# shuaigroup/Renormalizer

Measured on AMD Instinct MI355X. Metric: TDVP-PS sweep site-updates/sec at (Nsite=50, Dbond=256, dphys=2/16), higher is better.
Workload: dtype c128

## Files before the change

include/mpsengine.h:

```cpp
#ifndef MPSENGINE_H
#define MPSENGINE_H

#include <stddef.h>
#include <stdint.h>

#ifdef __cplusplus
extern "C" {
#endif

typedef struct mpse_ctx mpse_ctx;

enum {
  MPSE_OK = 0,
  MPSE_ERR_OOM = 1,
  MPSE_ERR_SHAPE = 2,
  MPSE_ERR_NOCONV = 3,
  MPSE_ERR_HIP = 4,
  MPSE_ERR_ARG = 5
};

enum { MPSE_F64 = 0, MPSE_C128 = 1 };
enum { MPSE_DOMAIN_L = 0, MPSE_DOMAIN_R = 1 };


// ... 78 lines not shown
  int64_t d0, d1;
  int64_t danc;
  int64_t wl, wm, wr;
  int64_t env_unit;
  int64_t danc1;
} mpse_dims;

int mpse_env_update(mpse_ctx* ctx, int dtype, int domain, const mpse_dims* dims,
                    const void* env, int env_dtype, const void* ket, const void* bra, int bra_conj,
                    const void* W, int w_dtype, void* out);

int mpse_env_update_multi(mpse_ctx* ctx, int dtype, int domain, const mpse_dims* dims, int n_mpo,
                          const int64_t* wl, const int64_t* wr, const void* env, int env_dtype,
                          const void* ket, const void* bra, int bra_conj, const void* const* W, int w_dtype, void* out);

int mpse_env_unit_channel(mpse_ctx* ctx, int dtype, const void* env, int64_t D, int64_t w, double tol,
                          int64_t* unit_host);

typedef struct {
  int nsite;
  mpse_dims dims;
  const void* L; int l_dtype;
  const void* R; int r_dtype;
  const void* W0; const void* W1; int w_dtype;
  int64_t l_unit, r_unit;
} mpse_heff;

int mpse_heff_apply(mpse_ctx* ctx, int dtype, const mpse_heff* h, const void* C, void* out);

int mpse_mpo_site_hint(mpse_ctx* ctx, const void* W_dev, const double* W_host_f64, int64_t wl, int64_t d, int64_t wr);

int mpse_heff_fused_stats(mpse_ctx* ctx, int64_t* bond_launches, int64_t* site_launches);

int mpse_heff_apply2(mpse_ctx* ctx, int dtype, const mpse_heff* h, const void* C, void* out);

enum { MPSE_LEG_UP = 0, MPSE_LEG_DOWN = 1 };
typedef struct {
  int64_t Dl, Dr, d_up, d_down;
  int64_t wl1, wr1, wl2, wr2;
  int leg1, leg2;
  int trans1, trans2;
  const void* L; int l_dtype;
  const void* R; int r_dtype;
  const void* W1; const void* W2; int w_dtype;
} mpse_heff_ft;

int mpse_heff_apply_ft(mpse_ctx* ctx, int dtype, const mpse_heff_ft* h, const void* C, void* out);

int mpse_env_update_ft(mpse_ctx* ctx, int dtype, int domain, const mpse_heff_ft* h, const void* env, int env_dtype,
                       const void* X, void* out);

int mpse_expm_centre_mask(mpse_ctx* ctx, const void* mask_dev, int64_t nbytes);

int mpse_expm_lanczos(mpse_ctx* ctx, int dtype, const mpse_heff* h, double dt_re, double dt_im,
                      const void* C, void* out, double rtol, double atol, int max_dim, int* nvec);
int mpse_expm_lanczos_batch(mpse_ctx* ctx, int dtype, int count, const mpse_heff* h, double dt_re, double dt_im,
                            const void* const* C, void* const* out, double rtol, double atol, int max_dim, int* nvec);
int mpse_expm_lanczos_batch_stats(mpse_ctx* ctx, int64_t* batched_members, int64_t* single_members);
int mpse_expm_lanczos_path_stats(mpse_ctx* ctx, int64_t* counts, int n);

int mpse_davidson(mpse_ctx* ctx, int dtype, const mpse_heff* h, int twolayer, const void* hdiag_f64,
                  const void* mask_f64, int nroots, int nguess, const void* guess, double tol, int max_cycle,
                  int max_space, double lindep, double shift, double* e_host, void* x_out, int* ncycle, int* nmatvec);

int mpse_pcg(mpse_ctx* ctx, int dtype, const mpse_heff* h, int twolayer, double shift, const void* diag_f64,
             const void* mask_f64, const void* b, void* x, double tol, int max_iter, int* iters_host,
             double* relres_host, double* lvalue_host);
int mpse_pcg_stats(mpse_ctx* ctx, int64_t* counts, int n);

int mpse_pcg_sum(mpse_ctx* ctx, int dtype, int nterms, const mpse_heff_ft* terms, const double* weights_host,
                 double shift, const void* diag_f64, const void* mask_f64, const void* b, void* x, double tol,
                 int max_iter, int* iters_host, double* relres_host, double* lvalue_host);
int mpse_pcg_sum_stats(mpse_ctx* ctx, int64_t* counts, int n);

int mpse_site_factor_ft(mpse_ctx* ctx, const mpse_heff_ft* h, void* S_f64);
int mpse_diag_ft(mpse_ctx* ctx, const mpse_heff_ft* h, const void* S_f64, double weight, double shift, int accumulate,
                 void* diag_f64);

int mpse_truncate_select(const double* sigma_host, const int64_t* block_id_host, int64_t count, int64_t m_max,
                         double percent, int64_t* picked_host, int64_t* npicked);


int mpse_block_qr(mpse_ctx* ctx, int dtype, const void* coef, int64_t nrow, int64_t ncol,
                  int nblocks, const int64_t* row_idx_host, const int64_t* row_off_host,
                  const int64_t* col_idx_host, const int64_t* col_off_host,
                  int system_is_R, void* U, void* Vt, int64_t K);

int mpse_block_qr_stats(mpse_ctx* ctx, int64_t* calls, int64_t* chol_calls, int64_t* chol_fallbacks);

int mpse_block_qr_optimistic(mpse_ctx* ctx, int on);
int mpse_block_qr_check(mpse_ctx* ctx, int* tripped);

int mpse_block_qr_pass_stats(mpse_ctx* ctx, int64_t* blocks, int64_t* two_pass);

int mpse_block_qr_scheme(mpse_ctx* ctx, int scheme);

int mpse_block_svd(mpse_ctx* ctx, int dtype, const void* coef, int64_t nrow, int64_t ncol,
                   int nblocks, const int64_t* row_idx_host, const int64_t* row_off_host,
                   const int64_t* col_idx_host, const int64_t* col_off_host,
                   void* U, void* Vt, double* S_host, int64_t K);

int mpse_block_svd_full(mpse_ctx* ctx, int dtype, const void* coef, int64_t nrow, int64_t ncol,
                        int nblocks, const int64_t* row_idx_host, const int64_t* row_off_host,
                        const int64_t* col_idx_host, const int64_t* col_off_host, const int64_t* extra_host,
                        void* U, int64_t KU, void* Vt, int64_t KV, double* S_host, int64_t K);

// ... 10 lines not shown
```

renormalizer_amd/csrc/mpse_contract.hip:

```cpp
#include <deque>

#include "mpse_internal.h"
#include "mpse_plans.h"

using namespace mpse_plan;

namespace {

__device__ __forceinline__ long long off2(const mpse_index m, long long i) {
  if (m.lo_ext >= m.ext) return i * m.s_lo;
  const long long hi = i / m.lo_ext;
  return hi * m.s_hi + (i - hi * m.lo_ext) * m.s_lo;
}

template <typename T>
__global__ __launch_bounds__(256) void k_copy_strided(T* dst, const T* src, mpse_index mi, mpse_index ni, mpse_index mo,
                                                      mpse_index no, const int* skip) {
  if (skip && *skip) return;
  const long long nn = ni.ext;
  const long long total = mi.ext * nn;
  const long long stride = (long long)gridDim.x * blockDim.x;
  for (long long t = (long long)blockIdx.x * blockDim.x + threadIdx.x; t < total; t += stride) {
    const long long i = t / nn, j = t - i * nn;
    dst[off2(mo, i) + off2(no, j)] = src[off2(mi, i) + off2(ni, j)];
// ... 268 lines not shown
      const dim3 grid((unsigned)((total + 255) / 256));
      if (s.dtb == MPSE_C128)
        hipLaunchKernelGGL((k_wsmall<true>), grid, dim3(256), 0, ctx->stream, g);
      else
        hipLaunchKernelGGL((k_wsmall<false>), grid, dim3(256), 0, ctx->stream, g);
      MPSE_HIP(ctx, hipGetLastError());
      continue;
    }
    if (s.kind == K_WMIX) {
      if (!bufs[s.b]) return mpse_fail(ctx, MPSE_ERR_ARG, "plan: missing buffer");
      WmixArgs g;
      memset(&g, 0, sizeof(g));
      g.W = (const double*)bufs[s.b];
      g.ndst = (int)s.mix.size();
      g.Da = (int)s.wp_Da, g.d = (int)s.wp_d, g.wr = (int)s.wp_wr, g.Dk = (int)s.wp_Dk;
      g.nchunk = (g.d + WM_CHUNK - 1) / WM_CHUNK;
      g.skip = skip;
      int nslot = 0;
      for (int j = 0; j < g.ndst; ++j) {
        const WMixDst& q = s.mix[j];
        if (!bufs[q.dst]) return mpse_fail(ctx, MPSE_ERR_ARG, "plan: missing buffer");
        g.dst[j].dst = (double*)((char*)const_cast<void*>(bufs[q.dst]) + size_t(q.dst_off) * es);
        g.dst[j].s_a = q.s_a, g.dst[j].s_d = q.s_d, g.dst[j].nterm = q.nterm;
        for (int t = 0; t < q.nterm; ++t) {
          const WMixTerm& tm = q.term[t];
          if (!bufs[tm.src]) return mpse_fail(ctx, MPSE_ERR_ARG, "plan: missing buffer");
          WmixTermDev& o = g.dst[j].term[t];
          o.src = (const double*)((const char*)bufs[tm.src] + size_t(tm.src_off) * es);
          o.s_a = tm.s_a, o.s_d = tm.s_d, o.b = tm.b, o.f = tm.f, o.ident = tm.ident ? 1 : 0;
          o.slot = tm.ident ? 0 : nslot++;
          memcpy(o.e_lo, tm.e_lo, sizeof(o.e_lo));
          memcpy(o.e_hi, tm.e_hi, sizeof(o.e_hi));
        }
      }
      g.nslot = nslot;
      const size_t lds = size_t(nslot > 0 ? nslot : 1) * g.d * g.d * sizeof(double);
      if (lds > 64 * 1024) return mpse_fail(ctx, MPSE_ERR_SHAPE, "plan: MPO blocks of the elementwise step exceed the LDS");
      const long long total = (long long)s.wp_Da * g.nchunk * s.wp_Dk;
      const dim3 grid((unsigned)((total + 255) / 256));
      if (dtype == MPSE_C128)
        hipLaunchKernelGGL((k_wmix<true>), grid, dim3(256), lds, ctx->stream, g);
      else
        hipLaunchKernelGGL((k_wmix<false>), grid, dim3(256), lds, ctx->stream, g);
      MPSE_HIP(ctx, hipGetLastError());
      continue;
    }
    if (s.kind == K_GGEMM) {
      GroupedDesc gd;
      gd.dta = s.dta, gd.dtb = s.dtb;
      gd.ma = s.ma, gd.ka = s.ka, gd.kb = s.kb, gd.nb = s.nb, gd.mc = s.mc, gd.nc = s.nc;
      gd.ngrp = (int)s.groups.size();
      TmpBuf MA(ctx), MB(ctx);
      const unsigned char *fa = nullptr, *fb = nullptr;
      bool stable = true;
      if (s.scan_a.on && bufs[s.scan_a.buf]) {
        bool st = false;
        MPSE_TRY(occ_mask_get(ctx, sc, (const char*)bufs[s.scan_a.buf] + size_t(s.scan_a.off) * dtype_size(s.scan_a.dt),
                              s.scan_a.dt, s.scan_a.r, s.scan_a.k, MA, &fa, &gd.am_pitch, &st));
        stable = stable && st;
      }
      if (s.scan_b.on && bufs[s.scan_b.buf]) {
        bool st = false;
        MPSE_TRY(occ_mask_get(ctx, sc, (const char*)bufs[s.scan_b.buf] + size_t(s.scan_b.off) * dtype_size(s.scan_b.dt),
                              s.scan_b.dt, s.scan_b.r, s.scan_b.k, MB, &fb, &gd.bm_pitch, &st));
        stable = stable && st;
      }
      const unsigned char* cm = nullptr;
      int cm_pitch = 0;
      {
        const char* pc = (const char*)bufs[B_C];
        const int64_t K = s.kb.ext, N = s.nb.ext;
        const int64_t nkw = ((K + 15) / 16 + 7) / 8, ntn = (N + 63) / 64;
        if (sc && sc->in_krylov(pc) && sc->cmask.bytes == ntn * nkw * 8) {
          cm = static_cast<const unsigned char*>(sc->cmask.ptr);
          cm_pitch = (int)(nkw * 8);
        }
      }
      for (int i = 0; i < gd.ngrp; ++i) {
        const GGroupPlan& g = s.groups[i];
        GroupedGrp& o = gd.grp[i];
        if (!bufs[g.cbuf]) return mpse_fail(ctx, MPSE_ERR_ARG, "plan: missing buffer");
        o.C = (char*)const_cast<void*>(bufs[g.cbuf]) + size_t(g.c_off) * es;
        o.nseg = g.nseg;
        o.beta = g.beta;
        for (int q = 0; q < g.nseg; ++q) {
          const GSegPlan& sg = g.seg[q];
          if (!bufs[sg.abuf] || !bufs[sg.bbuf]) return mpse_fail(ctx, MPSE_ERR_ARG, "plan: missing buffer");
          o.seg[q].A = (const char*)bufs[sg.abuf] + size_t(sg.a_off) * dtype_size(s.dta);
          o.seg[q].B = (const char*)bufs[sg.bbuf] + size_t(sg.b_off) * dtype_size(s.dtb);
          if (fa && sg.am_row0 >= 0) o.seg[q].am = fa + size_t(sg.am_row0) * gd.am_pitch;
          if (sg.bm_kind == BM_SCAN && fb) {
            o.seg[q].bm = fb + sg.bm_kt0;
          } else if (sg.bm_kind == BM_CENTRE && cm) {
            o.seg[q].bm = cm;
            gd.bm_pitch = cm_pitch;
          }
        }
      }
      gd.masks_stable = stable;
      if (gd.ngrp == 1 && s.groups[0].split2) {
        if (!bufs[B_OUT2]) return mpse_fail(ctx, MPSE_ERR_ARG, "plan: missing second result");
        gd.split2 = true;
        gd.c2 = const_cast<void*>(bufs[B_OUT2]);
      }
      const bool completes =
          &s == &p.steps.back() && gd.ngrp == 1 && s.groups[0].cbuf == B_OUT && s.groups[0].c_off == 0;
      MPSE_TRY(gemm_grouped(ctx, gd, sc, completes ? dot : nullptr));
      continue;
    }
    const char* a = (const char*)bufs[s.a] + size_t(s.a_off) * dtype_size(s.dta);
    const char* b = (const char*)bufs[s.b] + size_t(s.b_off) * dtype_size(s.dtb);
    const int dtc = (s.dta == MPSE_C128 || s.dtb == MPSE_C128) ? MPSE_C128 : MPSE_F64;
    if (dtc != dtype)
      return mpse_fail(ctx, MPSE_ERR_ARG, "plan step dtype mismatch (got %d want %d)", dtc, dtype);
    char* c = (char*)const_cast<void*>(bufs[s.c]) + size_t(s.c_off) * dtype_size(dtc);
    if (!bufs[s.a] || !bufs[s.b] || !bufs[s.c]) return mpse_fail(ctx, MPSE_ERR_ARG, "plan: missing buffer");
    if (s.kind == K_COPY) {
      MPSE_TRY(copy_call(ctx, dtc, a, c, s.ma, s.ka, s.mc, s.nc, skip));
      continue;
    }
    ProductReq rq;
    if (&s == &p.steps.back() && s.c == B_OUT && s.c_off == 0 && s.batch == 1) rq.dot = dot;
    if (s.cin >= 0) {
      if (!bufs[s.cin]) return mpse_fail(ctx, MPSE_ERR_ARG, "plan: missing beta source");
      rq.cin = (const char*)bufs[s.cin] + size_t(s.cin_off) * dtype_size(dtc);
      rq.cin_m = s.mcin;
      rq.cin_n = s.ncin;
    }
    if (&s == slice_producer) {
      const size_t blk = size_t(s.mc.ext) * size_t(s.nc.ext) * dtype_size(dtc);
      if (SLC.alloc(4 * blk) == MPSE_OK) {
        rq.slices = SLC.p;
        rq.slices_cap = 4 * blk;
      }
    }
    MPSE_TRY(gemm_call(ctx, s.dta, s.dtb, s.conja, s.conjb, s.ma, s.ka, s.kb, s.nb, s.mc, s.nc, s.batch, s.sba, s.sbb,
                       s.sbc, a, b, c, 1.0, s.beta, s.skip_zero, sc, &rq));
    if (rq.slices_used > 0) {
      slices_used = rq.slices_used;
      slice_elems = (long long)s.mc.ext * s.nc.ext;
      slice_b_lo = s.c_off / (slice_consumer->w_Da * slice_consumer->w_d * slice_consumer->w_N);
      slice_b_hi = slice_b_lo + s.mc.ext / slice_consumer->w_Da;
    }
  }
  return MPSE_OK;
}

int heff_apply(mpse_ctx* ctx, int dtype, const mpse_heff* h, const void* C, void* out, const SolveScope* sc,
               MatvecReq* mv) {
  if (!ctx || !h || !C || !out || !h->L || !h->R) return MPSE_ERR_ARG;
  MPSE_BIND(ctx);
  if (dtype != MPSE_C128 && (h->l_dtype == MPSE_C128 || h->r_dtype == MPSE_C128 || h->w_dtype == MPSE_C128))
// ... 204 lines not shown
```

renormalizer_amd/csrc/mpse_core.hip:

```cpp
#include "mpse_internal.h"
#include "mpse_plans.h"

int mpse_fail(mpse_ctx* ctx, int code, const char* fmt, ...) {
  if (ctx) {
    va_list ap;
    va_start(ap, fmt);
    vsnprintf(ctx->err, sizeof(ctx->err), fmt, ap);
    va_end(ap);
  }
  return code;
}

__global__ __launch_bounds__(256) void k_zero8(unsigned long long* dst, long long n) {
  for (long long i = (long long)blockIdx.x * 256 + threadIdx.x; i < n; i += (long long)gridDim.x * 256) dst[i] = 0ull;
}
__global__ __launch_bounds__(256) void k_copy8(unsigned long long* dst, const unsigned long long* __restrict__ src,
                                               long long n) {
  for (long long i = (long long)blockIdx.x * 256 + threadIdx.x; i < n; i += (long long)gridDim.x * 256) dst[i] = src[i];
}

__global__ __launch_bounds__(256) void k_zero8x2(unsigned long long* a, long long na, unsigned long long* b, long long nb) {
  for (long long i = (long long)blockIdx.x * 256 + threadIdx.x; i < na + nb; i += (long long)gridDim.x * 256) {
    if (i < na)
      a[i] = 0ull;
// ... 302 lines not shown

int mpse_device_info(mpse_ctx* ctx, char* name, size_t name_len, int* n_cu, void** stream) {
  if (!ctx) return MPSE_ERR_ARG;
  if (name && name_len) snprintf(name, name_len, "%s", ctx->dev_name);
  if (n_cu) *n_cu = ctx->n_cu;
  if (stream) *stream = (void*)ctx->stream;
  return MPSE_OK;
}

static size_t bucket_of(size_t bytes) {
  if (bytes < 256) return 256;
  if (bytes <= (size_t(1) << 20)) return (bytes + 255) & ~size_t(255);
  size_t p = size_t(1) << 20;
  while ((p << 1) <= bytes) p <<= 1;
  size_t step = p >> 3;
  return ((bytes + step - 1) / step) * step;
}

int mpse_malloc(mpse_ctx* ctx, size_t bytes, void** dptr) {
  if (!ctx || !dptr) return MPSE_ERR_ARG;
  MPSE_BIND(ctx);
  std::lock_guard<std::mutex> lock(ctx->pool_mu);
  size_t b = bucket_of(bytes);
  auto it = ctx->free_blocks.find(b);
  void* p = nullptr;
  if (it != ctx->free_blocks.end()) {
    p = it->second;
    ctx->free_blocks.erase(it);
  } else {
    hipError_t e = hipMalloc(&p, b);
    ++ctx->n_device_allocs;
    if (e != hipSuccess) {
      (void)hipGetLastError();
      pool_trim_locked(ctx);
      e = hipMalloc(&p, b);
      if (e != hipSuccess) {
        (void)hipGetLastError();
        *dptr = nullptr;
        return mpse_fail(ctx, MPSE_ERR_OOM, "hipMalloc(%zu) failed: %s (pool %zu B, in use %zu B)", b,
                         hipGetErrorString(e), ctx->pool_bytes, ctx->in_use_bytes);
      }
    }
    ctx->pool_bytes += b;
  }
  ctx->live[p] = b;
  ctx->in_use_bytes += b;
  *dptr = p;
  return MPSE_OK;
}

int mpse_free(mpse_ctx* ctx, void* dptr) {
  if (!ctx) return MPSE_ERR_ARG;
  if (!dptr) return MPSE_OK;
  std::lock_guard<std::mutex> lock(ctx->pool_mu);
  auto it = ctx->live.find(dptr);
  if (it == ctx->live.end()) return mpse_fail(ctx, MPSE_ERR_ARG, "mpse_free: unknown pointer %p", dptr);
  if (!ctx->wsite_info.empty()) ctx->wsite_info.erase(dptr);
  if (ctx->defer_hold) {
    ctx->defer_frees.push_back(dptr);
    return MPSE_OK;
  }
  ctx->free_blocks.emplace(it->second, dptr);
  ctx->in_use_bytes -= it->second;
  ctx->live.erase(it);
  return MPSE_OK;
}


int mpse_defer_begin(mpse_ctx* ctx, int list) {
  if (!ctx || list < 0 || list > 1) return MPSE_ERR_ARG;
  if (ctx->defer_recording >= 0) return mpse_fail(ctx, MPSE_ERR_ARG, "mpse_defer_begin: already recording");
  if (ctx->defer_armed == list) return mpse_fail(ctx, MPSE_ERR_ARG, "mpse_defer_begin: list %d is armed", list);
  ctx->defer_ops[list].clear();
  ctx->defer_recording = list;
  defer_update_hold(ctx);
  return MPSE_OK;
}

int mpse_defer_end(mpse_ctx* ctx) {
  if (!ctx) return MPSE_ERR_ARG;
  if (ctx->defer_recording < 0) return mpse_fail(ctx, MPSE_ERR_ARG, "mpse_defer_end: not recording");
  ctx->defer_recording = -1;
  defer_update_hold(ctx);
  return MPSE_OK;
}

int mpse_defer_arm(mpse_ctx* ctx, int list) {
  if (!ctx || list < 0 || list > 1) return MPSE_ERR_ARG;
  if (ctx->defer_recording >= 0) return mpse_fail(ctx, MPSE_ERR_ARG, "mpse_defer_arm: still recording");
  ctx->defer_armed = list;
  return MPSE_OK;
}

int mpse_defer_discard(mpse_ctx* ctx) {
  if (!ctx) return MPSE_ERR_ARG;
  ctx->defer_ops[0].clear();
  ctx->defer_ops[1].clear();
  ctx->defer_recording = ctx->defer_armed = -1;
  defer_update_hold(ctx);
  return MPSE_OK;
}

int mpse_defer_run(mpse_ctx* ctx, int list) {
  if (!ctx || list < 0 || list > 1) return MPSE_ERR_ARG;
  if (ctx->defer_recording >= 0) return mpse_fail(ctx, MPSE_ERR_ARG, "mpse_defer_run: still recording");
  MPSE_BIND(ctx);
// ... 113 lines not shown
```

renormalizer_amd/csrc/mpse_gemm.hip:

```cpp
#include <cstdlib>

#include "mpse_device.h"
#include "mpse_internal.h"

typedef double v4d __attribute__((ext_vector_type(4)));

static unsigned long long* gemm_trace_ptr(const mpse_ctx* ctx) {
  static const bool f0_only = [] {
    const char* e = getenv("MPSE_GEMM_TRACE_ONLY");
    return e && e[0] == 'f';
  }();
  return (ctx->prof_on && !f0_only) ? ctx->gemm_trace : nullptr;
}

namespace {

struct IdxMap {
  long long s_hi, s_lo;
  int ext, lo;
};

constexpr int GMAX_GRP = 8, GMAX_SEG = 4;
struct GSeg {
  const double* A;
// ... 1133 lines not shown
  if (base_blocks < tiles_limit && nkt_all >= 4) {
    int want = (int)((wg_target + base_blocks - 1) / base_blocks);
    int maxs = nkt_all / 2;
    int S = want < maxs ? want : maxs;
    if (S > 1) {
      g.kt_per_split = (nkt_all + S - 1) / S;
      g.ksplit = (nkt_all + g.kt_per_split - 1) / g.kt_per_split;
      const size_t esz = (ca || cb) ? 16 : 8;
      const size_t ws_bytes = size_t(d->batch) * g.ksplit * size_t(g.M) * size_t(g.N) * esz;
      const bool compact = is_single(g.mC) && is_single(g.nC) && g.mC.s_lo == g.N && (g.nC.s_lo == 1 || g.N == 1);
      if (rq && rq->slices && !rq->dot && d->batch == 1 && compact && !g.use_beta && d->alpha_re == 1.0 &&
          d->alpha_im == 0.0 && ws_bytes <= rq->slices_cap) {
        g.ws = static_cast<double*>(rq->slices);
        rq->slices_used = g.ksplit;
        leave_slices = true;
      } else {
        MPSE_TRY(WSB.alloc(ws_bytes));
        g.ws = WSB.as<double>();
      }
    }
  }
  g.slice_fast = g.ksplit > 1 && d->batch == 1;
  long long nblk = base_blocks * g.ksplit;
  if (nblk > 0x7fffffffLL) return mpse_fail(ctx, MPSE_ERR_SHAPE, "mpse_gemm: grid too large");

  MatvecReq::Dot* dot = rq ? rq->dot : nullptr;
  long long rgx = (g.N + 255) / 256 > 64 ? 64 : (g.N + 255) / 256;
  long long rgy = (long long)g.M * d->batch > 32768 ? 32768 : (long long)g.M * d->batch;
  if (dot && d->batch == 1) {
    long long producers = base_blocks;
    if (g.ksplit > 1) {
      const long long cap_y = dot->cap / rgx;
      if (cap_y >= 1 && rgy > cap_y) rgy = cap_y;
      producers = rgx * rgy;
    }
    if (producers >= 1 && producers <= dot->cap) {
      g.dot_y = static_cast<const double*>(dot->y);
      g.dot_part = dot->part;
      dot->nb_out = (int)producers;
    }
  }

  dim3 grid((unsigned)nblk), block(256);
  mpse_ctx::ProfRec rec;
  const int variant = (ca ? 1 : 0) + (cb ? 2 : 0);
  const double mnk = double(g.M) * double(g.N) * double(g.K) * double(d->batch);
  const bool prof_this = prof_begin(
      ctx, variant, mnk * ((ca && cb) ? 8.0 : (ca || cb) ? 4.0 : 2.0),
      double(d->batch) * (double(g.M) * g.K * (ca ? 16 : 8) + double(g.K) * g.N * (cb ? 16 : 8) +
                          double(g.M) * g.N * ((ca || cb) ? 16 : 8) * (g.use_beta ? 2 : 1)),
      &rec);
  g.kt_counter = prof_this && ctx->prof_ktiles ? ctx->prof_ktiles + variant : nullptr;
  bool mask_a_stable = true, mask_b_stable = true;
  if (skip_zero && is_single(g.kA) && is_single(g.kB) && nkt_all >= 2 && d->batch <= 16384) {
    g.nkw = (nkt_all + 7) / 8;
    const size_t wa = size_t(d->batch) * g.mtiles_m * g.nkw, wb = size_t(d->batch) * g.mtiles_n * g.nkw;
    const bool sa = skip_zero & 1, sb_ = skip_zero & 2;
    auto cacheable = [&](const void* p) { return sc && sc->in_env(p); };
    auto make_key = [&](const void* p, const IdxMap& rm, const IdxMap& km, long long sb, int nrows, int tiles, int cplx) {
      mpse_ctx::OccKey k;
      memset(&k, 0, sizeof(k));
      k.ptr = p;
      k.r_ext = rm.ext, k.r_lo = rm.lo, k.r_shi = rm.s_hi, k.r_slo = rm.s_lo;
      k.k_ext = km.ext, k.k_lo = km.lo, k.k_shi = km.s_hi, k.k_slo = km.s_lo;
      k.sb = sb, k.nrows = nrows, k.tiles = tiles, k.nkw = g.nkw, k.batch = (int)d->batch, k.K = g.K, k.cplx = cplx;
      return k;
    };
    auto find = [&](const mpse_ctx::OccKey& k) -> void* {
      for (const auto& e : ctx->occ_cache)
        if (memcmp(&e.key, &k, sizeof(k)) == 0) return e.mask;
      return nullptr;
    };
    unsigned long long *am = nullptr, *bmk = nullptr;
    bool scan_a = sa, scan_b = sb_, b_structural = false;
    mpse_ctx::OccKey ka, kb;
    const bool ca_ok = sa && cacheable(g.A), cb_ok = sb_ && cacheable(g.B);
    if (ca_ok) {
      ka = make_key(g.A, g.mA, g.kA, g.sbA, g.M, g.mtiles_m, ca ? 1 : 0);
      if (void* hit = find(ka)) am = static_cast<unsigned long long*>(hit), scan_a = false;
    }
    if (cb_ok) {
      kb = make_key(g.B, g.nB, g.kB, g.sbB, g.N, g.mtiles_n, cb ? 1 : 0);
      if (void* hit = find(kb)) bmk = static_cast<unsigned long long*>(hit), scan_b = false;
    }
    if (scan_b && sc && sc->in_krylov(g.B) && d->batch == 1 &&
        (long long)(wb * sizeof(unsigned long long)) == sc->cmask.bytes) {
      bmk = static_cast<unsigned long long*>(const_cast<void*>(sc->cmask.ptr));
      scan_b = false;
      b_structural = true;
    }
    mask_a_stable = !sa || ca_ok;
    mask_b_stable = !sb_ || cb_ok || b_structural;
    size_t tmp_words = 0;
    if (scan_a && !ca_ok) tmp_words += wa;
    if (scan_b && !cb_ok) tmp_words += wb;
    if (tmp_words) MPSE_TRY(MSK.alloc(tmp_words * sizeof(unsigned long long)));
    unsigned long long* tmp = MSK.as<unsigned long long>();
    if (scan_a) {
      if (ca_ok) {
        void* pm = nullptr;
        MPSE_TRY(mpse_malloc(ctx, wa * sizeof(unsigned long long), &pm));
        ctx->occ_cache.push_back({ka, pm});
        am = static_cast<unsigned long long*>(pm);
      } else {
        am = tmp;
        tmp += wa;
      }
    }
    if (scan_b) {
      if (cb_ok) {
        void* pm = nullptr;
        MPSE_TRY(mpse_malloc(ctx, wb * sizeof(unsigned long long), &pm));
        ctx->occ_cache.push_back({kb, pm});
        bmk = static_cast<unsigned long long*>(pm);
      } else {
        bmk = tmp;
      }
    }
    if (scan_a || scan_b) {
      OccOperand oa{g.A, g.mA, g.kA, g.M, scan_a ? g.mtiles_m : 0, ca ? 1 : 0, g.a_kfast, g.sbA, reinterpret_cast<unsigned char*>(am)};
      OccOperand ob{g.B, g.nB, g.kB, g.N, scan_b ? g.mtiles_n : 0, cb ? 1 : 0, g.b_kfast, g.sbB, reinterpret_cast<unsigned char*>(bmk)};
      const int tmax = (scan_a ? g.mtiles_m : 0) > (scan_b ? g.mtiles_n : 0) ? (scan_a ? g.mtiles_m : 0) : (scan_b ? g.mtiles_n : 0);
      const dim3 og((nkt_all + 3) / 4, tmax, (unsigned)(2 * d->batch));
      hipLaunchKernelGGL(k_tile_occ, og, dim3(256), 0, ctx->stream, oa, ob, g.K, g.nkw, (int)d->batch, skip);
    }
    g.amask = sa ? am : nullptr;
    g.bmask = sb_ ? bmk : nullptr;
  }
  TmpBuf PERM(ctx);
  const long long ntile_all = (long long)g.tiles_m * g.tiles_n;
  if (d->batch == 1 && (g.amask || g.bmask) && ntile_all * g.ksplit > 2 * n_cu && ntile_all <= 2048) {
    const bool keep = sc && sc->occ_cache && mask_a_stable && mask_b_stable;
    int* pp = nullptr;
    if (keep)
      for (const auto& e : ctx->perm_cache)
        if (e.amask == g.amask && e.bmask == g.bmask && e.tiles_m == g.tiles_m && e.tiles_n == g.tiles_n && e.nkt == nkt_all)
          pp = static_cast<int*>(e.perm);
    if (!pp) {
      if (keep) {
        void* pm = nullptr;
        MPSE_TRY(mpse_malloc(ctx, size_t(ntile_all) * sizeof(int), &pm));
        ctx->perm_cache.push_back({g.amask, g.bmask, g.tiles_m, g.tiles_n, nkt_all, pm});
        pp = static_cast<int*>(pm);
      } else {
        MPSE_TRY(PERM.alloc(size_t(ntile_all) * sizeof(int)));
        pp = PERM.as<int>();
      }
      hipLaunchKernelGGL(k_tile_order, dim3(1), dim3(1024), 0, ctx->stream, g.amask, g.bmask, g.nkw, nkt_all, g.tiles_m,
                         g.tiles_n, 1, pp, skip, GemmGroups(), (unsigned char*)nullptr, 0);
    }
    g.perm = pp;
  }
  auto span_ok = [](const IdxMap& m, const IdxMap& k, bool cplx) {
    if (m.s_hi < 0 || m.s_lo < 0 || k.s_hi < 0 || k.s_lo < 0) return false;
    auto span = [](const IdxMap& x) {
      if (x.ext <= 1) return 0.0;
      if (x.lo == 0x7fffffff) return double(x.ext - 1) * double(x.s_lo);
      return double((x.ext - 1) / x.lo) * double(x.s_hi) + double(x.lo - 1) * double(x.s_lo);
    };
    return (span(m) + span(k) + 1.0) * (cplx ? 16.0 : 8.0) < 4.0e9;
  };
  const bool ks = is_single(g.kA) && is_single(g.kB) && span_ok(g.mA, g.kA, ca) && span_ok(g.nB, g.kB, cb);
  if (!g.perm && g.ksplit == 1 && d->batch == 1 && (long long)g.tiles_m * g.tiles_n >= 64) {
    const double size_a = double(g.M) * (ca ? 2 : 1), size_b = double(g.N) * (cb ? 2 : 1);
    if (size_a >= size_b && g.tiles_m % 8 == 0)
      g.die_group = 1;
    else if (g.tiles_n % 8 == 0)
      g.die_group = 2;
    else if (g.tiles_m % 8 == 0)
      g.die_group = 1;
  }
#define MPSE_LAUNCH(CA_, CB_)                                                                         \
  do {                                                                                                \
    if (ks && wide)                                                                                   \
      hipLaunchKernelGGL((k_gemm<CA_, CB_, true, 2, 1>), grid, dim3(512), 0, ctx->stream, g);         \
    else if (ks)                                                                                      \
      hipLaunchKernelGGL((k_gemm<CA_, CB_, true, 2>), grid, block, 0, ctx->stream, g);                \
    else                                                                                              \
      hipLaunchKernelGGL((k_gemm<CA_, CB_, false, 2>), grid, block, 0, ctx->stream, g);               \
  } while (0)
  const bool wide = nblk <= n_cu && nkt_all >= 2;
  {
    long long* gp = ctx->gemm_paths;
    const bool masked = ks && (g.amask || g.bmask);
    ++gp[mpse_ctx::GP_LAUNCH];
    gp[mpse_ctx::GP_GENERAL] += !ks;
    gp[mpse_ctx::GP_WIDE] += ks && wide;
    gp[mpse_ctx::GP_SPLIT_B1] += g.ksplit > 1 && d->batch == 1;
    gp[mpse_ctx::GP_SPLIT_BN] += g.ksplit > 1 && d->batch > 1;
    gp[mpse_ctx::GP_DIE1] += g.die_group == 1;
    gp[mpse_ctx::GP_DIE2] += g.die_group == 2;
    gp[mpse_ctx::GP_SKEW] += g.skew && !g.perm && !g.die_group;
    gp[mpse_ctx::GP_ORDER] += g.perm != nullptr;
    gp[mpse_ctx::GP_MASK] += masked;
    gp[mpse_ctx::GP_MASK_GLOBAL] += masked && g.nkw > 64;
  }
  if (ca && cb)
    MPSE_LAUNCH(true, true);
  else if (ca)
    MPSE_LAUNCH(true, false);
  else if (cb)
    MPSE_LAUNCH(false, true);
  else
    MPSE_LAUNCH(false, false);
#undef MPSE_LAUNCH
  if (g.ksplit > 1 && !leave_slices) {
    const dim3 rgrid((unsigned)rgx, (unsigned)rgy);
    if (ca || cb)
      hipLaunchKernelGGL((k_splitk_reduce<true>), rgrid, dim3(256), 0, ctx->stream, g, (int)d->batch);
    else
      hipLaunchKernelGGL((k_splitk_reduce<false>), rgrid, dim3(256), 0, ctx->stream, g, (int)d->batch);
  }
  if (prof_this) prof_end(ctx, rec);
  MPSE_HIP(ctx, hipGetLastError());
  return MPSE_OK;
}

int occ_mask_get(mpse_ctx* ctx, const SolveScope* sc, const void* ptr, int dtype, mpse_index r, mpse_index k,
                 TmpBuf& tmp, const unsigned char** flags, int* pitch, bool* stable) {
  IdxMap rm, km;
  if (!to_map(r, &rm) || !to_map(k, &km) || !is_single(km))
    return mpse_fail(ctx, MPSE_ERR_SHAPE, "occupancy scan: K index must be single level");
  const int K = km.ext, nrows = rm.ext, nkt = (K + BK - 1) / BK, nkw = (nkt + 7) / 8, tiles = (nrows + BM - 1) / BM;
  const bool cplx = dtype == MPSE_C128;
  auto fastest = [](const IdxMap& m) { return m.ext <= 1 ? (long long)1 << 60 : (m.s_lo < 0 ? -m.s_lo : m.s_lo); };
  const int kfast = fastest(km) <= fastest(rm);
  mpse_ctx::OccKey key;
  memset(&key, 0, sizeof(key));
  key.ptr = ptr;
  key.r_ext = rm.ext, key.r_lo = rm.lo, key.r_shi = rm.s_hi, key.r_slo = rm.s_lo;
  key.k_ext = km.ext, key.k_lo = km.lo, key.k_shi = km.s_hi, key.k_slo = km.s_lo;
  key.sb = 0, key.nrows = nrows, key.tiles = tiles, key.nkw = nkw, key.batch = 1, key.K = K, key.cplx = cplx ? 1 : 0;
  const bool cacheable = sc && sc->in_env(ptr);
  *pitch = nkw * 8;
  *stable = cacheable;
  if (cacheable)
    for (const auto& e : ctx->occ_cache)
      if (memcmp(&e.key, &key, sizeof(key)) == 0) {
        *flags = static_cast<const unsigned char*>(e.mask);
        return MPSE_OK;
      }
  void* pm = nullptr;
  const size_t bytes = size_t(tiles) * nkw * 8;
  if (cacheable) {
    MPSE_TRY(mpse_malloc(ctx, bytes, &pm));
    ctx->occ_cache.push_back({key, pm});
  } else {
    MPSE_TRY(tmp.alloc(bytes));
    pm = tmp.p;
  }
  OccOperand oa{static_cast<const double*>(ptr), rm, km, nrows, tiles, cplx ? 1 : 0, kfast, 0, static_cast<unsigned char*>(pm)};
  OccOperand ob = oa;
  ob.tiles = 0;
  hipLaunchKernelGGL(k_tile_occ, dim3((nkt + 3) / 4, tiles, 2), dim3(256), 0, ctx->stream, oa, ob, K, nkw, 1,
                     sc ? sc->skip : nullptr);
  MPSE_HIP(ctx, hipGetLastError());
  *flags = static_cast<const unsigned char*>(pm);
  return MPSE_OK;
}

int gemm_grouped(mpse_ctx* ctx, const GroupedDesc& d, const SolveScope* sc, MatvecReq::Dot* dot) {
  GemmArgs g;
  memset(&g, 0, sizeof(g));
  if (d.ngrp < 1 || d.ngrp > GMAX_GRP) return mpse_fail(ctx, MPSE_ERR_ARG, "grouped product: 1 .. %d groups", GMAX_GRP);
  if (!to_map(d.ma, &g.mA) || !to_map(d.ka, &g.kA) || !to_map(d.kb, &g.kB) || !to_map(d.nb, &g.nB) ||
      !to_map(d.mc, &g.mC) || !to_map(d.nc, &g.nC))
    return mpse_fail(ctx, MPSE_ERR_SHAPE, "grouped product: extent out of range");
  g.M = g.mA.ext, g.N = g.nB.ext, g.K = g.kA.ext;
  if (g.M != g.mC.ext || g.N != g.nC.ext || g.K != g.kB.ext) return mpse_fail(ctx, MPSE_ERR_SHAPE, "grouped product: extents disagree");
  if (g.M == 0 || g.N == 0) return MPSE_OK;
  const bool ca = d.dta == MPSE_C128, cb = d.dtb == MPSE_C128;
  auto span_ok = [](const IdxMap& m, const IdxMap& k, bool cplx) {
    if (m.s_hi < 0 || m.s_lo < 0 || k.s_hi < 0 || k.s_lo < 0) return false;
    auto span = [](const IdxMap& x) {
      if (x.ext <= 1) return 0.0;
      if (x.lo == 0x7fffffff) return double(x.ext - 1) * double(x.s_lo);
      return double((x.ext - 1) / x.lo) * double(x.s_hi) + double(x.lo - 1) * double(x.s_lo);
    };
    return (span(m) + span(k) + 1.0) * (cplx ? 16.0 : 8.0) < 4.0e9;
  };
  if (!is_single(g.kA) || !is_single(g.kB) || !span_ok(g.mA, g.kA, ca) || !span_ok(g.nB, g.kB, cb) || g.K % BK != 0 ||
      g.K < BK || (d.ngrp > 1 && g.M % BM != 0) || !cb)
    return mpse_fail(ctx, MPSE_ERR_SHAPE, "grouped product: needs single-level K indices, K a multiple of %d, group "
                     "heights a multiple of %d and a complex second operand", BK, BM);
  g.mtiles_m = (g.M + BM - 1) / BM;
  g.mtiles_n = (g.N + BN - 1) / BN;
  g.tiles_m = g.mtiles_m * d.ngrp;
  g.tiles_n = g.mtiles_n;
  auto fast = [](const IdxMap& m) { return m.ext <= 1 ? (long long)1 << 60 : (m.s_lo < 0 ? -m.s_lo : m.s_lo); };
  g.a_kfast = fast(g.kA) <= fast(g.mA);
  g.b_kfast = fast(g.kB) <= fast(g.nB);
  g.alpha_re = 1.0, g.beta_re = 1.0;
  g.ksplit = 1;
  g.skip = sc ? sc->skip : nullptr;
  g.skew = 1;
  g.trace = gemm_trace_ptr(ctx);
  GemmGroups& gg = g.gg;
  gg.ngrp = d.ngrp, gg.tiles_m_grp = g.mtiles_m, gg.nkt_seg = g.K / BK;
  gg.am_pitch = d.am_pitch, gg.bm_pitch = d.bm_pitch;
  gg.split2 = d.split2 ? 1 : 0;
  gg.C2 = static_cast<double*>(d.c2);
  gg.cpd = (ctx->n_cu > 0 ? ctx->n_cu : 256) / 8;
  if (d.split2 && (d.ngrp != 1 || !d.c2 || g.M % BM != 0))
    return mpse_fail(ctx, MPSE_ERR_ARG, "grouped product: halved tiles need one group, whole tile rows and a second result");
  int max_seg = 0;
  bool any_mask = false, any_beta = false;
  for (int i = 0; i < d.ngrp; ++i) {
    const GroupedGrp& s = d.grp[i];
    if (s.nseg < 1 || s.nseg > GMAX_SEG || !s.C) return mpse_fail(ctx, MPSE_ERR_ARG, "grouped product: bad group");
    gg.g[i].C = static_cast<double*>(s.C);
    gg.g[i].nseg = s.nseg;
    gg.g[i].use_beta = s.beta != 0.0 ? 1 : 0;
    if (s.beta != 0.0 && s.beta != 1.0) return mpse_fail(ctx, MPSE_ERR_ARG, "grouped product: beta must be 0 or 1");
    any_beta = any_beta || s.beta != 0.0;
    for (int q = 0; q < s.nseg; ++q) {
      if (!s.seg[q].A || !s.seg[q].B) return mpse_fail(ctx, MPSE_ERR_ARG, "grouped product: null operand");
      gg.g[i].seg[q] = GSeg{static_cast<const double*>(s.seg[q].A), static_cast<const double*>(s.seg[q].B), s.seg[q].am, s.seg[q].bm};
      any_mask = any_mask || s.seg[q].am || s.seg[q].bm;
    }
    max_seg = s.nseg > max_seg ? s.nseg : max_seg;
  }
  g.A = gg.g[0].seg[0].A, g.B = gg.g[0].seg[0].B, g.C = gg.g[0].C;
  g.use_beta = any_beta;
  const int nkt_max = max_seg * gg.nkt_seg;
  g.nkw = (any_mask && (nkt_max + 7) / 8 <= 64) ? (nkt_max + 7) / 8 : 0;
  const int n_cu = ctx->n_cu > 0 ? ctx->n_cu : 256;
  const long long ntile = (long long)g.tiles_m * g.tiles_n;
  if (ntile > 0x7fffffffLL) return mpse_fail(ctx, MPSE_ERR_SHAPE, "grouped product: grid too large");
  const long long nwg = ntile * (d.split2 ? 2 : 1);
  if (dot && d.ngrp == 1 && nwg >= 1 && nwg <= dot->cap) {
    g.dot_y = static_cast<const double*>(dot->y);
    g.dot_part = dot->part;
    dot->nb_out = (int)nwg;
  }
  mpse_ctx::ProfRec rec;
  const int variant = (ca ? 1 : 0) + (cb ? 2 : 0);
  double segs = 0;
  for (int i = 0; i < d.ngrp; ++i) segs += d.grp[i].nseg;
  const double mnk = double(g.M) * double(g.N) * double(g.K) * segs;
  const bool prof_this = prof_begin(ctx, variant, mnk * ((ca && cb) ? 8.0 : 4.0),
                                    segs * (double(g.M) * g.K * (ca ? 16 : 8) + double(g.K) * g.N * 16.0) +
                                        double(d.ngrp) * double(g.M) * g.N * 16.0 * (any_beta ? 2 : 1),
                                    &rec);
  g.kt_counter = prof_this && ctx->prof_ktiles ? ctx->prof_ktiles + variant : nullptr;
  TmpBuf PERM(ctx);
  if (g.nkw > 0 && (ntile > 2 * n_cu || d.split2) && ntile <= 2048) {
    int* pp = nullptr;
    const void *ka = gg.g[0].seg[0].am, *kb = gg.g[0].seg[0].bm;
    const int nkt_key = nkt_max + 1000 * d.ngrp;
    const bool keep = sc && sc->occ_cache && d.masks_stable;
    if (keep)
      for (const auto& e : ctx->perm_cache)
        if (e.amask == ka && e.bmask == kb && e.tiles_m == g.tiles_m && e.tiles_n == g.tiles_n && e.nkt == nkt_key)
          pp = static_cast<int*>(e.perm);
    const size_t perm_bytes = (size_t(ntile) * sizeof(int) + 7) & ~size_t(7), flag_pitch = size_t(g.nkw) * 8;
    if (!pp) {
      if (keep) {
        void* pm = nullptr;
        MPSE_TRY(mpse_malloc(ctx, perm_bytes + size_t(ntile) * flag_pitch, &pm));
        ctx->perm_cache.push_back({ka, kb, g.tiles_m, g.tiles_n, nkt_key, pm});
        pp = static_cast<int*>(pm);
      } else {
        MPSE_TRY(PERM.alloc(perm_bytes + size_t(ntile) * flag_pitch));
        pp = PERM.as<int>();
      }
      hipLaunchKernelGGL(k_tile_order, dim3(1), dim3(1024), 0, ctx->stream, (const unsigned long long*)nullptr,
                         (const unsigned long long*)nullptr, 0, nkt_max, g.tiles_m, g.tiles_n, d.split2 ? 0 : 1, pp,
                         g.skip, gg, reinterpret_cast<unsigned char*>(pp) + perm_bytes, (int)flag_pitch);
    }
    g.perm = pp;
    g.gg.flags = reinterpret_cast<const unsigned long long*>(reinterpret_cast<const char*>(pp) + perm_bytes);
  }
  if (!g.perm && ntile >= 64) {
    const double size_a = double(g.M) * d.ngrp * (ca ? 2 : 1), size_b = double(g.N) * 2;
    if (size_a >= size_b && g.tiles_m % 8 == 0)
      g.die_group = 1;
    else if (g.tiles_n % 8 == 0)
      g.die_group = 2;
    else if (g.tiles_m % 8 == 0)
      g.die_group = 1;
  }
  const dim3 grid((unsigned)nwg);
  const bool wide = nwg <= n_cu;
  ++ctx->gemm_paths[mpse_ctx::GP_GROUPED];
  ctx->gemm_paths[mpse_ctx::GP_GROUPED_SPLIT2] += gg.split2 != 0;
  if (ca) {
    if (wide)
      hipLaunchKernelGGL((k_gemm<true, true, true, 2, 1, true>), grid, dim3(512), 0, ctx->stream, g);
    else
      hipLaunchKernelGGL((k_gemm<true, true, true, 2, 2, true>), grid, dim3(256), 0, ctx->stream, g);
  } else {
    if (wide)
      hipLaunchKernelGGL((k_gemm<false, true, true, 2, 1, true>), grid, dim3(512), 0, ctx->stream, g);
    else
      hipLaunchKernelGGL((k_gemm<false, true, true, 2, 2, true>), grid, dim3(256), 0, ctx->stream, g);
  }
  if (prof_this) prof_end(ctx, rec);
  MPSE_HIP(ctx, hipGetLastError());
  return MPSE_OK;
}

extern "C" int mpse_gemm(mpse_ctx* ctx, const mpse_gemm_desc* d, const void* A, const void* B, void* C) {
  if (ctx && d && MPSE_RECORDING(ctx)) {
    const mpse_gemm_desc dc = *d;
    ctx->defer_ops[ctx->defer_recording].push_back([ctx, dc, A, B, C] { return mpse_gemm(ctx, &dc, A, B, C); });
    return MPSE_OK;
  }
  return gemm_impl(ctx, d, A, B, C, d ? (d->skip_zero_tiles & 3) : 0, nullptr, nullptr);
}

extern "C" int mpse_gemm_path_stats(mpse_ctx* ctx, int64_t* counts, int n) {
  if (!ctx || n < 0 || (n > 0 && !counts)) return MPSE_ERR_ARG;
  for (int i = 0; i < n && i < mpse_ctx::GP_COUNT; ++i) counts[i] = ctx->gemm_paths[i];
  return MPSE_OK;
}

int gemm_call(mpse_ctx* ctx, int dta, int dtb, int conja, int conjb, mpse_index ma, mpse_index ka, mpse_index kb,
              mpse_index nb, mpse_index mc, mpse_index nc, int64_t batch, int64_t sba, int64_t sbb, int64_t sbc,
              const void* A, const void* B, void* C, double alpha, double beta, int skip_zero, const SolveScope* sc,
              ProductReq* rq) {
  mpse_gemm_desc d;
// ... 40 lines not shown
```

renormalizer_amd/csrc/mpse_heff0.hip:

```cpp
#include "mpse_device.h"
#include "mpse_internal.h"

typedef double v4d __attribute__((ext_vector_type(4)));

namespace {

__device__ __forceinline__ v4d mfma(double a, double b, v4d c) {
  return __builtin_amdgcn_mfma_f64_16x16x4f64(a, b, c, 0, 0, 0);
}

constexpr int F0_TMAX = 16;
struct F0Term {
  int b, e, x, pad;
  double w;
};
struct F0Info {
  int unit;
  int nt;
  unsigned long long lts;
  unsigned long long frn;
  unsigned long long cts;
  unsigned bpack, epack;
  double w[4];
};
// ... 12 lines not shown
  const int* nterm;
  const int* skip;
  const F0Info* info;
  long long n;
  int Dl, Dr, wl, wr, d, ntl, ntr, nkc, fc_pitch;
  unsigned long long* trace;
};

__device__ __forceinline__ void f0_transpose(double2* __restrict__ rt, const double2* __restrict__ r, int D, int w, int blk,
                                             int nblk) {
  const long long n = (long long)D * w * D;
  const long long stride = (long long)nblk * 256;
  for (long long i = (long long)blk * 256 + threadIdx.x; i < n; i += stride) {
    const int l = (int)(i % D);
    const long long bk = i / D;
    rt[i] = r[(long long)l * w * D + bk];
  }
}

__device__ __forceinline__ void f0_flags(const double2* __restrict__ E, int D, int w, int nt, unsigned char* __restrict__ F,
                                         int rt, int b) {
  __shared__ int s_f[64];
  const int row = threadIdx.x >> 4, col = threadIdx.x & 15;
  if (threadIdx.x < 64) s_f[threadIdx.x] = 0;
  __syncthreads();
  const double2* base = E + ((long long)(16 * rt + row) * w + b) * D;
  for (int ct = 0; ct < nt; ++ct) {
    const double2 v = base[16 * ct + col];
    if (v.x != 0.0 || v.y != 0.0) s_f[ct] = 1;
  }
  __syncthreads();
  if ((int)threadIdx.x < nt) F[((long long)rt * w + b) * nt + threadIdx.x] = s_f[threadIdx.x] ? 1 : 0;
}

__global__ __launch_bounds__(256) void k_f0_prepare(const double2* __restrict__ L, const double2* __restrict__ R,
                                                     double2* __restrict__ rt, unsigned char* __restrict__ FL,
                                                     unsigned char* __restrict__ FR, int Dl, int Dr, int wl, int wr, int ntl,
                                                     int ntr, const int* __restrict__ skip) {
  if (skip && *skip) return;
  int blk = blockIdx.x;
  if (blk < ntl * wl) {
    f0_flags(L, Dl, wl, ntl, FL, blk / wl, blk % wl);
    return;
  }
  blk -= ntl * wl;
  if (blk < ntr * wr) {
    f0_flags(R, Dr, wr, ntr, FR, blk / wr, blk % wr);
    return;
  }
  blk -= ntr * wr;
  f0_transpose(rt, R, Dr, wr, blk, (int)gridDim.x - ntl * wl - ntr * wr);
}

__global__ __launch_bounds__(1024) void k_f0_valid(const unsigned char* __restrict__ FL, const unsigned char* __restrict__ FC,
                                                    const unsigned char* __restrict__ FR, const F0Term* __restrict__ terms,
                                                    const int* __restrict__ nterm, int wl, int wr, int d, int ntl, int ntr,
                                                    int nkc, int fc_pitch, unsigned long long* __restrict__ mask,
                                                    const int* __restrict__ skip) {
  if (skip && *skip) return;
  __shared__ unsigned long long s1[64], s2[64];
  const int nparts = wr * nkc, tid = threadIdx.x;
  if (tid < 64) s1[tid] = s2[tid] = 0;
  __syncthreads();
  for (int t = tid; t < ntl * nparts; t += 1024) {
    const int at = t / nparts, s = t - at * nparts, f = s / nkc, kc = s - f * nkc;
    bool any = false;
    for (int q = 0; q < nterm[f]; ++q) {
      const F0Term tm = terms[f * F0_TMAX + q];
      for (int ct = 0; ct < ntl; ++ct)
        any = any || (FL[((long long)at * wl + tm.b) * ntl + ct] && (!FC || FC[(tm.e * nkc + kc) * fc_pitch + ct]));
    }
    if (any) atomicOr(&s1[at], 1ull << s);
  }
  for (int t = tid; t < ntr * nparts; t += 1024) {
    const int lt = t / nparts, s = t - lt * nparts, f = s / nkc, kc = s - f * nkc;
    bool any = false;
    for (int j = 0; j < 4; ++j) {
      const int kt = 4 * kc + j;
      if (kt < ntr) any = any || FR[((long long)lt * wr + f) * ntr + kt];
    }
    if (any) atomicOr(&s2[lt], 1ull << s);
  }
  __syncthreads();
  for (int t = tid; t < ntl * d * ntr; t += 1024) {
    const int row = t / ntr, lt = t - row * ntr;
    mask[t] = s1[row / d] & s2[lt];
  }
}

__global__ __launch_bounds__(1024) void k_f0_plan(const unsigned char* __restrict__ FL, const unsigned char* __restrict__ FC,
                                                   const unsigned char* __restrict__ FR, const F0Term* __restrict__ terms,
                                                   const int* __restrict__ nterm, int wl, int wr, int d, int ntl, int ntr,
                                                   int nkc, int fc_pitch, unsigned long long* __restrict__ mask, int n_cu,
                                                   F0Info* __restrict__ info, int compact, const int* __restrict__ skip) {
  if (skip && *skip) return;
  constexpr int WMAX = 256, MROWS = 1024;
  __shared__ unsigned long long s1[64], s2[64];
  __shared__ int hist[WMAX], start[WMAX], s_nw;
  __shared__ unsigned long long mL[MROWS], mR[MROWS], mC[64];
  __shared__ F0Term sT[16 * F0_TMAX];
  __shared__ int sNT[16];
  const int nparts = wr * nkc, tid = threadIdx.x, lane = tid & 63, wave = tid >> 6, nu = ntl * nparts * d;
  auto rows_to_masks = [&](const unsigned char* F, int nrows, int nt, int pitch, unsigned long long* out) {
    for (int r0 = wave; r0 < nrows; r0 += 64) {
      unsigned char v[4];
#pragma unroll
// ... 412 lines not shown
  if (dot && nwg * d > dot->cap) return MPSE_OK;
  std::vector<F0Term> terms(size_t(wr) * F0_TMAX);
  std::vector<int> nterm(wr, 0);
  for (int f = 0; f < wr; ++f) {
    if (h->nsite == 0) {
      terms[size_t(f) * F0_TMAX] = F0Term{f, 0, 0, 0, 1.0};
      nterm[f] = 1;
      continue;
    }
    for (int b = 0; b < wl; ++b)
      for (int x = 0; x < d; ++x)
        for (int e = 0; e < d; ++e) {
          const double v = w_host[((size_t(b) * d + x) * d + e) * wr + f];
          if (v == 0.0) continue;
          if (nterm[f] == F0_TMAX) return MPSE_OK;
          terms[size_t(f) * F0_TMAX + nterm[f]++] = F0Term{b, e, x, 0, v};
        }
  }
  const unsigned char* FC = nullptr;
  int fc_pitch = 0;
  {
    const long long nkw = (ntl + 7) / 8;
    const char* pc = static_cast<const char*>(C);
    if (sc && sc->in_krylov(pc) && sc->cmask.bytes == (long long)d * nkc * nkw * 8) {
      FC = static_cast<const unsigned char*>(sc->cmask.ptr);
      fc_pitch = (int)(nkw * 8);
    }
  }
  const size_t rt_bytes = size_t(wr) * Dr * Dr * 16;
  const size_t fl_bytes = (size_t(ntl) * wl * ntl + 15) & ~size_t(15), fr_bytes = (size_t(ntr) * wr * ntr + 15) & ~size_t(15);
  const size_t tm_bytes = terms.size() * sizeof(F0Term), nt_bytes = (size_t(wr) * sizeof(int) + 15) & ~size_t(15);
  const size_t mk_bytes = size_t(ntl) * d * ntr * 8;
  const size_t nu = size_t(nwg) * d;
  const size_t od_bytes = (nu * sizeof(F0Info) + 15) & ~size_t(15);
  bool compact = ntl <= 16 && ntr <= 16 && wl <= 255 && d <= 255;
  for (int f = 0; f < wr && compact; ++f)
    for (int x = 0; x < d; ++x) {
      int c = 0;
      for (int q = 0; q < nterm[f]; ++q) c += terms[size_t(f) * F0_TMAX + q].x == x;
      if (c > 4) compact = false;
    }
  if (!sc) return MPSE_OK;
  const int* skip = sc->skip;
  mpse_ctx::F0Cache& fc = ctx->f0;
  char* base = nullptr;
  const bool hit = fc.buf && fc.L == h->L && fc.R == h->R && fc.W == h->W0 && fc.cmask == (const void*)FC && fc.Dl == Dl &&
                   fc.Dr == Dr && fc.w == wr && fc.nsite == h->nsite;
  const size_t o_fl = rt_bytes, o_fr = o_fl + fl_bytes, o_tm = o_fr + fr_bytes, o_nt = o_tm + tm_bytes, o_mk = o_nt + nt_bytes;
  const size_t o_od = o_mk + mk_bytes, tot_bytes = o_od + od_bytes;
  static const bool order_on = [] {
    const char* e = getenv("MPSE_F0_ORDER");
    return !(e && e[0] == '0');
  }();
  if (hit) {
    base = static_cast<char*>(fc.buf);
  } else {
    void* p = nullptr;
    heff0_drop_cache(ctx);
    MPSE_TRY(mpse_malloc(ctx, tot_bytes, &p));
    fc.buf = p, fc.L = h->L, fc.R = h->R, fc.W = h->W0, fc.cmask = FC, fc.Dl = Dl, fc.Dr = Dr, fc.w = wr, fc.nsite = h->nsite;
    base = static_cast<char*>(p);
    {
      std::vector<char> up(tm_bytes + nt_bytes, 0);
      memcpy(up.data(), terms.data(), tm_bytes);
      memcpy(up.data() + tm_bytes, nterm.data(), size_t(wr) * sizeof(int));
      MPSE_TRY(stage_h2d(ctx, base + o_tm, up.data(), up.size()));
    }
    const long long nel = (long long)wr * Dr * Dr;
    int nb = (int)((nel + 255) / 256);
    if (nb > 2048) nb = 2048;
    hipLaunchKernelGGL(k_f0_prepare, dim3(ntl * wl + ntr * wr + nb), dim3(256), 0, ctx->stream,
                       static_cast<const double2*>(h->L), static_cast<const double2*>(h->R), reinterpret_cast<double2*>(base),
                       reinterpret_cast<unsigned char*>(base + o_fl), reinterpret_cast<unsigned char*>(base + o_fr), Dl, Dr, wl,
                       wr, ntl, ntr, skip);
    if (order_on)
      hipLaunchKernelGGL(k_f0_plan, dim3(1), dim3(1024), 0, ctx->stream, reinterpret_cast<const unsigned char*>(base + o_fl), FC,
                         reinterpret_cast<const unsigned char*>(base + o_fr), reinterpret_cast<const F0Term*>(base + o_tm),
                         reinterpret_cast<const int*>(base + o_nt), wl, wr, d, ntl, ntr, nkc, fc_pitch,
                         reinterpret_cast<unsigned long long*>(base + o_mk), ctx->n_cu > 0 ? ctx->n_cu : 256,
                         reinterpret_cast<F0Info*>(base + o_od), compact ? 1 : 0, skip);
    else
      hipLaunchKernelGGL(k_f0_valid, dim3(1), dim3(1024), 0, ctx->stream, reinterpret_cast<const unsigned char*>(base + o_fl), FC,
                         reinterpret_cast<const unsigned char*>(base + o_fr), reinterpret_cast<const F0Term*>(base + o_tm),
                         reinterpret_cast<const int*>(base + o_nt), wl, wr, d, ntl, ntr, nkc, fc_pitch,
                         reinterpret_cast<unsigned long long*>(base + o_mk), skip);
  }
  F0Args g{};
  g.L = static_cast<const double*>(h->L);
  g.Rt = reinterpret_cast<const double*>(base);
  g.C = static_cast<const double*>(C);
  g.parts = static_cast<double*>(pr.ptr);
  g.FL = reinterpret_cast<const unsigned char*>(base + o_fl);
  g.FC = FC;
  g.FR = reinterpret_cast<const unsigned char*>(base + o_fr);
  g.terms = reinterpret_cast<const F0Term*>(base + o_tm);
  g.nterm = reinterpret_cast<const int*>(base + o_nt);
  g.mask = reinterpret_cast<const unsigned long long*>(base + o_mk);
  g.skip = skip;
  g.info = order_on ? reinterpret_cast<const F0Info*>(base + o_od) : nullptr;
  g.trace = ctx->prof_on ? ctx->gemm_trace : nullptr;
  g.n = n;
  g.Dl = Dl, g.Dr = Dr, g.wl = wl, g.wr = wr, g.d = d, g.ntl = ntl, g.ntr = ntr, g.nkc = nkc, g.fc_pitch = fc_pitch;
  if (dot) {
    g.y = static_cast<const double*>(dot->y);
    g.dot_part = dot->part;
    dot->nb_out = nwg * d;
  }
  {
    const double fl = h->nsite == 0 ? 8.0 * wr * double(Dl) * Dr * (double(Dl) + Dr)
                                    : 8.0 * double(Dl) * Dl * wl * d * Dr + 4.0 * double(Dl) * Dr * wl * wr * d * d +
                                          8.0 * double(Dl) * Dr * Dr * wr * d;
    const double by = 16.0 * (double(Dl) * wl * Dl + double(Dr) * wr * Dr + 2.0 * double(n));
    ProfScope fprof(ctx, 7, fl, by);
    hipLaunchKernelGGL(k_heff0_fused, dim3(nwg * d), dim3(256), 0, ctx->stream, g);
    fprof.end();
  }
  MPSE_HIP(ctx, hipGetLastError());
  ++ctx->f0_launches[h->nsite == 1 ? 1 : 0];
  pr.used = nparts;
  pr.mask = g.mask;
  pr.mask_row = Dr;
  pr.mask_tiles = ntr;
  *taken = true;
  return MPSE_OK;
}

extern "C" int mpse_heff_fused_stats(mpse_ctx* ctx, int64_t* bond_launches, int64_t* site_launches) {
  if (!ctx) return MPSE_ERR_ARG;
  if (bond_launches) *bond_launches = ctx->f0_launches[0];
  if (site_launches) *site_launches = ctx->f0_launches[1];
  return MPSE_OK;
}
```

renormalizer_amd/csrc/mpse_internal.h:

```cpp
#pragma once
#include <hip/hip_runtime.h>

#include <cstdarg>
#include <cstdlib>
#include <cstdint>
#include <cstdio>
#include <cstring>
#include <functional>
#include <map>
#include <memory>
#include <mutex>
#include <string>
#include <unordered_map>
#include <vector>

#include "../../include/mpsengine.h"

struct mpse_ctx {
  int device = 0;
  hipStream_t stream = nullptr;
  int n_cu = 0;
  char err[512] = {0};
  char dev_name[128] = {0};

// ... 47 lines not shown
  };
  std::unordered_map<const void*, WSiteEntry> wsite_info;
  std::vector<std::function<int()>> defer_ops[2];
  int defer_recording = -1;
  int defer_armed = -1;
  bool defer_hold = false;
  std::vector<void*> defer_frees;
  struct CMask {
    const void* ptr = nullptr;
    long long bytes = 0;
  } cmask_pending;
  unsigned long long* gemm_trace = nullptr;
  bool gemm_trace_checked = false;
  std::vector<OccEntry> occ_cache;
  struct PermEntry {
    const void *amask, *bmask;
    int tiles_m, tiles_n, nkt;
    void* perm;
  };
  std::vector<PermEntry> perm_cache;
  struct SmallRt {
    const void* src = nullptr;
    void* rt = nullptr;
    size_t bytes = 0;
  } small_rt;
  struct F0Cache {
    void* buf = nullptr;
    const void *L = nullptr, *R = nullptr, *W = nullptr, *cmask = nullptr;
    int Dl = 0, Dr = 0, w = 0, nsite = -1;
  } f0;
  long long f0_launches[2] = {0, 0};
  enum GemmPath {
    GP_LAUNCH, GP_GENERAL, GP_WIDE, GP_SPLIT_B1, GP_SPLIT_BN, GP_DIE1, GP_DIE2, GP_SKEW, GP_ORDER, GP_MASK,
    GP_MASK_GLOBAL, GP_GROUPED, GP_GROUPED_SPLIT2, GP_COUNT
  };
  long long gemm_paths[GP_COUNT] = {0};
  long long qr_chol_calls = 0, qr_chol_fallbacks = 0, qr_calls = 0;
  bool qr_optimistic = false;
  int qr_scheme = -1;
  int* qr_words_dev = nullptr;
  long long lz_batch_members = 0, lz_batch_single = 0;
  enum LzPath {
    LP_SYNC, LP_ASYNC_DONE, LP_HOST_FIRST, LP_HOST_LATER, LP_LIMIT, LP_BD_ASYNC, LP_BD_SYNC, LP_FULL, LP_CONV,
    LP_NOCONV, LP_MERGED, LP_WAITS, LP_GROW, LP_PARTS, LP_VMASK, LP_UNVEC, LP_RESCALE, LP_ALIAS_RESTART, LP_COUNT
  };
  long long lz_paths[LP_COUNT] = {0};
  enum PcgStat {
    PS_SOLVES, PS_ITERS, PS_MATVECS, PS_WAITS, PS_END_TOL, PS_END_MAXITER, PS_END_CURVATURE, PS_TWOLAYER, PS_MASKED,
    PS_COUNT
  };
  long long pcg_stats[PS_COUNT] = {0};
  enum PcgSumStat { PSS_SOLVES, PSS_ITERS, PSS_TERM_APPLIES, PSS_WAITS, PSS_DIAGS, PSS_COUNT };
  long long pcg_sum_stats[PSS_COUNT] = {0};
};
int qr_words(mpse_ctx* ctx);

int mpse_fail(mpse_ctx* ctx, int code, const char* fmt, ...);
inline int mpse_bind(mpse_ctx* ctx) {
  int cur = -1;
  if (hipGetDevice(&cur) == hipSuccess && cur == ctx->device) return MPSE_OK;
  if (hipSetDevice(ctx->device) != hipSuccess) return mpse_fail(ctx, MPSE_ERR_HIP, "hipSetDevice(%d) failed", ctx->device);
  return MPSE_OK;
}
int stage_h2d(mpse_ctx* ctx, void* dst, const void* src_host, size_t bytes);
int device_zero(mpse_ctx* ctx, void* dst, size_t bytes);
inline void wsite_written(mpse_ctx* ctx, const void* dst, size_t bytes) {
  if (!dst || !bytes) return;
  std::lock_guard<std::mutex> lock(ctx->pool_mu);
  if (ctx->wsite_info.empty()) return;
  const char* lo = static_cast<const char*>(dst);
  for (auto it = ctx->wsite_info.begin(); it != ctx->wsite_info.end();) {
    const char* w = static_cast<const char*>(it->first);
    if (lo < w + it->second.bytes && w < lo + bytes)
      it = ctx->wsite_info.erase(it);
    else
      ++it;
  }
}
void prof_drain(mpse_ctx* ctx);
bool prof_begin(mpse_ctx* ctx, int variant, double flops, double bytes, mpse_ctx::ProfRec* rec);
void prof_end(mpse_ctx* ctx, const mpse_ctx::ProfRec& rec);
struct ProfScope {
  mpse_ctx* ctx;
  mpse_ctx::ProfRec rec;
  bool on;
  ProfScope(mpse_ctx* c, int variant, double flops, double bytes) : ctx(c), on(prof_begin(c, variant, flops, bytes, &rec)) {}
  ProfScope(const ProfScope&) = delete;
  ProfScope& operator=(const ProfScope&) = delete;
  void end() {
    if (on) prof_end(ctx, rec);
    on = false;
  }
  ~ProfScope() {
    if (!on) return;
    ctx->prof_free_events.push_back(rec.e0);
    ctx->prof_free_events.push_back(rec.e1);
  }
};

#define MPSE_HIP(ctx, call)                                                              \
  do {                                                                                   \
    hipError_t _e = (call);                                                              \
    if (_e != hipSuccess)                                                                \
      return mpse_fail((ctx), (_e == hipErrorOutOfMemory) ? MPSE_ERR_OOM : MPSE_ERR_HIP, \
                       "%s:%d %s -> %s", __FILE__, __LINE__, #call, hipGetErrorString(_e)); \
  } while (0)

#define MPSE_TRY(call)            \
  do {                            \
    int _s = (call);              \
    if (_s != MPSE_OK) return _s; \
  } while (0)

#define MPSE_BIND(ctx) MPSE_TRY(mpse_bind(ctx))

#define MPSE_RECORDING(ctx) ((ctx)->defer_recording >= 0)
int defer_replay(mpse_ctx* ctx, int status);

struct TmpBuf {
  mpse_ctx* ctx;
  void* p = nullptr;
  TmpBuf(mpse_ctx* c) : ctx(c) {}
  int alloc(size_t bytes) { return mpse_malloc(ctx, bytes ? bytes : 16, &p); }
  ~TmpBuf() {
    if (p) mpse_free(ctx, p);
  }
  template <class T>
  T* as() { return reinterpret_cast<T*>(p); }
};

static inline size_t dtype_size(int dt) { return dt == MPSE_C128 ? 16 : 8; }
static inline mpse_index idx1(int64_t ext, int64_t stride) { return mpse_index{ext, ext > 0 ? ext : 1, 0, stride}; }
static inline mpse_index idx2(int64_t hi_ext, int64_t lo_ext, int64_t s_hi, int64_t s_lo) {
  return mpse_index{hi_ext * lo_ext, lo_ext > 0 ? lo_ext : 1, s_hi, s_lo};
}

struct SolveScope {
  mpse_ctx* ctx;
  const int* skip = nullptr;
  bool occ_cache = false;
  const char* env_lo[2] = {nullptr, nullptr};
  const char* env_hi[2] = {nullptr, nullptr};
  mpse_ctx::CMask cmask;
  const char* krylov_lo = nullptr;
  const char* krylov_hi = nullptr;

  explicit SolveScope(mpse_ctx* c) : ctx(c) {}
  SolveScope(const SolveScope&) = delete;
  SolveScope& operator=(const SolveScope&) = delete;
  ~SolveScope();
  bool in_env(const void* p) const {
    const char* c = static_cast<const char*>(p);
    return occ_cache && ((c >= env_lo[0] && c < env_hi[0]) || (c >= env_lo[1] && c < env_hi[1]));
  }
  bool in_krylov(const void* p) const {
    const char* c = static_cast<const char*>(p);
    return cmask.ptr && c && c >= krylov_lo && c < krylov_hi;
  }
};

struct MatvecReq {
  struct Dot {
    const void* y = nullptr;
    double* part = nullptr;
    int cap = 0;
    int nb_out = 0;
  } dot;
  struct Parts {
    void* ptr = nullptr;
    long long cap_elems = 0, n = 0;
    int used = 0;
    bool masked_ok = false;
    const unsigned long long* mask = nullptr;
    int mask_row = 0, mask_tiles = 0;
  } parts;
};

struct ProductReq {
  MatvecReq::Dot* dot = nullptr;
  const void* cin = nullptr;
  mpse_index cin_m{}, cin_n{};
  void* slices = nullptr;
  size_t slices_cap = 0;
  int slices_used = 0;
};

int heff_apply(mpse_ctx* ctx, int dtype, const mpse_heff* h, const void* C, void* out, const SolveScope* sc,
               MatvecReq* mv);
int heff_apply2(mpse_ctx* ctx, int dtype, const mpse_heff* h, const void* C, void* out, const SolveScope* sc);
int heff_apply_ft(mpse_ctx* ctx, int dtype, const mpse_heff_ft* h, const void* C, void* out, const SolveScope* sc);
int heff_small_try(mpse_ctx* ctx, int dtype, const mpse_heff* h, const void* C, void* out, const SolveScope* sc,
                   MatvecReq* mv, bool* taken);
void heff_small_drop_cache(mpse_ctx* ctx);

struct BatchMember {
  const void* L;
  const void* R;
  const void* W;
  void* Rt;
  const void* C;
  void* out;
};
template <class T>
__host__ __device__ inline T* member_ptr(T* p, unsigned m, long long mstride) {
  return p ? reinterpret_cast<T*>(reinterpret_cast<uintptr_t>(p) + uintptr_t(m) * uintptr_t(mstride)) : p;
}
bool heff_small_batch_plan(const mpse_heff* h, int dtype, int64_t n, int dot_cap, size_t* rt_bytes, int* nparts,
                           int* nb_dot);
int heff_small_batch_rt(mpse_ctx* ctx, int dtype, const mpse_heff* h, int B, const BatchMember* mem, const int* skip0,
                        long long mstride);
int heff_small_batch_apply(mpse_ctx* ctx, int dtype, const mpse_heff* h, int B, const BatchMember* mem,
                           const void* C0, void* parts0, int64_t n, double* dot_part0, int dot_cap, const int* skip0,
                           long long mstride);
int heff0_fused_parts(const mpse_heff* h, int dtype);
int heff0_fused_try(mpse_ctx* ctx, int dtype, const mpse_heff* h, const void* C, const double* w_host,
                    const SolveScope* sc, MatvecReq* mv, bool* taken);
void heff0_drop_cache(mpse_ctx* ctx);
inline SolveScope::~SolveScope() {
  for (auto& e : ctx->occ_cache) mpse_free(ctx, e.mask);
  ctx->occ_cache.clear();
  for (auto& e : ctx->perm_cache) mpse_free(ctx, e.perm);
  ctx->perm_cache.clear();
  heff_small_drop_cache(ctx);
}

int gemm_call(mpse_ctx* ctx, int dta, int dtb, int conja, int conjb, mpse_index ma, mpse_index ka,
              mpse_index kb, mpse_index nb, mpse_index mc, mpse_index nc, int64_t batch, int64_t sba,
              int64_t sbb, int64_t sbc, const void* A, const void* B, void* C, double alpha = 1.0,
              double beta = 0.0, int skip_zero = 0, const SolveScope* sc = nullptr, ProductReq* rq = nullptr);

struct GroupedSeg {
  const void* A = nullptr;
  const void* B = nullptr;
  const unsigned char* am = nullptr;
  const unsigned char* bm = nullptr;
};
struct GroupedGrp {
  GroupedSeg seg[4];
  void* C = nullptr;
  int nseg = 0;
  double beta = 0.0;
};
struct GroupedDesc {
  int dta = MPSE_F64, dtb = MPSE_F64;
  mpse_index ma{}, ka{}, kb{}, nb{}, mc{}, nc{};
  int ngrp = 0;
  GroupedGrp grp[8];
  int am_pitch = 0, bm_pitch = 0;
  bool masks_stable = false;
  bool split2 = false;
  void* c2 = nullptr;
};
int gemm_grouped(mpse_ctx* ctx, const GroupedDesc& d, const SolveScope* sc, MatvecReq::Dot* dot);
int occ_mask_get(mpse_ctx* ctx, const SolveScope* sc, const void* ptr, int dtype, mpse_index r, mpse_index k,
                 TmpBuf& tmp, const unsigned char** flags, int* pitch, bool* stable);

int publish_and_wait(mpse_ctx* ctx, const double* dsrc, int count, int slot);
int publish_wait_seq(mpse_ctx* ctx, double seq, const double* dsrc, int count, int slot);

int dotc_sync(mpse_ctx* ctx, int dtype, const void* x, const void* y, int64_t n, double* re, double* im);

struct HhParam {
  double tau_re, tau_im;
  double scale_re, scale_im;
  double g[6];
};
struct QrBlk {
  long long ws_off;
  long long q_off;
  int mm, nn, k;
  int prm_off;
  int nq = 0;
  long long row_off = 0, col_off = 0;
};
constexpr int HH_BATCH_MAX_ROWS = 4096;
constexpr unsigned long long GEMM_TRACE_CAP = 1ull << 21;
constexpr int GEMM_TRACE_WORDS = 10;
int hh_qr(mpse_ctx* ctx, bool cplx, double* ws, double* q, HhParam* prm, const QrBlk* blks_host, int nblk, bool form_q,
          const QrBlk* blks_dev = nullptr);
bool cholqr_eligible(const mpse_ctx* ctx, const QrBlk* blks, int nblk);
int cholqr_blocks(mpse_ctx* ctx, bool cplx, double* ws, const QrBlk* blks, int nblk, const long long* drows,
                  const long long* dcols, int herm, void* U, void* Vt, long long K, long long ncol, bool* ok);
int device_zero2(mpse_ctx* ctx, void* a, size_t abytes, void* b, size_t bbytes);
```

renormalizer_amd/csrc/mpse_vec.hip:

```cpp
#include <cmath>
#include <complex>
#include <cstdlib>

#include "mpse_device.h"
#include "mpse_internal.h"

namespace {

template <bool CPLX>
__global__ __launch_bounds__(RED_THREADS) void k_dot_partial(const double* __restrict__ x, const double* __restrict__ y,
                                                             long long n, double* __restrict__ partial,
                                                             const int* __restrict__ done) {
  if (done && *done) return;
  double re = 0, im = 0;
  const long long stride = (long long)gridDim.x * RED_THREADS;
  if (CPLX) {
    const double2* x2 = reinterpret_cast<const double2*>(x);
    const double2* y2 = reinterpret_cast<const double2*>(y);
    for (long long i = (long long)blockIdx.x * RED_THREADS + threadIdx.x; i < n; i += 2 * stride) {
      const long long i1 = i + stride;
      const bool h1 = i1 < n;
      const double2 a0 = x2[i], b0 = y2[i];
      const double2 a1 = h1 ? x2[i1] : make_double2(0.0, 0.0), b1 = h1 ? y2[i1] : make_double2(0.0, 0.0);
      re += a0.x * b0.x + a0.y * b0.y;
// ... 814 lines not shown
  const size_t lb = size_t(s.Dl_ket) * s.wl * s.Dl_ket * (h->l_dtype == MPSE_C128 ? 16 : 8);
  const size_t rb = size_t(s.Dr_ket) * s.wr * s.Dr_ket * (h->r_dtype == MPSE_C128 ? 16 : 8);
  sc.env_lo[0] = static_cast<const char*>(h->L), sc.env_hi[0] = sc.env_lo[0] + lb;
  sc.env_lo[1] = static_cast<const char*>(h->R), sc.env_hi[1] = sc.env_lo[1] + rb;
  sc.occ_cache = true;
}

constexpr int LZ_FALLBACK = -77;
constexpr int LZ_BADSTART = -78;

int expm_lanczos_async(mpse_ctx* ctx, int dtype, const mpse_heff* h, std::complex<double> dt, const void* Cin, void* out,
                       double rtol, double atol, int max_dim, int* nvec, int64_t n) {
  const bool cplx = dtype == MPSE_C128;
  const size_t es = dtype_size(dtype);
  const int64_t nd = n * (cplx ? 2 : 1);
  const double tiny = 100.0 * double(n) * 2.220446049250313e-16;
  const int limit = max_dim < LZ_MAXM ? max_dim : LZ_MAXM;
  const unsigned long long key = ((unsigned long long)h->nsite << 60) ^ ((unsigned long long)n << 1) ^ (cplx ? 1ull : 0ull);
  int hint = 0;
  {
    auto it = ctx->lz_hint.find(key);
    if (it != ctx->lz_hint.end()) hint = it->second;
  }
  int wait_from = hint > 0 ? hint - 1 : 6;
  if (wait_from < 6) wait_from = 6;

  int cap = hint + 4 > 16 ? hint + 4 : 16;
  if (cap > limit + 1) cap = limit + 1;
  TmpBuf V(ctx), W(ctx), RES(ctx), SCAL(ctx);
  MPSE_TRY(V.alloc(size_t(cap) * n * es));
  long long wcap = (n <= 65536 ? 4 : 2) * n;
  const int f0_parts = (cplx && (reinterpret_cast<uintptr_t>(Cin) & 15) == 0) ? heff0_fused_parts(h, dtype) : 0;
  if ((long long)f0_parts * n > wcap) wcap = (long long)f0_parts * n;
  MPSE_TRY(W.alloc(size_t(wcap) * es));
  MPSE_TRY(RES.alloc(size_t(n) * es));
  const int SC_CTL = 4 + 4 * 130, SC_COEF = SC_CTL + 8;
  MPSE_TRY(SCAL.alloc(size_t(SC_COEF + 4 * LZ_MAXM) * sizeof(double)));
  double* scal = SCAL.as<double>();
  LzCtl* ctl = reinterpret_cast<LzCtl*>(scal + SC_CTL);
  double* coef = scal + SC_COEF;
  const int* done = &ctl->done;
  const int nb = red_blocks(nd);
  constexpr int DOT_CAP = 4096;
  double* part_a = ctx->dscratch + 16 * RED_MAX_BLOCKS;
  static_assert(16 * RED_MAX_BLOCKS + 2 * DOT_CAP < (1 << 16) - 8, "dot partials fit the device scratch");
  double* part_b = ctx->dscratch + 4 * RED_MAX_BLOCKS;
  const bool vec16 = (cplx || n % 2 == 0) && (reinterpret_cast<uintptr_t>(Cin) & 15) == 0;
  const double vbytes = double(n) * double(es);
  auto vec = [&](int j) { return V.as<char>() + size_t(j) * n * es; };

  SolveScope scope(ctx);
  scope.skip = done;
  keep_env_masks(scope, h);
  scope.cmask = ctx->cmask_pending;
  ctx->cmask_pending = mpse_ctx::CMask();

  const unsigned char* vmask = nullptr;
  int vm_row = 0, vm_kw = 0;
  static const bool vmask_on = [] {
    const char* e = getenv("MPSE_VEC_MASK");
    return !(e && e[0] == '0');
  }();
  if (vmask_on && vec16 && cplx && scope.cmask.ptr && h->dims.Dl_ket > 0 && h->dims.Dl_bra == h->dims.Dl_ket &&
      h->dims.Dr_bra == h->dims.Dr_ket && n < (int64_t(1) << 31)) {
    const int64_t Dl = h->dims.Dl_ket, N = n / Dl;
    const int64_t nkw = ((Dl + 15) / 16 + 7) / 8;
    if (N * Dl == n && N % 64 == 0 && scope.cmask.bytes == (N / 64) * nkw * 8) {
      vmask = static_cast<const unsigned char*>(scope.cmask.ptr);
      vm_row = (int)N;
      vm_kw = (int)(nkw * 8);
    }
  }
  auto bracket = [&](double bytes, auto&& launch) {
    mpse_ctx::ProfRec rec;
    const bool pt = prof_begin(ctx, 4, 0.0, bytes, &rec);
    launch();
    if (pt) prof_end(ctx, rec);
  };
  auto dot_partials = [&](const void* x, const void* y, double* dst) {
    bracket(2.0 * vbytes, [&] {
      if (cplx)
        hipLaunchKernelGGL((k_dot_partial<true>), dim3(nb), dim3(RED_THREADS), 0, ctx->stream, (const double*)x,
                           (const double*)y, (long long)n, dst, done);
      else
        hipLaunchKernelGGL((k_dot_partial<false>), dim3(nb), dim3(RED_THREADS), 0, ctx->stream, (const double*)x,
                           (const double*)y, (long long)n, dst, done);
    });
  };
  auto scale_into = [&](void* dst, const void* src, double* b2_out) {
    bracket(2.0 * vbytes, [&] {
      if (vec16)
        hipLaunchKernelGGL(k_scale_into_dev<true>, dim3(nb), dim3(RED_THREADS), 0, ctx->stream, (double*)dst,
                           (const double*)src, (long long)nd, (const double*)part_b, nb, b2_out, done);
      else
        hipLaunchKernelGGL(k_scale_into_dev<false>, dim3(nb), dim3(RED_THREADS), 0, ctx->stream, (double*)dst,
                           (const double*)src, (long long)nd, (const double*)part_b, nb, b2_out, done);
    });
  };
  double* part_b2[2] = {ctx->dscratch + 4 * RED_MAX_BLOCKS, ctx->dscratch + 8 * RED_MAX_BLOCKS};
  bracket(3.0 * vbytes, [&] {
    if (cplx)
      hipLaunchKernelGGL((k_lz_start<true>), dim3(nb), dim3(RED_THREADS), 0, ctx->stream, (double*)vec(0), (const double*)Cin,
                         (long long)n, part_b2[0], ctl);
    else
      hipLaunchKernelGGL((k_lz_start<false>), dim3(nb), dim3(RED_THREADS), 0, ctx->stream, (double*)vec(0),
                         (const double*)Cin, (long long)n, part_b2[0], ctl);
// ... 267 lines not shown
  out_host[0] = sqrt(re);
  return MPSE_OK;
}

static int expm_lanczos_solve(mpse_ctx* ctx, int dtype, const mpse_heff* h, double dt_re, double dt_im, const void* Cin,
                              void* out, double rtol, double atol, int max_dim, int* nvec, bool async_first = true,
                              bool rescale_ok = true);

static int expm_lanczos_rescaled(mpse_ctx* ctx, int dtype, const mpse_heff* h, double dt_re, double dt_im,
                                 const void* Cin, void* out, double rtol, double atol, int max_dim, int* nvec, int64_t n,
                                 const mpse_ctx::CMask& cmask, bool rescale_ok) {
  const int64_t nd = n * (dtype == MPSE_C128 ? 2 : 1);
  std::vector<double> hv(static_cast<size_t>(nd));
  MPSE_TRY(mpse_memcpy_d2h(ctx, hv.data(), Cin, size_t(nd) * sizeof(double)));
  double mx = 0.0;
  for (double x : hv) {
    if (!std::isfinite(x)) return mpse_fail(ctx, MPSE_ERR_ARG, "expm_lanczos: non-finite start vector");
    mx = std::max(mx, std::fabs(x));
  }
  if (!(mx > 0.0)) return mpse_fail(ctx, MPSE_ERR_ARG, "expm_lanczos: zero start vector");
  if (!rescale_ok) return mpse_fail(ctx, MPSE_ERR_ARG, "expm_lanczos: start vector out of range after scaling");
  const int e = -std::ilogb(mx);
  for (double& x : hv) x = std::ldexp(x, e);
  TmpBuf S(ctx);
  MPSE_TRY(S.alloc(size_t(nd) * sizeof(double)));
  MPSE_TRY(mpse_memcpy_h2d(ctx, S.p, hv.data(), size_t(nd) * sizeof(double)));
  ++ctx->lz_paths[mpse_ctx::LP_RESCALE];
  ctx->cmask_pending = cmask;
  const int st = expm_lanczos_solve(ctx, dtype, h, dt_re, dt_im, S.p, out, rtol, std::ldexp(atol, e), max_dim, nvec,
                                    true, false);
  if (st == MPSE_OK || st == MPSE_ERR_NOCONV) {
    hipLaunchKernelGGL((k_scal<false>), dim3(ew_blocks(nd)), dim3(256), 0, ctx->stream, (double*)out, (long long)nd,
                       std::ldexp(1.0, -e), 0.0);
    MPSE_HIP(ctx, hipGetLastError());
  }
  return st;
}

int mpse_expm_centre_mask(mpse_ctx* ctx, const void* mask_dev, int64_t nbytes) {
  if (!ctx || (nbytes > 0 && !mask_dev) || nbytes < 0) return MPSE_ERR_ARG;
  ctx->cmask_pending = mpse_ctx::CMask();
  if (nbytes > 0) {
    ctx->cmask_pending.ptr = mask_dev;
    ctx->cmask_pending.bytes = nbytes;
  }
  return MPSE_OK;
}

int mpse_expm_lanczos(mpse_ctx* ctx, int dtype, const mpse_heff* h, double dt_re, double dt_im, const void* Cin,
                      void* out, double rtol, double atol, int max_dim, int* nvec) {
  if (!ctx || !h || !Cin || !out) return MPSE_ERR_ARG;
  if (MPSE_RECORDING(ctx)) return mpse_fail(ctx, MPSE_ERR_ARG, "expm_lanczos: cannot be recorded (mpse_defer_begin is open)");
  MPSE_BIND(ctx);
  const int st = expm_lanczos_solve(ctx, dtype, h, dt_re, dt_im, Cin, out, rtol, atol, max_dim, nvec);
  ctx->cmask_pending = mpse_ctx::CMask();
  return defer_replay(ctx, st);
}

static int expm_lanczos_solve(mpse_ctx* ctx, int dtype, const mpse_heff* h, double dt_re, double dt_im, const void* Cin,
                              void* out, double rtol, double atol, int max_dim, int* nvec, bool async_first,
                              bool rescale_ok) {
  const bool cplx = dtype == MPSE_C128;
  if (!cplx && dt_im != 0.0)
    return mpse_fail(ctx, MPSE_ERR_ARG, "expm_lanczos: complex time step needs a complex128 centre tensor");
  const mpse_dims& s = h->dims;
  if ((s.Dl_bra > 0 && s.Dl_bra != s.Dl_ket) || (s.Dr_bra > 0 && s.Dr_bra != s.Dr_ket))
    return mpse_fail(ctx, MPSE_ERR_SHAPE, "expm_lanczos: the effective Hamiltonian must be square (bra bonds == ket bonds)");
  const int64_t anc = s.danc > 0 ? s.danc : 1;
  int64_t n = s.Dl_ket * s.Dr_ket;
  if (h->nsite >= 1) n *= s.d0 * anc;
  if (h->nsite == 2) n *= s.d1 * (s.danc1 > 0 ? s.danc1 : anc);
  if (n <= 0) return mpse_fail(ctx, MPSE_ERR_SHAPE, "expm_lanczos: empty centre tensor");
  if (max_dim <= 0 || max_dim > 128) max_dim = 128;
  const size_t es = dtype_size(dtype);
  {
    const char *c0 = static_cast<const char*>(Cin), *o0 = static_cast<const char*>(out);
    const size_t bytes = size_t(n) * es;
    if (o0 != c0 && o0 < c0 + bytes && c0 < o0 + bytes)
      return mpse_fail(ctx, MPSE_ERR_ARG, "expm_lanczos: out overlaps C without being C");
  }
  const mpse_ctx::CMask cmask = ctx->cmask_pending;
  if (async_first && lanczos_async_enabled() && n > 256) {
    const int st = expm_lanczos_async(ctx, dtype, h, std::complex<double>(dt_re, dt_im), Cin, out, rtol, atol, max_dim,
                                      nvec, n);
    if (st == LZ_BADSTART)
      return expm_lanczos_rescaled(ctx, dtype, h, dt_re, dt_im, Cin, out, rtol, atol, max_dim, nvec, n, cmask, rescale_ok);
    if (st != LZ_FALLBACK) return st;
  }
  ++ctx->lz_paths[mpse_ctx::LP_SYNC];
  const int64_t nd = n * (cplx ? 2 : 1);
  const std::complex<double> dt(dt_re, dt_im);
  const double tiny = 100.0 * double(n) * 2.220446049250313e-16;

  int cap = 16;
  TmpBuf V(ctx), W(ctx), RES(ctx), SCAL(ctx);
  MPSE_TRY(V.alloc(size_t(cap) * n * es));
  MPSE_TRY(W.alloc(size_t(n) * es));
  const int SC_FLAG = 4 + 4 * 130;
  MPSE_TRY(SCAL.alloc(size_t(SC_FLAG + 2) * sizeof(double)));
  double* scal = SCAL.as<double>();
  const int nb = red_blocks(nd);
  double* part_a = ctx->dscratch;
  double* part_b = ctx->dscratch + 4 * RED_MAX_BLOCKS;

  const double vbytes = double(n) * double(es);
  auto dot_partials = [&](const void* x, const void* y, double* dst_partial) {
    mpse_ctx::ProfRec rec;
    const bool pt = prof_begin(ctx, 4, 0.0, 2.0 * vbytes, &rec);
// ... 24 lines not shown

  std::vector<double> alpha, beta;
  double nrmv = 0.0, nrm2 = 0.0;
  bool have_res = false;
  void* res_prev = nullptr;
  int pending_m = 0;
  auto vec = [&](int j) { return V.as<char>() + size_t(j) * n * es; };
  auto fetch = [&](int upto) -> int {
    const int cnt = 4 + 4 * (upto + 1);
    MPSE_TRY(publish_and_wait(ctx, scal, cnt, 16));
    if (ctx->prof_pending.size() > 2048) prof_drain(ctx);
    const double* p = ctx->pinned + 16;
    nrm2 = p[0];
    nrmv = sqrt(p[0]);
    for (int j = (int)alpha.size(); j <= upto; ++j) {
      alpha.push_back(p[4 + 4 * j]);
      beta.push_back(sqrt(p[6 + 4 * j]));
    }
    return MPSE_OK;
  };
  auto finish = [&](int m, void* dst, const void* prev, int* flag_out) -> int {
    Coefs c;
    expm_coefs(m, alpha, beta, nrmv, dt, &c);
    unsigned int* dflag = reinterpret_cast<unsigned int*>(ctx->dscratch + (size_t(1) << 16) - 8);
    unsigned int gen = 0;
    if (prev) {
      gen = ++ctx->flag_gen;
      if (gen == 0) {
        MPSE_HIP(ctx, hipMemsetAsync(dflag, 0, sizeof(unsigned int), ctx->stream));
        gen = ++ctx->flag_gen;
      }
    }
    if (cplx)
      hipLaunchKernelGGL((k_lincomb<true>), dim3(ew_blocks(n)), dim3(256), 0, ctx->stream, (double*)dst,
                         V.as<double>(), (long long)n, m, c, (const double*)prev, rtol, atol, dflag, gen);
    else
      hipLaunchKernelGGL((k_lincomb<false>), dim3(ew_blocks(n)), dim3(256), 0, ctx->stream, (double*)dst,
                         V.as<double>(), (long long)n, m, c, (const double*)prev, rtol, atol, dflag, gen);
    MPSE_HIP(ctx, hipGetLastError());
    if (prev && flag_out) {
      MPSE_TRY(publish_and_wait(ctx, reinterpret_cast<const double*>(dflag), 1, 8));
      *flag_out = (*reinterpret_cast<unsigned int*>(ctx->pinned + 8) == gen) ? 1 : 0;
    }
    return MPSE_OK;
  };
  auto breakdown_at = [&](int upto) -> int {
    for (int j = 0; j <= upto && j < (int)beta.size(); ++j)
      if (!(beta[j] >= tiny)) return j;
    return -1;
  };

  SolveScope scope(ctx);
  keep_env_masks(scope, h);
  for (int j = 0;; ++j) {
    MPSE_TRY(heff_apply(ctx, dtype, h, vec(j), W.p, &scope, nullptr));
    dot_partials(W.p, vec(j), part_a);
    if (j == n - 1) {
      hipLaunchKernelGGL(k_reduce_final, dim3(1), dim3(RED_THREADS), 0, ctx->stream, part_a, nb, scal + 4 + 4 * j,
                         (const int*)nullptr);
      MPSE_TRY(fetch(j));
      if (!(nrm2 >= LZ_N2_MIN && nrm2 < LZ_N2_MAX))
        return expm_lanczos_rescaled(ctx, dtype, h, dt_re, dt_im, Cin, out, rtol, atol, max_dim, nvec, n, cmask, rescale_ok);
      int bd = breakdown_at(j - 1);
      const int m = bd >= 0 ? bd + 1 : j + 1;
      ++ctx->lz_paths[bd >= 0 ? mpse_ctx::LP_BD_SYNC : mpse_ctx::LP_FULL];
      MPSE_TRY(finish(m, out, nullptr, nullptr));
      if (nvec) *nvec = m;
      return MPSE_OK;
    }
    if (!vec16) ++ctx->lz_paths[mpse_ctx::LP_UNVEC];
    mpse_ctx::ProfRec urec;
    const bool upt = prof_begin(ctx, 4, 0.0, (j > 0 ? 4.0 : 3.0) * vbytes, &urec);
    if (vec16)
      hipLaunchKernelGGL(k_lanczos_update<true>, dim3(nb), dim3(RED_THREADS), 0, ctx->stream, W.as<double>(),
                         (const double*)vec(j), j > 0 ? (const double*)vec(j - 1) : (const double*)nullptr,
                         (long long)nd, (const double*)part_a, nb, scal + 4 + 4 * j,
                         (const double*)(scal + 6 + 4 * (j > 0 ? j - 1 : 0)), part_b, (const int*)nullptr);
    else
      hipLaunchKernelGGL(k_lanczos_update<false>, dim3(nb), dim3(RED_THREADS), 0, ctx->stream, W.as<double>(),
                         (const double*)vec(j), j > 0 ? (const double*)vec(j - 1) : (const double*)nullptr,
                         (long long)nd, (const double*)part_a, nb, scal + 4 + 4 * j,
                         (const double*)(scal + 6 + 4 * (j > 0 ? j - 1 : 0)), part_b, (const int*)nullptr);
    if (upt) prof_end(ctx, urec);
    const bool check = (j > 3 && j % 2 == 0);
    const bool last = (j + 1 >= max_dim);
    const bool defer = check && !have_res && pending_m == 0 && !last;
    const bool sync_now = (check && !defer) || last;
    if (sync_now)
      hipLaunchKernelGGL(k_reduce_final, dim3(1), dim3(RED_THREADS), 0, ctx->stream, part_b, nb, scal + 6 + 4 * j,
                         (const int*)nullptr);
    MPSE_HIP(ctx, hipGetLastError());
    if (sync_now) {
      MPSE_TRY(fetch(j));
      if (!(nrm2 >= LZ_N2_MIN && nrm2 < LZ_N2_MAX))
        return expm_lanczos_rescaled(ctx, dtype, h, dt_re, dt_im, Cin, out, rtol, atol, max_dim, nvec, n, cmask, rescale_ok);
      const int bd = breakdown_at(j);
      if (bd >= 0) {
        ++ctx->lz_paths[mpse_ctx::LP_BD_SYNC];
        MPSE_TRY(finish(bd + 1, out, nullptr, nullptr));
        if (nvec) *nvec = bd + 1;
        return MPSE_OK;
      }
    }
    if (defer) {
      pending_m = j + 1;
    } else if (check) {
// ... 215 lines not shown
        bool all = true;
        for (int m = 0; m < B; ++m) {
          if (hc[m].bad || hc[m].need_host) single[m] = 1;
          else if (hc[m].done) fin[m] = 1;
          else all = false;
        }
        if (all) break;
      }
    }
    if (last) {
      for (int m = 0; m < B; ++m)
        if (!fin[m]) single[m] = 1;
      break;
    }
  }
  int best = 0;
  for (int m = 0; m < B; ++m) {
    if (!fin[m]) continue;
    if (hc[m].which == 1)
      MPSE_TRY(mpse_memcpy_d2d(ctx, outs[bs.idx[m]], member_ptr(RES, m, mstride), size_t(n) * es));
    if (nvec) nvec[bs.idx[m]] = hc[m].nvec;
    if (hc[m].nvec > best) best = hc[m].nvec;
    st_out[bs.idx[m]] = MPSE_OK;
  }
  if (best > 0) ctx->lz_hint[key] = best;
  for (int m = 0; m < B; ++m) {
    if (!single[m]) continue;
    const int i = bs.idx[m];
    ctx->cmask_pending = mpse_ctx::CMask();
    int nv = 0;
    const int st = expm_lanczos_solve(ctx, dtype, &hs[i], dt.real(), dt.imag(), member_ptr(vec(0), m, mstride), outs[i],
                                      rtol, atol, max_dim, &nv, hc[m].bad != 0);
    if (nvec) nvec[i] = nv;
    st_out[i] = st;
    if (st != MPSE_OK) msg[i] = ctx->err;
  }
  return MPSE_OK;
}

}

extern "C" {

int mpse_expm_lanczos_batch(mpse_ctx* ctx, int dtype, int count, const mpse_heff* h, double dt_re, double dt_im,
                            const void* const* C, void* const* out, double rtol, double atol, int max_dim, int* nvec) {
  if (!ctx || count < 0 || (count > 0 && (!h || !C || !out))) return MPSE_ERR_ARG;
  if (MPSE_RECORDING(ctx))
    return mpse_fail(ctx, MPSE_ERR_ARG, "expm_lanczos_batch: cannot be recorded (mpse_defer_begin is open)");
  if (count == 0) return MPSE_OK;
  MPSE_BIND(ctx);
  const int md = (max_dim <= 0 || max_dim > 128) ? 128 : max_dim;
  const bool cplx = dtype == MPSE_C128;
  const mpse_ctx::CMask saved_mask = ctx->cmask_pending;
  std::vector<int> st(count, MPSE_OK);
  std::vector<std::string> msg(count);
  std::vector<char> grouped(count, 0);
  std::vector<BatchSet> sets;
  if (lanczos_async_enabled() && !(!cplx && dt_im != 0.0)) {
    std::vector<BatchSet> open;
    for (int i = 0; i < count; ++i) {
      const mpse_heff& hi = h[i];
      if (!C[i] || !out[i] || !hi.L || !hi.R) continue;
      const mpse_dims& s = hi.dims;
      if ((s.Dl_bra > 0 && s.Dl_bra != s.Dl_ket) || (s.Dr_bra > 0 && s.Dr_bra != s.Dr_ket)) continue;
      int64_t n = s.Dl_ket * s.Dr_ket;
      if (hi.nsite >= 1) n *= s.d0 * (s.danc > 0 ? s.danc : 1);
      if (hi.nsite != 0 && hi.nsite != 1) continue;
      if (n <= 256) continue;
      if (!((cplx || n % 2 == 0) && (reinterpret_cast<uintptr_t>(C[i]) & 15) == 0)) continue;
      {
        const char *c0 = static_cast<const char*>(C[i]), *o0 = static_cast<const char*>(out[i]);
        const size_t bytes = size_t(n) * (cplx ? 16 : 8);
        if (o0 != c0 && o0 < c0 + bytes && c0 < o0 + bytes) continue;
      }
      size_t rtb = 0;
      int np = 0, nbd = 0;
      if (!heff_small_batch_plan(&hi, dtype, n, LZB_DOT_CAP, &rtb, &np, &nbd)) continue;
      BatchSet* tgt = nullptr;
      for (auto& o : open) {
        const mpse_heff& h0 = *o.h0;
        if (h0.nsite == hi.nsite && memcmp(&h0.dims, &hi.dims, sizeof(mpse_dims)) == 0 && h0.l_dtype == hi.l_dtype &&
            h0.r_dtype == hi.r_dtype && h0.w_dtype == hi.w_dtype && (h0.W0 != nullptr) == (hi.W0 != nullptr)) {
          tgt = &o;
          break;
        }
      }
      if (tgt && (int)tgt->idx.size() == LZB_MAX) {
        sets.push_back(*tgt);
        tgt->idx.clear();
      }
      if (!tgt) {
        open.push_back(BatchSet{&hi, {}, n, np, nbd, rtb});
        tgt = &open.back();
      }
      tgt->idx.push_back(i);
    }
    for (auto& o : open) sets.push_back(o);
  }
  for (const BatchSet& bs : sets) {
    if (bs.idx.size() < 2) continue;
    std::vector<char> single(bs.idx.size(), 0);
    MPSE_TRY(expm_lanczos_batch_set(ctx, dtype, bs, h, C, out, std::complex<double>(dt_re, dt_im), rtol, atol, md, nvec,
                                    single, st, msg));
    for (size_t m = 0; m < bs.idx.size(); ++m) {
      grouped[bs.idx[m]] = 1;
      if (single[m])
        ++ctx->lz_batch_single;
      else
        ++ctx->lz_batch_members;
    }
  }
  for (int i = 0; i < count; ++i) {
    if (grouped[i]) continue;
    ++ctx->lz_batch_single;
    ctx->cmask_pending = mpse_ctx::CMask();
    if (!C[i] || !out[i]) {
      st[i] = mpse_fail(ctx, MPSE_ERR_ARG, "expm_lanczos: null vector");
      msg[i] = ctx->err;
      continue;
    }
    int nv = 0;
    st[i] = expm_lanczos_solve(ctx, dtype, &h[i], dt_re, dt_im, C[i], out[i], rtol, atol, max_dim, &nv);
    if (nvec) nvec[i] = nv;
    if (st[i] != MPSE_OK) msg[i] = ctx->err;
  }
  ctx->cmask_pending = saved_mask;
  int status = MPSE_OK;
  for (int i = 0; i < count; ++i)
    if (st[i] != MPSE_OK) {
      status = mpse_fail(ctx, st[i], "expm_lanczos_batch: member %d: %s", i, msg[i].c_str());
      break;
    }
  return defer_replay(ctx, status);
}

int mpse_expm_lanczos_path_stats(mpse_ctx* ctx, int64_t* counts, int n) {
  if (!ctx || n < 0 || (n > 0 && !counts)) return MPSE_ERR_ARG;
  for (int i = 0; i < n && i < mpse_ctx::LP_COUNT; ++i) counts[i] = ctx->lz_paths[i];
  return MPSE_OK;
}

int mpse_expm_lanczos_batch_stats(mpse_ctx* ctx, int64_t* batched_members, int64_t* single_members) {
  if (!ctx) return MPSE_ERR_ARG;
  if (batched_members) *batched_members = ctx->lz_batch_members;
  if (single_members) *single_members = ctx->lz_batch_single;
  return MPSE_OK;
}

}
```

renormalizer_amd/engine.py:

```python
import collections
import ctypes as C
import math
import os
import threading

import numpy as np

_HERE = os.path.dirname(os.path.abspath(__file__))
LIB_PATH = os.environ.get("RENO_MPSENGINE") or os.path.join(_HERE, "csrc", "libmpsengine.so")

F64, C128 = 0, 1
MPSE_OK, MPSE_ERR_OOM, MPSE_ERR_SHAPE, MPSE_ERR_NOCONV, MPSE_ERR_HIP, MPSE_ERR_ARG = 0, 1, 2, 3, 4, 5
DOMAIN_L, DOMAIN_R = 0, 1

STATUS = {0: "OK", 1: "OOM", 2: "SHAPE", 3: "NOCONV", 4: "HIP", 5: "ARG"}


PcgResult = collections.namedtuple("PcgResult", "status iters relres lvalue")


class EngineError(RuntimeError):
    pass


# ... 49 lines not shown
    return mpse_index(int(hi) * int(lo), max(int(lo), 1), int(s_hi), int(s_lo))


def dtype_code(dt):
    dt = np.dtype(dt)
    if dt == np.float64:
        return F64
    if dt == np.complex128:
        return C128
    raise TypeError(f"unsupported dtype {dt}; the engine computes in float64 / complex128")


_i64p = C.POINTER(C.c_int64)
_dblp = C.POINTER(C.c_double)

_SIGNATURES = {
    "mpse_ctx_create": [C.c_int, C.POINTER(C.c_void_p)],
    "mpse_ctx_destroy": [C.c_void_p],
    "mpse_sync": [C.c_void_p],
    "mpse_device_info": [C.c_void_p, C.c_char_p, C.c_size_t, C.POINTER(C.c_int), C.POINTER(C.c_void_p)],
    "mpse_prof_enable": [C.c_void_p, C.c_int],
    "mpse_prof_reset": [C.c_void_p],
    "mpse_prof_get": [C.c_void_p, C.c_int, _dblp, _dblp, _dblp, C.POINTER(C.c_int64)],
    "mpse_prof_get_ktiles": [C.c_void_p, C.c_int, C.POINTER(C.c_int64)],
    "mpse_prof_get_svd_sweeps": [C.c_void_p, C.POINTER(C.c_int64)],
    "mpse_mpo_site_hint": [C.c_void_p, C.c_void_p, C.c_void_p, C.c_int64, C.c_int64, C.c_int64],
    "mpse_block_qr_stats": [C.c_void_p] + [C.POINTER(C.c_int64)] * 3,
    "mpse_heff_fused_stats": [C.c_void_p] + [C.POINTER(C.c_int64)] * 2,
    "mpse_block_qr_optimistic": [C.c_void_p, C.c_int],
    "mpse_block_qr_scheme": [C.c_void_p, C.c_int],
    "mpse_block_qr_check": [C.c_void_p, C.POINTER(C.c_int)],
    "mpse_block_qr_pass_stats": [C.c_void_p] + [C.POINTER(C.c_int64)] * 2,
    "mpse_malloc": [C.c_void_p, C.c_size_t, C.POINTER(C.c_void_p)],
    "mpse_free": [C.c_void_p, C.c_void_p],
    "mpse_pool_trim": [C.c_void_p],
    "mpse_mem_info": [C.c_void_p] + [C.POINTER(C.c_size_t)] * 4,
    "mpse_memcpy_h2d": [C.c_void_p, C.c_void_p, C.c_void_p, C.c_size_t],
    "mpse_memcpy_d2h": [C.c_void_p, C.c_void_p, C.c_void_p, C.c_size_t],
    "mpse_memcpy_d2d": [C.c_void_p, C.c_void_p, C.c_void_p, C.c_size_t],
    "mpse_memset_zero": [C.c_void_p, C.c_void_p, C.c_size_t],
    "mpse_memcpy_2d": [C.c_void_p, C.c_void_p, C.c_size_t, C.c_void_p, C.c_size_t, C.c_size_t, C.c_size_t],
    "mpse_cast_f64_to_c128": [C.c_void_p, C.c_void_p, C.c_void_p, C.c_int64],
    "mpse_conj_inplace": [C.c_void_p, C.c_void_p, C.c_int64],
    "mpse_scal": [C.c_void_p, C.c_int, C.c_void_p, C.c_int64, C.c_double, C.c_double],
    "mpse_axpy": [C.c_void_p, C.c_int, C.c_void_p, C.c_void_p, C.c_int64, C.c_double, C.c_double],
    "mpse_mul_real": [C.c_void_p, C.c_int, C.c_void_p, C.c_void_p, C.c_int64],
    "mpse_davidson_precond": [C.c_void_p, C.c_int, C.c_void_p, C.c_void_p, C.c_void_p, C.c_void_p, C.c_int64,
                              C.c_double, C.c_double],
    "mpse_real_part": [C.c_void_p, C.c_void_p, C.c_void_p, C.c_int64],
    "mpse_dotc": [C.c_void_p, C.c_int, C.c_void_p, C.c_void_p, C.c_int64, _dblp],
    "mpse_nrm2": [C.c_void_p, C.c_int, C.c_void_p, C.c_int64, _dblp],
    "mpse_scaled_rms": [C.c_void_p, C.c_int, C.c_void_p, C.c_void_p, C.c_void_p, C.c_int64, C.c_double, C.c_double, _dblp],
    "mpse_expm_centre_mask": [C.c_void_p, C.c_void_p, C.c_int64],
    "mpse_defer_begin": [C.c_void_p, C.c_int],
    "mpse_defer_end": [C.c_void_p],
    "mpse_defer_arm": [C.c_void_p, C.c_int],
    "mpse_defer_run": [C.c_void_p, C.c_int],
    "mpse_defer_discard": [C.c_void_p],
    "mpse_gemm": [C.c_void_p, C.POINTER(mpse_gemm_desc), C.c_void_p, C.c_void_p, C.c_void_p],
    "mpse_gemm_path_stats": [C.c_void_p, _i64p, C.c_int],
    "mpse_transpose_inner": [C.c_void_p, C.c_int, C.c_void_p, C.c_void_p, C.c_int64, C.c_int64, C.c_int64, C.c_int],
    "mpse_env_update": [C.c_void_p, C.c_int, C.c_int, C.POINTER(mpse_dims), C.c_void_p, C.c_int, C.c_void_p,
                        C.c_void_p, C.c_int, C.c_void_p, C.c_int, C.c_void_p],
    "mpse_heff_apply": [C.c_void_p, C.c_int, C.POINTER(mpse_heff), C.c_void_p, C.c_void_p],
    "mpse_heff_apply2": [C.c_void_p, C.c_int, C.POINTER(mpse_heff), C.c_void_p, C.c_void_p],
    "mpse_env_update_multi": [C.c_void_p, C.c_int, C.c_int, C.POINTER(mpse_dims), C.c_int, _i64p, _i64p, C.c_void_p,
                              C.c_int, C.c_void_p, C.c_void_p, C.c_int, C.POINTER(C.c_void_p), C.c_int, C.c_void_p],
    "mpse_env_unit_channel": [C.c_void_p, C.c_int, C.c_void_p, C.c_int64, C.c_int64, C.c_double, _i64p],
    "mpse_expm_lanczos": [C.c_void_p, C.c_int, C.POINTER(mpse_heff), C.c_double, C.c_double, C.c_void_p, C.c_void_p,
                          C.c_double, C.c_double, C.c_int, C.POINTER(C.c_int)],
    "mpse_expm_lanczos_batch": [C.c_void_p, C.c_int, C.c_int, C.POINTER(mpse_heff), C.c_double, C.c_double,
                                C.POINTER(C.c_void_p), C.POINTER(C.c_void_p), C.c_double, C.c_double, C.c_int,
                                C.POINTER(C.c_int)],
    "mpse_expm_lanczos_batch_stats": [C.c_void_p, _i64p, _i64p],
    "mpse_expm_lanczos_path_stats": [C.c_void_p, _i64p, C.c_int],
    "mpse_davidson": [C.c_void_p, C.c_int, C.POINTER(mpse_heff), C.c_int, C.c_void_p, C.c_void_p, C.c_int, C.c_int,
                      C.c_void_p, C.c_double, C.c_int, C.c_int, C.c_double, C.c_double, _dblp, C.c_void_p,
                      C.POINTER(C.c_int), C.POINTER(C.c_int)],
    "mpse_pcg": [C.c_void_p, C.c_int, C.POINTER(mpse_heff), C.c_int, C.c_double, C.c_void_p, C.c_void_p, C.c_void_p,
                 C.c_void_p, C.c_double, C.c_int, C.POINTER(C.c_int), _dblp, _dblp],
    "mpse_pcg_stats": [C.c_void_p, _i64p, C.c_int],
    "mpse_heff_apply_ft": [C.c_void_p, C.c_int, C.POINTER(mpse_heff_ft), C.c_void_p, C.c_void_p],
    "mpse_env_update_ft": [C.c_void_p, C.c_int, C.c_int, C.POINTER(mpse_heff_ft), C.c_void_p, C.c_int, C.c_void_p,
                           C.c_void_p],
    "mpse_pcg_sum": [C.c_void_p, C.c_int, C.c_int, C.POINTER(mpse_heff_ft), _dblp, C.c_double, C.c_void_p, C.c_void_p,
                     C.c_void_p, C.c_void_p, C.c_double, C.c_int, C.POINTER(C.c_int), _dblp, _dblp],
    "mpse_pcg_sum_stats": [C.c_void_p, _i64p, C.c_int],
    "mpse_site_factor_ft": [C.c_void_p, C.POINTER(mpse_heff_ft), C.c_void_p],
    "mpse_diag_ft": [C.c_void_p, C.POINTER(mpse_heff_ft), C.c_void_p, C.c_double, C.c_double, C.c_int, C.c_void_p],
    "mpse_truncate_select": [_dblp, _i64p, C.c_int64, C.c_int64, C.c_double, _i64p, _i64p],
    "mpse_block_qr": [C.c_void_p, C.c_int, C.c_void_p, C.c_int64, C.c_int64, C.c_int, _i64p, _i64p, _i64p, _i64p,
                      C.c_int, C.c_void_p, C.c_void_p, C.c_int64],
    "mpse_block_svd": [C.c_void_p, C.c_int, C.c_void_p, C.c_int64, C.c_int64, C.c_int, _i64p, _i64p, _i64p, _i64p,
                       C.c_void_p, C.c_void_p, _dblp, C.c_int64],
    "mpse_block_svd_full": [C.c_void_p, C.c_int, C.c_void_p, C.c_int64, C.c_int64, C.c_int, _i64p, _i64p, _i64p, _i64p,
                            _i64p, C.c_void_p, C.c_int64, C.c_void_p, C.c_int64, _dblp, C.c_int64],
    "mpse_gather_cols": [C.c_void_p, C.c_int, C.c_void_p, C.c_void_p, C.c_int64, C.c_int64, _i64p, _dblp, C.c_int64],
    "mpse_gather_rows": [C.c_void_p, C.c_int, C.c_void_p, C.c_void_p, C.c_int64, _i64p, _dblp, C.c_int64],
}
EXPORTED_SYMBOLS = sorted(list(_SIGNATURES) + ["mpse_last_error", "mpse_version"])


def load_library(path=LIB_PATH):
    if not os.path.exists(path):
        raise EngineError(
            f"{path} not found: build it with `python -c 'import __graft_entry__ as g; g.build()'` "
# ... 317 lines not shown
        self._check(self.lib.mpse_heff_apply_ft(self.ctx, c.code, C.byref(term), c.ptr, out.ptr))
        return out

    def env_update_ft(self, term, domain, env, x):
        left = domain == "L"
        oshape = (term.Dr, term.wr1, term.wr2, term.Dr) if left else (term.Dl, term.wl1, term.wl2, term.Dl)
        dt = np.complex128 if (x.is_complex or env.is_complex) else np.float64
        assert x.dtype == dt, "the site must have the working dtype"
        out = self.empty(oshape, dt)
        self._check(self.lib.mpse_env_update_ft(self.ctx, x.code, DOMAIN_L if left else DOMAIN_R, C.byref(term),
                                                env.ptr, env.code, x.ptr, out.ptr))
        return out

    def site_factor_ft(self, term):
        s = self.empty((term.wl1, term.wl2, term.d_up, term.d_down, term.wr1, term.wr2), np.float64)
        self._check(self.lib.mpse_site_factor_ft(self.ctx, C.byref(term), s.ptr))
        return s

    def diag_ft_sum(self, terms, factors, weights, shift):
        t0 = terms[0]
        diag = self.empty((t0.Dl, t0.d_up, t0.d_down, t0.Dr), np.float64)
        for k, (t, s, w) in enumerate(zip(terms, factors, weights)):
            self._check(self.lib.mpse_diag_ft(self.ctx, C.byref(t), s.ptr, float(w), float(shift), int(k > 0), diag.ptr))
        return diag

    PCG_SUM_STATS = ("solves", "iterations", "term_applies", "host_waits", "diagonals")

    def pcg_sum_stats(self):
        v = (C.c_int64 * len(self.PCG_SUM_STATS))()
        self._check(self.lib.mpse_pcg_sum_stats(self.ctx, v, len(v)))
        return dict(zip(self.PCG_SUM_STATS, (int(x) for x in v)))

    def pcg_sum(self, terms, weights, b, x, diag=None, mask=None, shift=0.0, tol=1e-5, max_iter=0, check=True):
        nt = len(terms)
        arr = (mpse_heff_ft * nt)(*terms)
        w = (C.c_double * nt)(*[float(v) for v in weights])
        n = x.size
        assert b.size == n and b.dtype == x.dtype
        assert diag is None or (diag.size == n and diag.dtype == np.float64)
        assert mask is None or (mask.size == n and mask.dtype == np.float64)
        it, rel, lv = C.c_int(0), C.c_double(0.0), C.c_double(0.0)
        st = self.lib.mpse_pcg_sum(self.ctx, x.code, nt, arr, w, float(shift), None if diag is None else diag.ptr,
                                   None if mask is None else mask.ptr, b.ptr, x.ptr, float(tol), int(max_iter),
                                   C.byref(it), C.byref(rel), C.byref(lv))
        if check and st not in (0, 3):
            self._check(st)
        return PcgResult(int(st), it.value, rel.value, lv.value)

    def block_qr_stats(self):
        a, b, c = C.c_int64(), C.c_int64(), C.c_int64()
        self._check(self.lib.mpse_block_qr_stats(self.ctx, C.byref(a), C.byref(b), C.byref(c)))
        return a.value, b.value, c.value

    def heff_fused_stats(self):
        a, b = C.c_int64(), C.c_int64()
        self._check(self.lib.mpse_heff_fused_stats(self.ctx, C.byref(a), C.byref(b)))
        return a.value, b.value

    GEMM_PATHS = ("launches", "general", "eight_wave", "split_b1", "split_batched", "die_group1", "die_group2", "skew",
                  "tile_order", "masks", "masks_global", "grouped", "grouped_split2")

    def gemm_path_stats(self):
        v = (C.c_int64 * len(self.GEMM_PATHS))()
        self._check(self.lib.mpse_gemm_path_stats(self.ctx, v, len(v)))
        return dict(zip(self.GEMM_PATHS, (int(x) for x in v)))

    def block_qr_optimistic(self, on):
        self._check(self.lib.mpse_block_qr_optimistic(self.ctx, int(bool(on))))

    def block_qr_scheme(self, scheme):
        self._check(self.lib.mpse_block_qr_scheme(self.ctx, int(scheme)))

    def block_qr_check(self):
        v = C.c_int(0)
        self._check(self.lib.mpse_block_qr_check(self.ctx, C.byref(v)))
        return bool(v.value)

    def block_qr_pass_stats(self):
        a, b = C.c_int64(0), C.c_int64(0)
        self._check(self.lib.mpse_block_qr_pass_stats(self.ctx, C.byref(a), C.byref(b)))
        return a.value, b.value

    def prof_get(self):
        names = {0: "f64xf64", 1: "c128xf64", 2: "f64xc128", 3: "c128xc128", 4: "lanczos_vec", 5: "block_qr", 6: "block_svd",
                 7: "heff_fused"}
        issued_per_mac = {0: 2.0, 1: 4.0, 2: 4.0, 3: 6.0}
        out = {}
        for v, nm in names.items():
            ms, fl, by, n = C.c_double(), C.c_double(), C.c_double(), C.c_int64()
            self._check(self.lib.mpse_prof_get(self.ctx, v, C.byref(ms), C.byref(fl), C.byref(by), C.byref(n)))
            out[nm] = dict(ms=ms.value, flops=fl.value, bytes=by.value, launches=n.value)
            if v < 4:
                kt = C.c_int64()
                self._check(self.lib.mpse_prof_get_ktiles(self.ctx, v, C.byref(kt)))
                out[nm]["ktiles"] = kt.value
                out[nm]["issued_flops"] = kt.value * 65536.0 * issued_per_mac[v]
        sw = C.c_int64()
        self._check(self.lib.mpse_prof_get_svd_sweeps(self.ctx, C.byref(sw)))
        out["block_svd"]["sweeps"] = sw.value
        return out

    def empty(self, shape, dtype=np.float64):
        if isinstance(shape, (int, np.integer)):
            shape = (shape,)
        dtype = np.dtype(dtype)
        dtype_code(dtype)
# ... 93 lines not shown
```

renormalizer_amd/lib/krylov.py:

```python
import ctypes as C

import numpy as np
import scipy.linalg

from ..engine import get_engine
from ..mps.hop_expr import Hop


def expm_krylov(Afunc, dt, vstart, block_size=50, rtol=1e-5, atol=1e-8, out=None):
    eng = get_engine()
    dt = complex(dt)
    v = eng.asdevice(vstart)
    if isinstance(Afunc, Hop):
        if (dt.imag != 0 or Afunc.operator_is_complex) and not v.is_complex:
            v = v.to_complex()
        if out is None:
            out = eng.empty(v.shape, v.dtype)
        elif out.size != v.size or out.dtype != v.dtype:
            raise ValueError("expm_krylov: out does not match the start vector")
        nv = C.c_int()
        if Afunc.cmask is not None:
            eng._check(eng.lib.mpse_expm_centre_mask(eng.ctx, Afunc.cmask.ptr, Afunc.cmask.nbytes))
        eng._check(eng.lib.mpse_expm_lanczos(eng.ctx, v.code, C.byref(Afunc.heff), dt.real, dt.imag, v.ptr, out.ptr,
                                             rtol, atol, 0, C.byref(nv)))
        return out, nv.value
    return _expm_krylov_generic(eng, Afunc, dt, v, block_size, rtol, atol)


def expm_krylov_batch(hops, dt, vstarts, rtol=1e-5, atol=1e-8, outs=None):
    eng = get_engine()
    dt = complex(dt)
    hops, vstarts = list(hops), list(vstarts)
    if len(hops) != len(vstarts) or (outs is not None and len(outs) != len(hops)):
        raise ValueError("expm_krylov_batch: hops, vstarts and outs differ in length")
    res, dims = [None] * len(hops), [0] * len(hops)
    eng_idx, heffs, vs, os_ = [], [], [], []
    code = None
    for i, (h, v0) in enumerate(zip(hops, vstarts)):
        out = None if outs is None else outs[i]
        if not isinstance(h, Hop):
            res[i], dims[i] = expm_krylov(h, dt, v0, rtol=rtol, atol=atol)
            continue
        v = eng.asdevice(v0)
        if (dt.imag != 0 or h.operator_is_complex) and not v.is_complex:
            v = v.to_complex()
        if out is None:
            out = eng.empty(v.shape, v.dtype)
        elif out.size != v.size or out.dtype != v.dtype:
            raise ValueError("expm_krylov_batch: out does not match the start vector")
        if (code is not None and v.code != code) or h.cmask is not None:
            res[i], dims[i] = expm_krylov(h, dt, v, rtol=rtol, atol=atol, out=out)
            continue
        code = v.code
        eng_idx.append(i)
        heffs.append(h.heff)
        vs.append(v)
        os_.append(out)
        res[i] = out
    if eng_idx:
        cnt = len(eng_idx)
        harr = (type(heffs[0]) * cnt)(*heffs)
        carr = (C.c_void_p * cnt)(*[v.ptr for v in vs])
        oarr = (C.c_void_p * cnt)(*[o.ptr for o in os_])
        nv = (C.c_int * cnt)()
        eng._check(eng.lib.mpse_expm_lanczos_batch(eng.ctx, code, cnt, harr, dt.real, dt.imag, carr, oarr, rtol, atol,
                                                   0, nv))
        for k, i in enumerate(eng_idx):
            dims[i] = nv[k]
    return res, dims


def _combine(eng, V, coef, dtype):
    out = eng.zeros(V[0].shape, dtype)
    for c, vec in zip(coef, V):
        c = complex(c)
# ... 38 lines not shown
```

renormalizer_amd/mps/hop_expr.py:

```python
import ctypes as C

import numpy as np

from ..engine import DeviceTensor, get_engine, mpse_heff


class Hop:
    def __init__(self, ltensor, rtensor, cmo, cshape, twolayer=False):
        self.eng = get_engine()
        self.twolayer = bool(twolayer)
        eng = self.eng
        nsite = len(cmo)
        cshape = tuple(int(s) for s in cshape)
        ancilla = (nsite > 0) and (2 * nsite + 2 == len(cshape))
        if not ancilla:
            assert nsite + 2 == len(cshape)
        self.nsite = nsite
        self.cshape = cshape
        self.cmask = None
        self.l = eng.asdevice(ltensor)
        self.r = eng.asdevice(rtensor)
        if self.twolayer:
            assert nsite in (1, 2) and self.l.ndim == 4 and self.r.ndim == 4
            assert self.l.shape[1] == self.l.shape[2] and self.r.shape[1] == self.r.shape[2]
        self.cmo = [eng.asdevice(w) for w in cmo]
        if nsite == 1 and isinstance(cmo[0], np.ndarray):
            eng.mpo_site_hint(self.cmo[0], cmo[0])
        if nsite == 2 and self.cmo[0].is_complex != self.cmo[1].is_complex:
            self.cmo = [w.to_complex() for w in self.cmo]
        h = mpse_heff()
        h.nsite = nsite
        d = h.dims
        d.Dl_ket, d.Dr_ket = cshape[0], cshape[-1]
        d.Dl_bra, d.Dr_bra = self.l.shape[0], self.r.shape[0]
        assert self.l.shape[-1] == cshape[0] and self.r.shape[-1] == cshape[-1], (self.l.shape, self.r.shape, cshape)
        self.oshape = (self.l.shape[0],) + cshape[1:-1] + (self.r.shape[0],)
        self.square = self.oshape == cshape
        d.danc = cshape[2] if ancilla else 1
        d.danc1 = cshape[4] if (ancilla and nsite == 2) else 0
        d.wl, d.wr = self.l.shape[1], self.r.shape[1]
        d.d0 = self.cmo[0].shape[1] if nsite >= 1 else 1
        d.d1 = self.cmo[1].shape[1] if nsite == 2 else 1
        d.wm = self.cmo[0].shape[3] if nsite == 2 else 1
        h.L, h.l_dtype, h.R, h.r_dtype = self.l.ptr, self.l.code, self.r.ptr, self.r.code
        h.l_unit, h.r_unit = self.l.unit, self.r.unit
        if nsite >= 1:
            h.W0, h.w_dtype = self.cmo[0].ptr, self.cmo[0].code
        if nsite == 2:
            h.W1 = self.cmo[1].ptr
        self.heff = h
        self.operator_is_complex = self.l.is_complex or self.r.is_complex or any(w.is_complex for w in self.cmo)

    def __call__(self, c: DeviceTensor) -> DeviceTensor:
        eng = self.eng
        c = eng.asdevice(c)
        if self.operator_is_complex and not c.is_complex:
            c = c.to_complex()
        c = c.reshape(self.cshape)
        out = eng.empty(self.oshape, c.dtype)
        apply = eng.lib.mpse_heff_apply2 if self.twolayer else eng.lib.mpse_heff_apply
        eng._check(apply(eng.ctx, c.code, C.byref(self.heff), c.ptr, out.ptr))
        return out

    def dense(self):
        assert self.square and (self.heff.dims.danc == 1 or self.nsite == 0)
        eng = self.eng
        n = int(np.prod(self.cshape))
        dt = np.complex128 if self.operator_is_complex else np.float64
        eye = np.eye(n, dtype=dt).reshape(self.cshape + self.cshape)
        nd = len(self.cshape)
        x = np.moveaxis(eye.reshape(self.cshape + (n,)), -1, nd - 1)
        h = mpse_heff()
        C.memmove(C.byref(h), C.byref(self.heff), C.sizeof(mpse_heff))
        if self.nsite == 1:
            h.dims.danc = n
        else:
            h.dims.danc, h.dims.danc1 = 1, n
        xin = eng.asdevice(np.ascontiguousarray(x))
        out = eng.empty(xin.shape, dt)
        apply = eng.lib.mpse_heff_apply2 if self.twolayer else eng.lib.mpse_heff_apply
        eng._check(apply(eng.ctx, xin.code, C.byref(h), xin.ptr, out.ptr))
        res = np.moveaxis(out.to_host(), nd - 1, -1)
        return res.reshape(n, n)


def hop_expr(ltensor, rtensor, cmo, cshape, twolayer: bool = False):
    return Hop(ltensor, rtensor, list(cmo), cshape, twolayer)


_CMASK_CACHE = {}


def centre_tile_mask(eng, qnbigl, qnbigr, qntot, cshape):
    Dl, Dr = int(cshape[0]), int(cshape[-1])
    inner = int(np.prod(cshape[1:-1]))
    ql = np.ascontiguousarray(np.asarray(qnbigl).reshape(-1, np.asarray(qnbigl).shape[-1]))
    qr = np.ascontiguousarray(np.asarray(qnbigr).reshape(-1, np.asarray(qnbigr).shape[-1]))
    qt = np.asarray(qntot).reshape(-1)
    if ql.shape[0] != Dl * inner or qr.shape[0] != Dr:
        return None
    key = (id(eng), Dl, inner, Dr, ql.tobytes(), qr.tobytes(), qt.tobytes())
    hit = _CMASK_CACHE.get(key)
    if hit is not None:
        return hit
    ul, il = np.unique(ql, axis=0, return_inverse=True)
    ur, ir = np.unique(qr, axis=0, return_inverse=True)
    ok = (ul[:, None, :] + ur[None, :, :] == qt).all(-1)
    allowed = ok[np.asarray(il).reshape(-1)][:, np.asarray(ir).reshape(-1)]
    n = inner * Dr
    view = allowed.reshape(Dl, n)
    nkt, ntn = (Dl + 15) // 16, (n + 63) // 64
    pad = np.zeros((nkt * 16, ntn * 64), dtype=bool)
    pad[:Dl, :n] = view
    flags = pad.reshape(nkt, 16, ntn, 64).any(axis=(1, 3))
    nkw = (nkt + 7) // 8
    out = np.zeros((ntn, nkw * 8), dtype=np.uint8)
    out[:, :nkt] = flags.T
    dev = eng.asdevice(out.view(np.float64).reshape(-1))
    if len(_CMASK_CACHE) > 4096:
        _CMASK_CACHE.clear()
    _CMASK_CACHE[key] = dev
    return dev
```

renormalizer_amd/mps/mps.py:

```python
import ctypes
import logging
import os
import threading
from typing import Dict, List

import numpy as np

from ..engine import DeviceTensor, EngineError, get_engine
from ..lib.krylov import expm_krylov
from ..model import Model, Op, OpSum
from ..utils import CompressConfig, CompressCriteria, EvolveConfig, EvolveMethod, OptimizeConfig
from . import svd_qn
from .hop_expr import centre_tile_mask, hop_expr
from . import lib as _lib
from .lib import Environ, contract_one_site
from .mpo import Mpo
from .svd_qn import add_outer, get_qn_mask

logger = logging.getLogger("renormalizer_amd")


def _vn_entropy(p):
    p = np.asarray(p, dtype=float)
    assert np.allclose(p[p < 0], 0)
    p = p / p.sum()
    p = p[p > 0]
    return float(-(p * np.log(p)).sum())


def _is_identity_site(w):
    w = np.asarray(w)
    return w.shape[0] == 1 and w.shape[3] == 1 and np.array_equal(w[0, :, :, 0], np.eye(w.shape[1]))


class Mps:
    def __init__(self):
        self._mp: List[DeviceTensor] = []
        self.dtype = np.dtype(np.float64)
        self.model: Model = None
        self.compress_config: CompressConfig = CompressConfig()
        self.evolve_config: EvolveConfig = EvolveConfig()
        self.optimize_config: OptimizeConfig = OptimizeConfig()
        self.qn: List[np.ndarray] = []
        self.qnidx: int = None
        self.qntot: np.ndarray = None
        self.to_right: bool = None
        self.coeff = 1.0

    @classmethod
    def from_arrays(cls, model, arrays, qn, qnidx, qntot, to_right, coeff=1.0):
        eng = get_engine()
        mps = cls()
        mps.model = model
        cplx = any(np.iscomplexobj(a) for a in arrays)
        mps.dtype = np.dtype(np.complex128 if cplx else np.float64)
        mps._mp = [eng.asdevice(np.asarray(a), mps.dtype) for a in arrays]
        q = len(np.atleast_1d(qntot))
        mps.qn = [np.asarray(x, dtype=int).reshape(-1, q) for x in qn]
        mps.qnidx = int(qnidx)
        mps.qntot = np.asarray(qntot, dtype=int).reshape(q)
        mps.to_right = bool(to_right)
        mps.coeff = coeff
        return mps

    @classmethod
    def random(cls, model, qntot, m_max, percent=1.0, rng=None) -> "Mps":
# ... 1153 lines not shown
                        local_steps.append(j)
                        centre = mps[nbr] = absorb(b_t.reshape(bond.shape), nbr)
                        continue
                    out, hop_b, bond, nbr = after_site
                    eng.arm(0)
                    _, j = expm_krylov(hop, -1j * evolve_dt / 2, centre, out=out)
                    local_steps.append(j)
                    note_qr(imps)
                    b_out = eng.empty(bond.shape, bond.dtype)
                    with eng.recording(1):
                        new_centre = absorb(b_out, nbr)
                    mps[nbr] = new_centre
                    ready = prepare(nbr, list(new_centre.shape))
                    after_site = None
                    if ready[1]:
                        out = eng.empty(new_centre.shape, new_centre.dtype)
                        with eng.recording(0):
                            after_site = (out,) + split_site(nbr, out, ready, list(new_centre.shape))
                    eng.arm(1)
                    _, j = expm_krylov(hop_b, 1j * evolve_dt / 2, bond, out=b_out)
                    local_steps.append(j)
                    centre = new_centre
                mps._switch_direction()
        except BaseException:
            eng.defer_discard()
            raise
        return sw.finish()


class _PsSweep:

    def __init__(self, src, mpo, evolve_dt, learn_qr=False, carry=None):
        eng = get_engine()
        self.eng, self.mpo, self.learn_qr = eng, mpo, learn_qr
        self.carry = _CARRY if carry is None else carry
        if np.iscomplex(evolve_dt):
            mps = src.copy()
        else:
            mps = src.to_complex()
        self.evolve_dt = complex(evolve_dt)
        self.mps = mps
        self.n = len(mps)
        ahead = "R" if mps.to_right else "L"
        environ = _carried_environ(mps, mpo, ahead, self.carry)
        if environ is None:
            environ = Environ(mps, mpo, ahead)
        self.environ = environ
        self.local_steps = []
        self.q = len(mps.qntot)
        self.hh_sites = _householder_sites(mps)
        self.hh_sites.tick()
        self.qr_redone = eng.block_qr_stats()[2]
        self.use_cmask = os.environ.get("MPSE_CENTRE_MASK", "1") != "0"

    def note_qr(self, imps):
        if self.learn_qr:
            now = self.eng.block_qr_stats()[2]
            if now != self.qr_redone:
                self.hh_sites.note((imps, self.mps.to_right))
            self.qr_redone = now

    def prepare(self, imps, shape):
        mps, eng, n = self.mps, self.eng, self.n
        hop = hop_expr(self.environ.read("L", imps - 1), self.environ.read("R", imps + 1), [self.mpo.device(imps, eng)],
                       shape)
        split = (not mps.to_right and imps != 0) or (mps.to_right and imps != n - 1)
        qnbigl = qnbigr = plan = None
        if split:
            qnbigl, qnbigr, _ = mps._get_big_qn([imps], need_mat=False)
            plan = svd_qn.block_plan(qnbigl, qnbigr, mps.qntot)
            if self.use_cmask and len(shape) == 3 and shape[0] * shape[0] * shape[1] * shape[2] >= (1 << 22):
                if mps.to_right:
                    ql, qr = qnbigl, qnbigr
                else:
                    ql = add_outer(np.array(mps.qn[imps]), mps._get_sigmaqn(imps))
                    qr = np.array(mps.qn[imps + 1])
                hop.cmask = centre_tile_mask(eng, ql, qr, mps.qntot, shape)
        return hop, split, qnbigl, qnbigr, plan

    def split_site(self, imps, centre, ready, shape):
        mps, eng, mpo, environ, q = self.mps, self.eng, self.mpo, self.environ, self.q
        hop, _, qnbigl, qnbigr, plan = ready
        l_array, r_array = hop.l, hop.r
        u, qnlset, v, qnrset = svd_qn.svd_qn(centre, qnbigl, qnbigr, mps.qntot, QR=True,
                                             system="L" if mps.to_right else "R", full_matrices=False, plan=plan,
                                             householder=(imps, mps.to_right) in self.hh_sites)
        vt = v.T
        if not mps.to_right:
            mps[imps] = vt.reshape([-1] + shape[1:])
            mps.qn[imps] = np.array(qnrset, dtype=int).reshape(-1, q)
            mps.qnidx = imps - 1
            r_array = environ.GetLR("R", imps, mps, mpo, itensor=r_array, method="System", canonical=True)
            hop_b = hop_expr(l_array, r_array, [], u.shape)
            if self.use_cmask and u.shape[0] * u.shape[1] >= (1 << 14):
                hop_b.cmask = centre_tile_mask(eng, qnbigl, np.array(qnrset, dtype=int).reshape(-1, q), mps.qntot,
                                               u.shape)
            return hop_b, u, imps - 1
        mps[imps] = u.reshape(shape[:-1] + [-1])
        mps.qn[imps + 1] = np.array(qnlset, dtype=int).reshape(-1, q)
        mps.qnidx = imps + 1
        l_array = environ.GetLR("L", imps, mps, mpo, itensor=l_array, method="System", canonical=True)
        hop_b = hop_expr(l_array, r_array, [], vt.shape)
        if self.use_cmask and vt.shape[0] * vt.shape[1] >= (1 << 14):
            hop_b.cmask = centre_tile_mask(eng, np.array(qnlset, dtype=int).reshape(-1, q), qnbigr, mps.qntot,
                                           vt.shape)
        return hop_b, vt, imps + 1

    def absorb(self, bond, nbr):
        mps, eng = self.mps, self.eng
        t = mps[nbr]
        if mps.to_right:
            return eng.matmul(bond, t.reshape(t.shape[0], -1)).reshape((bond.shape[0],) + t.shape[1:])
        return eng.matmul(t.reshape(-1, t.shape[-1]), bond).reshape(t.shape[:-1] + (bond.shape[1],))

    def finish(self):
        mps, local_steps = self.mps, self.local_steps
        mps.evolve_config.stat = dict(nobs=len(local_steps), min=int(np.min(local_steps)),
                                      max=int(np.max(local_steps)), mean=float(np.mean(local_steps)),
                                      steps=list(local_steps))
        _carry_environ(mps, self.mpo, self.environ, self.carry)
        return mps


_OPTIMISTIC_REDONE = [0]



class _QrNotes:
    FIRST = 8

    def __init__(self):
        self.d = {}

    def copy(self):
        new = _QrNotes()
        new.d = {k: list(v) for k, v in self.d.items()}
        return new

    def __contains__(self, key):
        e = self.d.get(key)
        return e is not None and e[0] > 0

    def note(self, key):
        e = self.d.get(key)
        patience = min(2 * e[1], 1 << 20) if e else self.FIRST
        self.d[key] = [patience, patience]

    def tick(self):
        for e in self.d.values():
            if e[0] > 0:
                e[0] -= 1


def _householder_sites(mps):
    notes = mps.__dict__.get("_qr_notes")
# ... 295 lines not shown
```

Measured before the change: 584.7.

## Derive environment tile masks from quantum-number structure and persist tile plans

Adds environment structure handles built from quantum numbers, so tile occupancy masks for the L/R environments come from symmetry rather than from scanning the environment tensors on device. Tile-ordering plans (GEMM permutations and the heff0 F0 plans) are kept in a persistent plan cache keyed on those structural masks and released when the owning buffers are freed. The aim is to drop repeated occupancy scans and plan-building kernel launches inside each Lanczos solve. In exchange it adds host-side key building, cache bookkeeping, and the risk that a structural mask misses nonzero tiles; an optional check mode compares it against a real scan.

Result: faster. 596.5 (median of 4 runs) (+2.0%).

```diff
diff --git a/include/mpsengine.h b/include/mpsengine.h
--- a/include/mpsengine.h
+++ b/include/mpsengine.h
@@ -154,6 +154,13 @@
 
 int mpse_expm_centre_mask(mpse_ctx* ctx, const void* mask_dev, int64_t nbytes);
 
+int mpse_env_structure_create(mpse_ctx* ctx, int nq, int64_t n_row, const int64_t* qrow, int64_t n_chan,
+                              const int64_t* qchan, int64_t n_col, const int64_t* qcol, int sign_chan,
+                              const int64_t* qoff, uint64_t* handle);
+int mpse_env_structure_free(mpse_ctx* ctx, uint64_t handle);
+int mpse_expm_env_structure(mpse_ctx* ctx, uint64_t handle_l, uint64_t handle_r);
+int mpse_env_structure_stats(mpse_ctx* ctx, int64_t* out, int n);
+
 int mpse_expm_lanczos(mpse_ctx* ctx, int dtype, const mpse_heff* h, double dt_re, double dt_im,
                       const void* C, void* out, double rtol, double atol, int max_dim, int* nvec);
 int mpse_expm_lanczos_batch(mpse_ctx* ctx, int dtype, int count, const mpse_heff* h, double dt_re, double dt_im,
diff --git a/renormalizer_amd/csrc/mpse_contract.hip b/renormalizer_amd/csrc/mpse_contract.hip
--- a/renormalizer_amd/csrc/mpse_contract.hip
+++ b/renormalizer_amd/csrc/mpse_contract.hip
@@ -344,18 +344,20 @@
       gd.ngrp = (int)s.groups.size();
       TmpBuf MA(ctx), MB(ctx);
       const unsigned char *fa = nullptr, *fb = nullptr;
-      bool stable = true;
+      bool stable = true, structural = true;
       if (s.scan_a.on && bufs[s.scan_a.buf]) {
         bool st = false;
         MPSE_TRY(occ_mask_get(ctx, sc, (const char*)bufs[s.scan_a.buf] + size_t(s.scan_a.off) * dtype_size(s.scan_a.dt),
-                              s.scan_a.dt, s.scan_a.r, s.scan_a.k, MA, &fa, &gd.am_pitch, &st));
+                              s.scan_a.dt, s.scan_a.r, s.scan_a.k, MA, &fa, &gd.am_pitch, &st, &gd.owner[0]));
         stable = stable && st;
+        structural = structural && gd.owner[0] != 0;
       }
       if (s.scan_b.on && bufs[s.scan_b.buf]) {
         bool st = false;
         MPSE_TRY(occ_mask_get(ctx, sc, (const char*)bufs[s.scan_b.buf] + size_t(s.scan_b.off) * dtype_size(s.scan_b.dt),
-                              s.scan_b.dt, s.scan_b.r, s.scan_b.k, MB, &fb, &gd.bm_pitch, &st));
+                              s.scan_b.dt, s.scan_b.r, s.scan_b.k, MB, &fb, &gd.bm_pitch, &st, &gd.owner[1]));
         stable = stable && st;
+        structural = structural && gd.owner[1] != 0;
       }
       const unsigned char* cm = nullptr;
       int cm_pitch = 0;
@@ -386,10 +388,12 @@
           } else if (sg.bm_kind == BM_CENTRE && cm) {
             o.seg[q].bm = cm;
             gd.bm_pitch = cm_pitch;
+            gd.foreign = cm;
           }
         }
       }
       gd.masks_stable = stable;
+      gd.persistent = stable && structural && (gd.owner[0] || gd.owner[1]);
       if (gd.ngrp == 1 && s.groups[0].split2) {
         if (!bufs[B_OUT2]) return mpse_fail(ctx, MPSE_ERR_ARG, "plan: missing second result");
         gd.split2 = true;
diff --git a/renormalizer_amd/csrc/mpse_core.hip b/renormalizer_amd/csrc/mpse_core.hip
--- a/renormalizer_amd/csrc/mpse_core.hip
+++ b/renormalizer_amd/csrc/mpse_core.hip
@@ -378,6 +378,11 @@
 int mpse_free(mpse_ctx* ctx, void* dptr) {
   if (!ctx) return MPSE_ERR_ARG;
   if (!dptr) return MPSE_OK;
+  {
+    std::vector<void*> release;
+    plan_cache_collect_ptr(ctx, dptr, &release);
+    for (void* p : release) mpse_free(ctx, p);
+  }
   std::lock_guard<std::mutex> lock(ctx->pool_mu);
   auto it = ctx->live.find(dptr);
   if (it == ctx->live.end()) return mpse_fail(ctx, MPSE_ERR_ARG, "mpse_free: unknown pointer %p", dptr);
diff --git a/renormalizer_amd/csrc/mpse_gemm.hip b/renormalizer_amd/csrc/mpse_gemm.hip
--- a/renormalizer_amd/csrc/mpse_gemm.hip
+++ b/renormalizer_amd/csrc/mpse_gemm.hip
@@ -1209,6 +1209,8 @@
       &rec);
   g.kt_counter = prof_this && ctx->prof_ktiles ? ctx->prof_ktiles + variant : nullptr;
   bool mask_a_stable = true, mask_b_stable = true;
+  uint64_t own_a = 0, own_b = 0;
+  const void* foreign = nullptr;
   if (skip_zero && is_single(g.kA) && is_single(g.kB) && nkt_all >= 2 && d->batch <= 16384) {
     g.nkw = (nkt_all + 7) / 8;
     const size_t wa = size_t(d->batch) * g.mtiles_m * g.nkw, wb = size_t(d->batch) * g.mtiles_n * g.nkw;
@@ -1231,7 +1233,18 @@
     unsigned long long *am = nullptr, *bmk = nullptr;
     bool scan_a = sa, scan_b = sb_, b_structural = false;
     mpse_ctx::OccKey ka, kb;
-    const bool ca_ok = sa && cacheable(g.A), cb_ok = sb_ && cacheable(g.B);
+    bool ca_ok = sa && cacheable(g.A), cb_ok = sb_ && cacheable(g.B);
+    const unsigned char *st_a = nullptr, *st_b = nullptr;
+    auto es_lay = [&](const IdxMap& rm, const IdxMap& km, long long sb, int nrows, int tiles, int cplx) {
+      return EsLayout{rm.ext, rm.lo, rm.s_hi, rm.s_lo, km.ext, km.lo, km.s_hi, km.s_lo, sb, nrows, tiles, g.nkw,
+                      (int)d->batch, g.K, cplx};
+    };
+    if (ca_ok) MPSE_TRY(env_structure_mask(ctx, sc, g.A, es_lay(g.mA, g.kA, g.sbA, g.M, g.mtiles_m, ca ? 1 : 0), &st_a, &own_a));
+    if (cb_ok) MPSE_TRY(env_structure_mask(ctx, sc, g.B, es_lay(g.nB, g.kB, g.sbB, g.N, g.mtiles_n, cb ? 1 : 0), &st_b, &own_b));
+    const bool es_chk = env_structure_check();
+    const bool stable_a = ca_ok, stable_b = cb_ok;
+    if (st_a) ca_ok = false, scan_a = es_chk;
+    if (st_b) cb_ok = false, scan_b = es_chk;
     if (ca_ok) {
       ka = make_key(g.A, g.mA, g.kA, g.sbA, g.M, g.mtiles_m, ca ? 1 : 0);
       if (void* hit = find(ka)) am = static_cast<unsigned long long*>(hit), scan_a = false;
@@ -1246,8 +1259,8 @@
       scan_b = false;
       b_structural = true;
     }
-    mask_a_stable = !sa || ca_ok;
-    mask_b_stable = !sb_ || cb_ok || b_structural;
+    mask_a_stable = !sa || stable_a;
+    mask_b_stable = !sb_ || stable_b || b_structural;
     size_t tmp_words = 0;
     if (scan_a && !ca_ok) tmp_words += wa;
     if (scan_b && !cb_ok) tmp_words += wb;
@@ -1280,7 +1293,19 @@
       const int tmax = (scan_a ? g.mtiles_m : 0) > (scan_b ? g.mtiles_n : 0) ? (scan_a ? g.mtiles_m : 0) : (scan_b ? g.mtiles_n : 0);
       const dim3 og((nkt_all + 3) / 4, tmax, (unsigned)(2 * d->batch));
       hipLaunchKernelGGL(k_tile_occ, og, dim3(256), 0, ctx->stream, oa, ob, g.K, g.nkw, (int)d->batch, skip);
-    }
+      if (sc && ((scan_a && stable_a) || (scan_b && stable_b))) ++ctx->es_stats[mpse_ctx::ES_SCANS];
+    }
+    if (st_a) {
+      if (scan_a)
+        MPSE_TRY(env_structure_compare(ctx, reinterpret_cast<const unsigned char*>(am), st_a, (int)(d->batch * g.mtiles_m), g.nkw * 8, nkt_all, 1, skip));
+      am = reinterpret_cast<unsigned long long*>(const_cast<unsigned char*>(st_a));
+    }
+    if (st_b) {
+      if (scan_b)
+        MPSE_TRY(env_structure_compare(ctx, reinterpret_cast<const unsigned char*>(bmk), st_b, (int)(d->batch * g.mtiles_n), g.nkw * 8, nkt_all, 2, skip));
+      bmk = reinterpret_cast<unsigned long long*>(const_cast<unsigned char*>(st_b));
+    }
+    if (b_structural) foreign = sc->cmask.ptr;
     g.amask = sa ? am : nullptr;
     g.bmask = sb_ ? bmk : nullptr;
   }
@@ -1288,13 +1313,23 @@
   const long long ntile_all = (long long)g.tiles_m * g.tiles_n;
   if (d->batch == 1 && (g.amask || g.bmask) && ntile_all * g.ksplit > 2 * n_cu && ntile_all <= 2048) {
     const bool keep = sc && sc->occ_cache && mask_a_stable && mask_b_stable;
+    const bool persist = keep && (own_a || own_b) && (!g.amask || own_a) && (!g.bmask || own_b || foreign);
     int* pp = nullptr;
-    if (keep)
+    std::vector<unsigned char> pkey;
+    if (persist) {
+      key_put(pkey, g.amask), key_put(pkey, g.bmask), key_put(pkey, g.tiles_m), key_put(pkey, g.tiles_n);
+      key_put(pkey, nkt_all), key_put(pkey, g.nkw);
+      pp = static_cast<int*>(plan_cache_find(ctx, 0, pkey));
+    } else if (keep)
       for (const auto& e : ctx->perm_cache)
         if (e.amask == g.amask && e.bmask == g.bmask && e.tiles_m == g.tiles_m && e.tiles_n == g.tiles_n && e.nkt == nkt_all)
           pp = static_cast<int*>(e.perm);
     if (!pp) {
-      if (keep) {
+      if (persist) {
+        void* pm = nullptr;
+        MPSE_TRY(plan_cache_insert(ctx, 0, pkey, own_a, own_b, foreign, size_t(ntile_all) * sizeof(int), &pm));
+        pp = static_cast<int*>(pm);
+      } else if (keep) {
         void* pm = nullptr;
         MPSE_TRY(mpse_malloc(ctx, size_t(ntile_all) * sizeof(int), &pm));
         ctx->perm_cache.push_back({g.amask, g.bmask, g.tiles_m, g.tiles_n, nkt_all, pm});
@@ -1304,7 +1339,8 @@
         pp = PERM.as<int>();
       }
       hipLaunchKernelGGL(k_tile_order, dim3(1), dim3(1024), 0, ctx->stream, g.amask, g.bmask, g.nkw, nkt_all, g.tiles_m,
-                         g.tiles_n, 1, pp, skip, GemmGroups(), (unsigned char*)nullptr, 0);
+                         g.tiles_n, 1, pp, persist ? nullptr : skip, GemmGroups(), (unsigned char*)nullptr, 0);
+      if (keep) ++ctx->es_stats[mpse_ctx::ES_PLAN_LAUNCHES];
     }
     g.perm = pp;
   }
@@ -1374,7 +1410,7 @@
 }
 
 int occ_mask_get(mpse_ctx* ctx, const SolveScope* sc, const void* ptr, int dtype, mpse_index r, mpse_index k,
-                 TmpBuf& tmp, const unsigned char** flags, int* pitch, bool* stable) {
+                 TmpBuf& tmp, const unsigned char** flags, int* pitch, bool* stable, uint64_t* owner) {
   IdxMap rm, km;
   if (!to_map(r, &rm) || !to_map(k, &km) || !is_single(km))
     return mpse_fail(ctx, MPSE_ERR_SHAPE, "occupancy scan: K index must be single level");
@@ -1391,7 +1427,17 @@
   const bool cacheable = sc && sc->in_env(ptr);
   *pitch = nkw * 8;
   *stable = cacheable;
-  if (cacheable)
+  if (owner) *owner = 0;
+  const unsigned char* st = nullptr;
+  if (cacheable && owner) {
+    const EsLayout lay{rm.ext, rm.lo, rm.s_hi, rm.s_lo, km.ext, km.lo, km.s_hi, km.s_lo, 0, nrows, tiles, nkw, 1, K, cplx ? 1 : 0};
+    MPSE_TRY(env_structure_mask(ctx, sc, ptr, lay, &st, owner));
+    if (st && !env_structure_check()) {
+      *flags = st;
+      return MPSE_OK;
+    }
+  }
+  if (cacheable && !st)
     for (const auto& e : ctx->occ_cache)
       if (memcmp(&e.key, &key, sizeof(key)) == 0) {
         *flags = static_cast<const unsigned char*>(e.mask);
@@ -1399,7 +1445,7 @@
       }
   void* pm = nullptr;
   const size_t bytes = size_t(tiles) * nkw * 8;
-  if (cacheable) {
+  if (cacheable && !st) {
     MPSE_TRY(mpse_malloc(ctx, bytes, &pm));
     ctx->occ_cache.push_back({key, pm});
   } else {
@@ -1412,6 +1458,12 @@
   hipLaunchKernelGGL(k_tile_occ, dim3((nkt + 3) / 4, tiles, 2), dim3(256), 0, ctx->stream, oa, ob, K, nkw, 1,
                      sc ? sc->skip : nullptr);
   MPSE_HIP(ctx, hipGetLastError());
+  if (cacheable) ++ctx->es_stats[mpse_ctx::ES_SCANS];
+  if (st) {
+    MPSE_TRY(env_structure_compare(ctx, static_cast<const unsigned char*>(pm), st, tiles, nkw * 8, nkt, 4, sc ? sc->skip : nullptr));
+    *flags = st;
+    return MPSE_OK;
+  }
   *flags = static_cast<const unsigned char*>(pm);
   return MPSE_OK;
 }
@@ -1506,13 +1558,27 @@
     const void *ka = gg.g[0].seg[0].am, *kb = gg.g[0].seg[0].bm;
     const int nkt_key = nkt_max + 1000 * d.ngrp;
     const bool keep = sc && sc->occ_cache && d.masks_stable;
-    if (keep)
+    const bool persist = keep && d.persistent;
+    std::vector<unsigned char> pkey;
+    if (persist) {
+      key_put(pkey, d.ngrp), key_put(pkey, g.tiles_m), key_put(pkey, g.tiles_n), key_put(pkey, gg.nkt_seg);
+      key_put(pkey, gg.am_pitch), key_put(pkey, gg.bm_pitch), key_put(pkey, gg.split2), key_put(pkey, g.nkw);
+      for (int i = 0; i < d.ngrp; ++i) {
+        key_put(pkey, gg.g[i].nseg);
+        for (int q = 0; q < gg.g[i].nseg; ++q) key_put(pkey, gg.g[i].seg[q].am), key_put(pkey, gg.g[i].seg[q].bm);
+      }
+      pp = static_cast<int*>(plan_cache_find(ctx, 1, pkey));
+    } else if (keep)
       for (const auto& e : ctx->perm_cache)
         if (e.amask == ka && e.bmask == kb && e.tiles_m == g.tiles_m && e.tiles_n == g.tiles_n && e.nkt == nkt_key)
           pp = static_cast<int*>(e.perm);
     const size_t perm_bytes = (size_t(ntile) * sizeof(int) + 7) & ~size_t(7), flag_pitch = size_t(g.nkw) * 8;
     if (!pp) {
-      if (keep) {
+      if (persist) {
+        void* pm = nullptr;
+        MPSE_TRY(plan_cache_insert(ctx, 1, pkey, d.owner[0], d.owner[1], d.foreign, perm_bytes + size_t(ntile) * flag_pitch, &pm));
+        pp = static_cast<int*>(pm);
+      } else if (keep) {
         void* pm = nullptr;
         MPSE_TRY(mpse_malloc(ctx, perm_bytes + size_t(ntile) * flag_pitch, &pm));
         ctx->perm_cache.push_back({ka, kb, g.tiles_m, g.tiles_n, nkt_key, pm});
@@ -1523,7 +1589,8 @@
       }
       hipLaunchKernelGGL(k_tile_order, dim3(1), dim3(1024), 0, ctx->stream, (const unsigned long long*)nullptr,
                          (const unsigned long long*)nullptr, 0, nkt_max, g.tiles_m, g.tiles_n, d.split2 ? 0 : 1, pp,
-                         g.skip, gg, reinterpret_cast<unsigned char*>(pp) + perm_bytes, (int)flag_pitch);
+                         persist ? nullptr : g.skip, gg, reinterpret_cast<unsigned char*>(pp) + perm_bytes, (int)flag_pitch);
+      if (keep) ++ctx->es_stats[mpse_ctx::ES_PLAN_LAUNCHES];
     }
     g.perm = pp;
     g.gg.flags = reinterpret_cast<const unsigned long long*>(reinterpret_cast<const char*>(pp) + perm_bytes);
diff --git a/renormalizer_amd/csrc/mpse_heff0.hip b/renormalizer_amd/csrc/mpse_heff0.hip
--- a/renormalizer_amd/csrc/mpse_heff0.hip
+++ b/renormalizer_amd/csrc/mpse_heff0.hip
@@ -88,6 +88,12 @@
   f0_transpose(rt, R, Dr, wr, blk, (int)gridDim.x - ntl * wl - ntr * wr);
 }
 
+__global__ __launch_bounds__(256) void k_f0_transpose(const double2* __restrict__ R, double2* __restrict__ rt, int Dr, int wr,
+                                                       const int* __restrict__ skip) {
+  if (skip && *skip) return;
+  f0_transpose(rt, R, Dr, wr, (int)blockIdx.x, (int)gridDim.x);
+}
+
 __global__ __launch_bounds__(1024) void k_f0_valid(const unsigned char* __restrict__ FL, const unsigned char* __restrict__ FC,
                                                     const unsigned char* __restrict__ FR, const F0Term* __restrict__ terms,
                                                     const int* __restrict__ nterm, int wl, int wr, int d, int ntl, int ntr,
@@ -606,52 +612,107 @@
     const char* e = getenv("MPSE_F0_ORDER");
     return !(e && e[0] == '0');
   }();
+  const unsigned char *sFL = nullptr, *sFR = nullptr;
+  uint64_t own_l = 0, own_r = 0;
+  MPSE_TRY(env_structure_f0_flags(ctx, sc, 0, &sFL, &own_l));
+  MPSE_TRY(env_structure_f0_flags(ctx, sc, 1, &sFR, &own_r));
+  const bool structural = sFL && sFR;
+  const bool es_chk = structural && env_structure_check();
+  const int n_cu = ctx->n_cu > 0 ? ctx->n_cu : 256;
+  const char* plan = nullptr;
+  if (structural) {
+    std::vector<unsigned char> pkey;
+    key_put(pkey, sFL), key_put(pkey, sFR), key_put(pkey, FC), key_put(pkey, fc_pitch), key_put(pkey, wl), key_put(pkey, wr);
+    key_put(pkey, d), key_put(pkey, ntl), key_put(pkey, ntr), key_put(pkey, nkc), key_put(pkey, n_cu);
+    key_put(pkey, (int)compact), key_put(pkey, (int)order_on);
+    for (int f = 0; f < wr; ++f) {
+      key_put(pkey, nterm[f]);
+      for (int q = 0; q < nterm[f]; ++q) {
+        const F0Term& tm = terms[size_t(f) * F0_TMAX + q];
+        key_put(pkey, tm.b), key_put(pkey, tm.e), key_put(pkey, tm.x), key_put(pkey, tm.w);
+      }
+    }
+    plan = static_cast<const char*>(plan_cache_find(ctx, 2, pkey));
+    if (!plan) {
+      void* pp = nullptr;
+      MPSE_TRY(plan_cache_insert(ctx, 2, pkey, own_l, own_r, FC, tot_bytes - o_tm, &pp));
+      char* pb = static_cast<char*>(pp);
+      std::vector<char> up(tm_bytes + nt_bytes, 0);
+      memcpy(up.data(), terms.data(), tm_bytes);
+      memcpy(up.data() + tm_bytes, nterm.data(), size_t(wr) * sizeof(int));
+      MPSE_TRY(stage_h2d(ctx, pb, up.data(), up.size()));
+      if (order_on)
+        hipLaunchKernelGGL(k_f0_plan, dim3(1), dim3(1024), 0, ctx->stream, sFL, FC, sFR, reinterpret_cast<const F0Term*>(pb),
+                           reinterpret_cast<const int*>(pb + (o_nt - o_tm)), wl, wr, d, ntl, ntr, nkc, fc_pitch,
+                           reinterpret_cast<unsigned long long*>(pb + (o_mk - o_tm)), n_cu,
+                           reinterpret_cast<F0Info*>(pb + (o_od - o_tm)), compact ? 1 : 0, (const int*)nullptr);
+      else
+        hipLaunchKernelGGL(k_f0_valid, dim3(1), dim3(1024), 0, ctx->stream, sFL, FC, sFR, reinterpret_cast<const F0Term*>(pb),
+                           reinterpret_cast<const int*>(pb + (o_nt - o_tm)), wl, wr, d, ntl, ntr, nkc, fc_pitch,
+                           reinterpret_cast<unsigned long long*>(pb + (o_mk - o_tm)), (const int*)nullptr);
+      ++ctx->es_stats[mpse_ctx::ES_PLAN_LAUNCHES];
+      plan = pb;
+    }
+  }
   if (hit) {
     base = static_cast<char*>(fc.buf);
   } else {
     void* p = nullptr;
     heff0_drop_cache(ctx);
-    MPSE_TRY(mpse_malloc(ctx, tot_bytes, &p));
+    MPSE_TRY(mpse_malloc(ctx, (structural && !es_chk) ? rt_bytes : tot_bytes, &p));
     fc.buf = p, fc.L = h->L, fc.R = h->R, fc.W = h->W0, fc.cmask = FC, fc.Dl = Dl, fc.Dr = Dr, fc.w = wr, fc.nsite = h->nsite;
     base = static_cast<char*>(p);
-    {
-      std::vector<char> up(tm_bytes + nt_bytes, 0);
-      memcpy(up.data(), terms.data(), tm_bytes);
-      memcpy(up.data() + tm_bytes, nterm.data(), size_t(wr) * sizeof(int));
-      MPSE_TRY(stage_h2d(ctx, base + o_tm, up.data(), up.size()));
-    }
     const long long nel = (long long)wr * Dr * Dr;
     int nb = (int)((nel + 255) / 256);
     if (nb > 2048) nb = 2048;
-    hipLaunchKernelGGL(k_f0_prepare, dim3(ntl * wl + ntr * wr + nb), dim3(256), 0, ctx->stream,
-                       static_cast<const double2*>(h->L), static_cast<const double2*>(h->R), reinterpret_cast<double2*>(base),
-                       reinterpret_cast<unsigned char*>(base + o_fl), reinterpret_cast<unsigned char*>(base + o_fr), Dl, Dr, wl,
-                       wr, ntl, ntr, skip);
-    if (order_on)
-      hipLaunchKernelGGL(k_f0_plan, dim3(1), dim3(1024), 0, ctx->stream, reinterpret_cast<const unsigned char*>(base + o_fl), FC,
-                         reinterpret_cast<const unsigned char*>(base + o_fr), reinterpret_cast<const F0Term*>(base + o_tm),
-                         reinterpret_cast<const int*>(base + o_nt), wl, wr, d, ntl, ntr, nkc, fc_pitch,
-                         reinterpret_cast<unsigned long long*>(base + o_mk), ctx->n_cu > 0 ? ctx->n_cu : 256,
-                         reinterpret_cast<F0Info*>(base + o_od), compact ? 1 : 0, skip);
-    else
-      hipLaunchKernelGGL(k_f0_valid, dim3(1), dim3(1024), 0, ctx->stream, reinterpret_cast<const unsigned char*>(base + o_fl), FC,
-                         reinterpret_cast<const unsigned char*>(base + o_fr), reinterpret_cast<const F0Term*>(base + o_tm),
-                         reinterpret_cast<const int*>(base + o_nt), wl, wr, d, ntl, ntr, nkc, fc_pitch,
-                         reinterpret_cast<unsigned long long*>(base + o_mk), skip);
-  }
+    if (structural && !es_chk) {
+      hipLaunchKernelGGL(k_f0_transpose, dim3(nb), dim3(256), 0, ctx->stream, static_cast<const double2*>(h->R),
+                         reinterpret_cast<double2*>(base), Dr, wr, skip);
+    } else {
+      if (!structural) {
+        std::vector<char> up(tm_bytes + nt_bytes, 0);
+        memcpy(up.data(), terms.data(), tm_bytes);
+        memcpy(up.data() + tm_bytes, nterm.data(), size_t(wr) * sizeof(int));
+        MPSE_TRY(stage_h2d(ctx, base + o_tm, up.data(), up.size()));
+      }
+      hipLaunchKernelGGL(k_f0_prepare, dim3(ntl * wl + ntr * wr + nb), dim3(256), 0, ctx->stream,
+                         static_cast<const double2*>(h->L), static_cast<const double2*>(h->R), reinterpret_cast<double2*>(base),
+                         reinterpret_cast<unsigned char*>(base + o_fl), reinterpret_cast<unsigned char*>(base + o_fr), Dl, Dr, wl,
+                         wr, ntl, ntr, skip);
+      ++ctx->es_stats[mpse_ctx::ES_SCANS];
+    }
+    if (es_chk) {
+      MPSE_TRY(env_structure_compare(ctx, reinterpret_cast<const unsigned char*>(base + o_fl), sFL, ntl * wl, ntl, ntl, 8, skip));
+      MPSE_TRY(env_structure_compare(ctx, reinterpret_cast<const unsigned char*>(base + o_fr), sFR, ntr * wr, ntr, ntr, 16, skip));
+    } else if (!structural) {
+      if (order_on)
+        hipLaunchKernelGGL(k_f0_plan, dim3(1), dim3(1024), 0, ctx->stream, reinterpret_cast<const unsigned char*>(base + o_fl), FC,
+                           reinterpret_cast<const unsigned char*>(base + o_fr), reinterpret_cast<const F0Term*>(base + o_tm),
+                           reinterpret_cast<const int*>(base + o_nt), wl, wr, d, ntl, ntr, nkc, fc_pitch,
+                           reinterpret_cast<unsigned long long*>(base + o_mk), n_cu,
+                           reinterpret_cast<F0Info*>(base + o_od), compact ? 1 : 0, skip);
+      else
+        hipLaunchKernelGGL(k_f0_valid, dim3(1), dim3(1024), 0, ctx->stream, reinterpret_cast<const unsigned char*>(base + o_fl), FC,
+                           reinterpret_cast<const unsigned char*>(base + o_fr), reinterpret_cast<const F0Term*>(base + o_tm),
+                           reinterpret_cast<const int*>(base + o_nt), wl, wr, d, ntl, ntr, nkc, fc_pitch,
+                           reinterpret_cast<unsigned long long*>(base + o_mk), skip);
+      ++ctx->es_stats[mpse_ctx::ES_PLAN_LAUNCHES];
+    }
+  }
+  const char* tb = structural ? plan - o_tm : base;
   F0Args g{};
   g.L = static_cast<const double*>(h->L);
   g.Rt = reinterpret_cast<const double*>(base);
   g.C = static_cast<const double*>(C);
   g.parts = static_cast<double*>(pr.ptr);
-  g.FL = reinterpret_cast<const unsigned char*>(base + o_fl);
+  g.FL = structural ? sFL : reinterpret_cast<const unsigned char*>(base + o_fl);
   g.FC = FC;
-  g.FR = reinterpret_cast<const unsigned char*>(base + o_fr);
-  g.terms = reinterpret_cast<const F0Term*>(base + o_tm);
-  g.nterm = reinterpret_cast<const int*>(base + o_nt);
-  g.mask = reinterpret_cast<const unsigned long long*>(base + o_mk);
+  g.FR = structural ? sFR : reinterpret_cast<const unsigned char*>(base + o_fr);
+  g.terms = reinterpret_cast<const F0Term*>(tb + o_tm);
+  g.nterm = reinterpret_cast<const int*>(tb + o_nt);
+  g.mask = reinterpret_cast<const unsigned long long*>(tb + o_mk);
   g.skip = skip;
-  g.info = order_on ? reinterpret_cast<const F0Info*>(base + o_od) : nullptr;
+  g.info = order_on ? reinterpret_cast<const F0Info*>(tb + o_od) : nullptr;
   g.trace = ctx->prof_on ? ctx->gemm_trace : nullptr;
   g.n = n;
   g.Dl = Dl, g.Dr = Dr, g.wl = wl, g.wr = wr, g.d = d, g.ntl = ntl, g.ntr = ntr, g.nkc = nkc, g.fc_pitch = fc_pitch;
diff --git a/renormalizer_amd/csrc/mpse_internal.h b/renormalizer_amd/csrc/mpse_internal.h
--- a/renormalizer_amd/csrc/mpse_internal.h
+++ b/renormalizer_amd/csrc/mpse_internal.h
@@ -123,6 +123,26 @@
   long long pcg_stats[PS_COUNT] = {0};
   enum PcgSumStat { PSS_SOLVES, PSS_ITERS, PSS_TERM_APPLIES, PSS_WAITS, PSS_DIAGS, PSS_COUNT };
   long long pcg_sum_stats[PSS_COUNT] = {0};
+  struct EnvStruct;
+  struct PlanEntry {
+    int kind = 0;
+    std::vector<unsigned char> key;
+    uint64_t owner[2] = {0, 0};
+    const void* foreign = nullptr;
+    void* dev = nullptr;
+    unsigned long long tick = 0;
+  };
+  static constexpr size_t PLAN_CACHE_CAP = 1024;
+  std::mutex plan_mu;
+  std::unordered_map<uint64_t, std::shared_ptr<EnvStruct>> env_structs;
+  uint64_t env_struct_next = 1;
+  uint64_t env_struct_pending[2] = {0, 0};
+  std::vector<PlanEntry> plan_cache;
+  unsigned long long plan_tick = 0;
+  enum EsStat { ES_ALIVE, ES_MASKS, ES_PLAN_BUILDS, ES_PLAN_HITS, ES_SCANS, ES_PLAN_LAUNCHES, ES_VIOLATIONS, ES_COUNT };
+  long long es_stats[ES_COUNT] = {0};
+  int* es_check_word = nullptr;
+  bool es_check_used = false;
 };
 int qr_words(mpse_ctx* ctx);
 
@@ -213,6 +233,7 @@
   const char* env_lo[2] = {nullptr, nullptr};
   const char* env_hi[2] = {nullptr, nullptr};
   mpse_ctx::CMask cmask;
+  mpse_ctx::EnvStruct* es[2] = {nullptr, nullptr};
   const char* krylov_lo = nullptr;
   const char* krylov_hi = nullptr;
 
@@ -319,12 +340,38 @@
   GroupedGrp grp[8];
   int am_pitch = 0, bm_pitch = 0;
   bool masks_stable = false;
+  bool persistent = false;
+  uint64_t owner[2] = {0, 0};
+  const void* foreign = nullptr;
   bool split2 = false;
   void* c2 = nullptr;
 };
 int gemm_grouped(mpse_ctx* ctx, const GroupedDesc& d, const SolveScope* sc, MatvecReq::Dot* dot);
 int occ_mask_get(mpse_ctx* ctx, const SolveScope* sc, const void* ptr, int dtype, mpse_index r, mpse_index k,
-                 TmpBuf& tmp, const unsigned char** flags, int* pitch, bool* stable);
+                 TmpBuf& tmp, const unsigned char** flags, int* pitch, bool* stable, uint64_t* owner = nullptr);
+
+bool env_structure_enabled();
+bool env_structure_check();
+void env_structure_take(mpse_ctx* ctx, SolveScope* sc, const mpse_heff* h);
+struct EsLayout {
+  long long r_ext, r_lo, r_shi, r_slo, k_ext, k_lo, k_shi, k_slo, sb;
+  int nrows, tiles, nkw, batch, K, cplx;
+};
+int env_structure_mask(mpse_ctx* ctx, const SolveScope* sc, const void* ptr, const EsLayout& lay,
+                       const unsigned char** flags, uint64_t* owner);
+int env_structure_f0_flags(mpse_ctx* ctx, const SolveScope* sc, int side, const unsigned char** flags, uint64_t* owner);
+int env_structure_compare(mpse_ctx* ctx, const unsigned char* scanned, const unsigned char* structural, int rows,
+                          int pitch, int nvalid, int code, const int* skip);
+int env_structure_solve_end(mpse_ctx* ctx, int status);
+void* plan_cache_find(mpse_ctx* ctx, int kind, const std::vector<unsigned char>& key);
+int plan_cache_insert(mpse_ctx* ctx, int kind, const std::vector<unsigned char>& key, uint64_t owner0, uint64_t owner1,
+                      const void* foreign, size_t bytes, void** dev);
+void plan_cache_collect_ptr(mpse_ctx* ctx, const void* freed, std::vector<void*>* release);
+template <class T>
+inline void key_put(std::vector<unsigned char>& k, const T& v) {
+  const unsigned char* p = reinterpret_cast<const unsigned char*>(&v);
+  k.insert(k.end(), p, p + sizeof(T));
+}
 
 int publish_and_wait(mpse_ctx* ctx, const double* dsrc, int count, int slot);
 int publish_wait_seq(mpse_ctx* ctx, double seq, const double* dsrc, int count, int slot);
diff --git a/renormalizer_amd/csrc/mpse_structure.h b/renormalizer_amd/csrc/mpse_structure.h
--- /dev/null
+++ b/renormalizer_amd/csrc/mpse_structure.h
@@ -0,0 +1,106 @@
+#pragma once
+#include <cstdint>
+#include <cstring>
+#include <map>
+#include <vector>
+
+namespace mpse_structure {
+
+struct EnvStructure {
+  int nq = 0, n_row = 0, n_chan = 0, n_col = 0;
+  std::vector<int> rcls, bcls, ccls;
+  int nr = 0, nb = 0, nc = 0;
+  std::vector<unsigned char> ok;
+  bool allowed(int r, int b, int c) const { return ok[(size_t(rcls[r]) * nb + bcls[b]) * nc + ccls[c]] != 0; }
+};
+
+inline void classify(int nq, int n, const int64_t* q, std::vector<int>* cls, std::vector<std::vector<int64_t>>* vals) {
+  std::map<std::vector<int64_t>, int> seen;
+  cls->resize(n);
+  for (int i = 0; i < n; ++i) {
+    std::vector<int64_t> v(q + size_t(i) * nq, q + size_t(i + 1) * nq);
+    auto it = seen.find(v);
+    if (it == seen.end()) {
+      it = seen.emplace(v, (int)vals->size()).first;
+      vals->push_back(v);
+    }
+    (*cls)[i] = it->second;
+  }
+}
+
+inline EnvStructure build(int nq, int n_row, const int64_t* qrow, int n_chan, const int64_t* qchan, int n_col,
+                          const int64_t* qcol, int sign_chan, const int64_t* qoff) {
+  EnvStructure s;
+  s.nq = nq, s.n_row = n_row, s.n_chan = n_chan, s.n_col = n_col;
+  std::vector<std::vector<int64_t>> vr, vb, vc;
+  classify(nq, n_row, qrow, &s.rcls, &vr);
+  classify(nq, n_chan, qchan, &s.bcls, &vb);
+  classify(nq, n_col, qcol, &s.ccls, &vc);
+  s.nr = (int)vr.size(), s.nb = (int)vb.size(), s.nc = (int)vc.size();
+  s.ok.assign(size_t(s.nr) * s.nb * s.nc, 0);
+  for (int r = 0; r < s.nr; ++r)
+    for (int b = 0; b < s.nb; ++b)
+      for (int c = 0; c < s.nc; ++c) {
+        bool eq = true;
+        for (int k = 0; k < nq; ++k)
+          eq = eq && vr[r][k] == vc[c][k] + sign_chan * vb[b][k] + (qoff ? qoff[k] : 0);
+        s.ok[(size_t(r) * s.nb + b) * s.nc + c] = eq ? 1 : 0;
+      }
+  return s;
+}
+
+struct Map {
+  long long ext = 0, lo = 1, s_hi = 0, s_lo = 0;
+  long long off(long long i) const { return lo >= ext ? i * s_lo : (i / lo) * s_hi + (i % lo) * s_lo; }
+};
+
+struct MaskLayout {
+  long long base = 0, sb = 0;
+  Map r, k;
+  int nrows = 0, tiles = 0, nkw = 0, batch = 1, K = 0;
+  bool operator==(const MaskLayout& o) const {
+    return base == o.base && sb == o.sb && r.ext == o.r.ext && r.lo == o.r.lo && r.s_hi == o.r.s_hi && r.s_lo == o.r.s_lo &&
+           k.ext == o.k.ext && k.lo == o.k.lo && k.s_hi == o.k.s_hi && k.s_lo == o.k.s_lo && nrows == o.nrows &&
+           tiles == o.tiles && nkw == o.nkw && batch == o.batch && K == o.K;
+  }
+};
+
+inline bool tile_flags(const EnvStructure& s, const MaskLayout& m, std::vector<unsigned char>* out) {
+  const long long pitch = (long long)m.nkw * 8, wc = (long long)s.n_chan * s.n_col, total = (long long)s.n_row * wc;
+  const int nkt = (m.K + 15) / 16;
+  if (m.tiles != (m.nrows + 63) / 64 || nkt > pitch || m.batch < 1) return false;
+  out->assign(size_t(m.batch) * m.tiles * pitch, 0);
+  std::vector<long long> koff(m.K);
+  for (int k = 0; k < m.K; ++k) koff[k] = m.k.off(k);
+  for (int b = 0; b < m.batch; ++b)
+    for (int i = 0; i < m.nrows; ++i) {
+      const long long ro = m.base + (long long)b * m.sb + m.r.off(i);
+      unsigned char* frow = out->data() + (size_t(b) * m.tiles + i / 64) * pitch;
+      for (int k = 0; k < m.K; ++k) {
+        if (frow[k / 16]) {
+          k |= 15;
+          continue;
+        }
+        const long long e = ro + koff[k];
+        if (e < 0 || e >= total) return false;
+        const int r = (int)(e / wc), bc = (int)(e % wc);
+        if (s.allowed(r, bc / s.n_col, bc % s.n_col)) frow[k / 16] = 1;
+      }
+    }
+  return true;
+}
+
+inline void f0_flags(const EnvStructure& s, std::vector<unsigned char>* out) {
+  const int ntr = (s.n_row + 15) / 16, ntc = (s.n_col + 15) / 16;
+  out->assign(size_t(ntr) * s.n_chan * ntc, 0);
+  for (int rt = 0; rt < ntr; ++rt)
+    for (int b = 0; b < s.n_chan; ++b)
+      for (int ct = 0; ct < ntc; ++ct) {
+        bool any = false;
+        for (int r = 16 * rt; r < 16 * rt + 16 && r < s.n_row && !any; ++r)
+          for (int c = 16 * ct; c < 16 * ct + 16 && c < s.n_col && !any; ++c) any = s.allowed(r, b, c);
+        (*out)[(size_t(rt) * s.n_chan + b) * ntc + ct] = any ? 1 : 0;
+      }
+}
+
+}
diff --git a/renormalizer_amd/csrc/mpse_structure.hip b/renormalizer_amd/csrc/mpse_structure.hip
--- /dev/null
+++ b/renormalizer_amd/csrc/mpse_structure.hip
@@ -0,0 +1,278 @@
+#include "mpse_internal.h"
+#include "mpse_structure.h"
+
+struct mpse_ctx::EnvStruct {
+  uint64_t id = 0;
+  mpse_structure::EnvStructure s;
+  struct Mask {
+    mpse_structure::MaskLayout lay;
+    void* dev;
+  };
+  std::vector<Mask> masks;
+  void* f0 = nullptr;
+};
+
+namespace {
+
+__global__ __launch_bounds__(256) void k_flags_compare(const unsigned char* __restrict__ scanned,
+                                                        const unsigned char* __restrict__ structural, int rows, int pitch,
+                                                        int nvalid, int* __restrict__ word, int code,
+                                                        const int* __restrict__ skip) {
+  if (skip && *skip) return;
+  const long long i = (long long)blockIdx.x * 256 + threadIdx.x;
+  if (i >= (long long)rows * nvalid) return;
+  const long long o = (i / nvalid) * pitch + i % nvalid;
+  if (scanned[o] && !structural[o]) atomicOr(word, code);
+}
+
+int env_flag(const char* name, int dflt) {
+  const char* e = getenv(name);
+  return e ? atoi(e) : dflt;
+}
+
+void struct_release(mpse_ctx* ctx, mpse_ctx::EnvStruct& e) {
+  for (auto& m : e.masks) mpse_free(ctx, m.dev);
+  e.masks.clear();
+  if (e.f0) mpse_free(ctx, e.f0);
+  e.f0 = nullptr;
+}
+
+}
+
+bool env_structure_enabled() {
+  static const bool on = env_flag("MPSE_ENV_STRUCTURE", 1) != 0;
+  return on;
+}
+bool env_structure_check() {
+  static const bool on = env_flag("MPSE_ENV_STRUCTURE_CHECK", 0) != 0;
+  return on;
+}
+
+void env_structure_take(mpse_ctx* ctx, SolveScope* sc, const mpse_heff* h) {
+  uint64_t ids[2];
+  {
+    std::lock_guard<std::mutex> lock(ctx->plan_mu);
+    ids[0] = ctx->env_struct_pending[0], ids[1] = ctx->env_struct_pending[1];
+    if (!env_structure_enabled() || !h) return;
+    const mpse_dims& d = h->dims;
+    const int64_t rows[2] = {d.Dl_bra > 0 ? d.Dl_bra : d.Dl_ket, d.Dr_bra > 0 ? d.Dr_bra : d.Dr_ket};
+    const int64_t chan[2] = {d.wl, d.wr}, cols[2] = {d.Dl_ket, d.Dr_ket};
+    for (int side = 0; side < 2; ++side) {
+      if (!ids[side]) continue;
+      auto it = ctx->env_structs.find(ids[side]);
+      if (it == ctx->env_structs.end()) continue;
+      const mpse_structure::EnvStructure& s = it->second->s;
+      if (s.n_row == rows[side] && s.n_chan == chan[side] && s.n_col == cols[side]) sc->es[side] = it->second.get();
+    }
+  }
+  if (env_structure_check() && (sc->es[0] || sc->es[1])) ctx->es_check_used = true;
+}
+
+int env_structure_mask(mpse_ctx* ctx, const SolveScope* sc, const void* ptr, const EsLayout& lay,
+                       const unsigned char** flags, uint64_t* owner) {
+  *flags = nullptr;
+  *owner = 0;
+  if (!sc || !sc->occ_cache || lay.batch < 1) return MPSE_OK;
+  const char* p = static_cast<const char*>(ptr);
+  int side = -1;
+  for (int i = 0; i < 2; ++i)
+    if (sc->es[i] && p >= sc->env_lo[i] && p < sc->env_hi[i]) side = i;
+  if (side < 0) return MPSE_OK;
+  mpse_ctx::EnvStruct& e = *sc->es[side];
+  const long long esz = lay.cplx ? 16 : 8, boff = p - sc->env_lo[side];
+  const long long total = (long long)e.s.n_row * e.s.n_chan * e.s.n_col;
+  if (boff % esz || (sc->env_hi[side] - sc->env_lo[side]) != total * esz) return MPSE_OK;
+  mpse_structure::MaskLayout m;
+  m.base = boff / esz, m.sb = lay.sb;
+  m.r.ext = lay.r_ext, m.r.lo = lay.r_lo, m.r.s_hi = lay.r_shi, m.r.s_lo = lay.r_slo;
+  m.k.ext = lay.k_ext, m.k.lo = lay.k_lo, m.k.s_hi = lay.k_shi, m.k.s_lo = lay.k_slo;
+  m.nrows = lay.nrows, m.tiles = lay.tiles, m.nkw = lay.nkw, m.batch = lay.batch, m.K = lay.K;
+  for (const auto& have : e.masks)
+    if (have.lay == m) {
+      *flags = static_cast<const unsigned char*>(have.dev);
+      *owner = e.id;
+      return MPSE_OK;
+    }
+  std::vector<unsigned char> host;
+  if (!mpse_structure::tile_flags(e.s, m, &host)) return MPSE_OK;
+  void* dev = nullptr;
+  MPSE_TRY(mpse_malloc(ctx, host.size() ? host.size() : 16, &dev));
+  const int st = stage_h2d(ctx, dev, host.data(), host.size());
+  if (st != MPSE_OK) {
+    mpse_free(ctx, dev);
+    return st;
+  }
+  e.masks.push_back({m, dev});
+  ++ctx->es_stats[mpse_ctx::ES_MASKS];
+  *flags = static_cast<const unsigned char*>(dev);
+  *owner = e.id;
+  return MPSE_OK;
+}
+
+int env_structure_f0_flags(mpse_ctx* ctx, const SolveScope* sc, int side, const unsigned char** flags, uint64_t* owner) {
+  *flags = nullptr;
+  *owner = 0;
+  if (!sc || !sc->es[side]) return MPSE_OK;
+  mpse_ctx::EnvStruct& e = *sc->es[side];
+  if (!e.f0) {
+    std::vector<unsigned char> host;
+    mpse_structure::f0_flags(e.s, &host);
+    void* dev = nullptr;
+    MPSE_TRY(mpse_malloc(ctx, host.size() ? host.size() : 16, &dev));
+    const int st = stage_h2d(ctx, dev, host.data(), host.size());
+    if (st != MPSE_OK) {
+      mpse_free(ctx, dev);
+      return st;
+    }
+    e.f0 = dev;
+    ++ctx->es_stats[mpse_ctx::ES_MASKS];
+  }
+  *flags = static_cast<const unsigned char*>(e.f0);
+  *owner = e.id;
+  return MPSE_OK;
+}
+
+int env_structure_compare(mpse_ctx* ctx, const unsigned char* scanned, const unsigned char* structural, int rows,
+                          int pitch, int nvalid, int code, const int* skip) {
+  if (!ctx->es_check_word) {
+    void* p = nullptr;
+    MPSE_TRY(mpse_malloc(ctx, 16, &p));
+    MPSE_TRY(device_zero(ctx, p, 16));
+    ctx->es_check_word = static_cast<int*>(p);
+  }
+  const long long n = (long long)rows * nvalid;
+  if (n <= 0) return MPSE_OK;
+  hipLaunchKernelGGL(k_flags_compare, dim3((unsigned)((n + 255) / 256)), dim3(256), 0, ctx->stream, scanned, structural, rows,
+                     pitch, nvalid, ctx->es_check_word, code, skip);
+  MPSE_HIP(ctx, hipGetLastError());
+  return MPSE_OK;
+}
+
+int env_structure_solve_end(mpse_ctx* ctx, int status) {
+  if (!ctx->es_check_used) return status;
+  ctx->es_check_used = false;
+  if (!ctx->es_check_word) return status;
+  int word = 0;
+  MPSE_TRY(mpse_memcpy_d2h(ctx, &word, ctx->es_check_word, sizeof(int)));
+  if (!word) return status;
+  MPSE_TRY(device_zero(ctx, ctx->es_check_word, 16));
+  ++ctx->es_stats[mpse_ctx::ES_VIOLATIONS];
+  return mpse_fail(ctx, MPSE_ERR_ARG, "environment structure: a tile with data lies outside the declared structure "
+                   "(MPSE_ENV_STRUCTURE_CHECK; where: %d = 1 product operand A | 2 operand B | 4 grouped product | 8 fused "
+                   "matvec L | 16 fused matvec R)", word);
+}
+
+
+void* plan_cache_find(mpse_ctx* ctx, int kind, const std::vector<unsigned char>& key) {
+  std::lock_guard<std::mutex> lock(ctx->plan_mu);
+  for (auto& e : ctx->plan_cache)
+    if (e.kind == kind && e.key == key) {
+      e.tick = ++ctx->plan_tick;
+      ++ctx->es_stats[mpse_ctx::ES_PLAN_HITS];
+      return e.dev;
+    }
+  return nullptr;
+}
+
+int plan_cache_insert(mpse_ctx* ctx, int kind, const std::vector<unsigned char>& key, uint64_t owner0, uint64_t owner1,
+                      const void* foreign, size_t bytes, void** dev) {
+  MPSE_TRY(mpse_malloc(ctx, bytes, dev));
+  void* evicted = nullptr;
+  {
+    std::lock_guard<std::mutex> lock(ctx->plan_mu);
+    if (ctx->plan_cache.size() >= mpse_ctx::PLAN_CACHE_CAP) {
+      size_t old = 0;
+      for (size_t i = 1; i < ctx->plan_cache.size(); ++i)
+        if (ctx->plan_cache[i].tick < ctx->plan_cache[old].tick) old = i;
+      evicted = ctx->plan_cache[old].dev;
+      ctx->plan_cache[old] = std::move(ctx->plan_cache.back());
+      ctx->plan_cache.pop_back();
+    }
+    mpse_ctx::PlanEntry e;
+    e.kind = kind, e.key = key, e.owner[0] = owner0, e.owner[1] = owner1, e.foreign = foreign, e.dev = *dev;
+    e.tick = ++ctx->plan_tick;
+    ctx->plan_cache.push_back(std::move(e));
+    ++ctx->es_stats[mpse_ctx::ES_PLAN_BUILDS];
+  }
+  if (evicted) mpse_free(ctx, evicted);
+  return MPSE_OK;
+}
+
+void plan_cache_collect_ptr(mpse_ctx* ctx, const void* freed, std::vector<void*>* release) {
+  std::lock_guard<std::mutex> lock(ctx->plan_mu);
+  for (size_t i = 0; i < ctx->plan_cache.size();) {
+    if (ctx->plan_cache[i].foreign == freed) {
+      release->push_back(ctx->plan_cache[i].dev);
+      ctx->plan_cache[i] = std::move(ctx->plan_cache.back());
+      ctx->plan_cache.pop_back();
+    } else {
+      ++i;
+    }
+  }
+}
+
+
+extern "C" int mpse_env_structure_create(mpse_ctx* ctx, int nq, int64_t n_row, const int64_t* qrow, int64_t n_chan,
+                                         const int64_t* qchan, int64_t n_col, const int64_t* qcol, int sign_chan,
+                                         const int64_t* qoff, uint64_t* handle) {
+  if (!ctx || !handle) return MPSE_ERR_ARG;
+  *handle = 0;
+  if (nq < 1 || nq > 16 || n_row < 1 || n_chan < 1 || n_col < 1 || n_row > (1 << 20) || n_chan > (1 << 20) ||
+      n_col > (1 << 20) || !qrow || !qchan || !qcol || (sign_chan != 1 && sign_chan != -1))
+    return mpse_fail(ctx, MPSE_ERR_ARG, "env_structure_create: bad argument");
+  auto e = std::make_shared<mpse_ctx::EnvStruct>();
+  e->s = mpse_structure::build(nq, (int)n_row, qrow, (int)n_chan, qchan, (int)n_col, qcol, sign_chan, qoff);
+  std::lock_guard<std::mutex> lock(ctx->plan_mu);
+  e->id = ctx->env_struct_next++;
+  ctx->env_structs.emplace(e->id, e);
+  *handle = e->id;
+  return MPSE_OK;
+}
+
+extern "C" int mpse_env_structure_free(mpse_ctx* ctx, uint64_t handle) {
+  if (!ctx) return MPSE_ERR_ARG;
+  if (!handle) return MPSE_OK;
+  std::shared_ptr<mpse_ctx::EnvStruct> e;
+  std::vector<void*> release;
+  {
+    std::lock_guard<std::mutex> lock(ctx->plan_mu);
+    auto it = ctx->env_structs.find(handle);
+    if (it == ctx->env_structs.end()) return mpse_fail(ctx, MPSE_ERR_ARG, "env_structure_free: unknown handle");
+    e = it->second;
+    ctx->env_structs.erase(it);
+    for (int i = 0; i < 2; ++i)
+      if (ctx->env_struct_pending[i] == handle) ctx->env_struct_pending[i] = 0;
+    for (size_t i = 0; i < ctx->plan_cache.size();) {
+      if (ctx->plan_cache[i].owner[0] == handle || ctx->plan_cache[i].owner[1] == handle) {
+        release.push_back(ctx->plan_cache[i].dev);
+        ctx->plan_cache[i] = std::move(ctx->plan_cache.back());
+        ctx->plan_cache.pop_back();
+      } else {
+        ++i;
+      }
+    }
+  }
+  for (void* p : release) mpse_free(ctx, p);
+  struct_release(ctx, *e);
+  return MPSE_OK;
+}
+
+extern "C" int mpse_expm_env_structure(mpse_ctx* ctx, uint64_t handle_l, uint64_t handle_r) {
+  if (!ctx) return MPSE_ERR_ARG;
+  std::lock_guard<std::mutex> lock(ctx->plan_mu);
+  const uint64_t hs[2] = {handle_l, handle_r};
+  for (int i = 0; i < 2; ++i)
+    if (hs[i] && !ctx->env_structs.count(hs[i])) return mpse_fail(ctx, MPSE_ERR_ARG, "expm_env_structure: unknown handle");
+  ctx->env_struct_pending[0] = handle_l, ctx->env_struct_pending[1] = handle_r;
+  return MPSE_OK;
+}
+
+extern "C" int mpse_env_structure_stats(mpse_ctx* ctx, int64_t* out, int n) {
+  if (!ctx || n < 0 || (n > 0 && !out)) return MPSE_ERR_ARG;
+  std::lock_guard<std::mutex> lock(ctx->plan_mu);
+  ctx->es_stats[mpse_ctx::ES_ALIVE] = (long long)ctx->env_structs.size();
+  for (int i = 0; i < n && i < mpse_ctx::ES_COUNT; ++i) out[i] = ctx->es_stats[i];
+  if (n > mpse_ctx::ES_COUNT) out[mpse_ctx::ES_COUNT] = (long long)ctx->plan_cache.size();
+  for (int i = mpse_ctx::ES_COUNT + 1; i < n; ++i) out[i] = 0;
+  return MPSE_OK;
+}
diff --git a/renormalizer_amd/csrc/mpse_vec.hip b/renormalizer_amd/csrc/mpse_vec.hip
--- a/renormalizer_amd/csrc/mpse_vec.hip
+++ b/renormalizer_amd/csrc/mpse_vec.hip
@@ -890,6 +890,7 @@
   SolveScope scope(ctx);
   scope.skip = done;
   keep_env_masks(scope, h);
+  env_structure_take(ctx, &scope, h);
   scope.cmask = ctx->cmask_pending;
   ctx->cmask_pending = mpse_ctx::CMask();
 
@@ -1263,8 +1264,13 @@
   if (!ctx || !h || !Cin || !out) return MPSE_ERR_ARG;
   if (MPSE_RECORDING(ctx)) return mpse_fail(ctx, MPSE_ERR_ARG, "expm_lanczos: cannot be recorded (mpse_defer_begin is open)");
   MPSE_BIND(ctx);
-  const int st = expm_lanczos_solve(ctx, dtype, h, dt_re, dt_im, Cin, out, rtol, atol, max_dim, nvec);
+  int st = expm_lanczos_solve(ctx, dtype, h, dt_re, dt_im, Cin, out, rtol, atol, max_dim, nvec);
   ctx->cmask_pending = mpse_ctx::CMask();
+  {
+    std::lock_guard<std::mutex> lock(ctx->plan_mu);
+    ctx->env_struct_pending[0] = ctx->env_struct_pending[1] = 0;
+  }
+  st = env_structure_solve_end(ctx, st);
   return defer_replay(ctx, st);
 }
 
@@ -1395,6 +1401,7 @@
 
   SolveScope scope(ctx);
   keep_env_masks(scope, h);
+  env_structure_take(ctx, &scope, h);
   for (int j = 0;; ++j) {
     MPSE_TRY(heff_apply(ctx, dtype, h, vec(j), W.p, &scope, nullptr));
     dot_partials(W.p, vec(j), part_a);
@@ -1716,6 +1723,12 @@
   const int md = (max_dim <= 0 || max_dim > 128) ? 128 : max_dim;
   const bool cplx = dtype == MPSE_C128;
   const mpse_ctx::CMask saved_mask = ctx->cmask_pending;
+  uint64_t saved_es[2];
+  {
+    std::lock_guard<std::mutex> lock(ctx->plan_mu);
+    saved_es[0] = ctx->env_struct_pending[0], saved_es[1] = ctx->env_struct_pending[1];
+    ctx->env_struct_pending[0] = ctx->env_struct_pending[1] = 0;
+  }
   std::vector<int> st(count, MPSE_OK);
   std::vector<std::string> msg(count);
   std::vector<char> grouped(count, 0);
@@ -1789,6 +1802,10 @@
     if (st[i] != MPSE_OK) msg[i] = ctx->err;
   }
   ctx->cmask_pending = saved_mask;
+  {
+    std::lock_guard<std::mutex> lock(ctx->plan_mu);
+    ctx->env_struct_pending[0] = saved_es[0], ctx->env_struct_pending[1] = saved_es[1];
+  }
   int status = MPSE_OK;
   for (int i = 0; i < count; ++i)
     if (st[i] != MPSE_OK) {
diff --git a/renormalizer_amd/engine.py b/renormalizer_amd/engine.py
--- a/renormalizer_amd/engine.py
+++ b/renormalizer_amd/engine.py
@@ -125,6 +125,11 @@
     "mpse_nrm2": [C.c_void_p, C.c_int, C.c_void_p, C.c_int64, _dblp],
     "mpse_scaled_rms": [C.c_void_p, C.c_int, C.c_void_p, C.c_void_p, C.c_void_p, C.c_int64, C.c_double, C.c_double, _dblp],
     "mpse_expm_centre_mask": [C.c_void_p, C.c_void_p, C.c_int64],
+    "mpse_env_structure_create": [C.c_void_p, C.c_int, C.c_int64, _i64p, C.c_int64, _i64p, C.c_int64, _i64p, C.c_int,
+                                  _i64p, C.POINTER(C.c_uint64)],
+    "mpse_env_structure_free": [C.c_void_p, C.c_uint64],
+    "mpse_expm_env_structure": [C.c_void_p, C.c_uint64, C.c_uint64],
+    "mpse_env_structure_stats": [C.c_void_p, _i64p, C.c_int],
     "mpse_defer_begin": [C.c_void_p, C.c_int],
     "mpse_defer_end": [C.c_void_p],
     "mpse_defer_arm": [C.c_void_p, C.c_int],
@@ -548,6 +553,45 @@
         self._check(self.lib.mpse_block_qr_stats(self.ctx, C.byref(a), C.byref(b), C.byref(c)))
         return a.value, b.value, c.value
 
+    ENV_STRUCTURE_STATS = ("alive", "masks_built", "plan_builds", "plan_hits", "solve_scans", "solve_plan_launches",
+                           "check_violations", "plans_alive")
+    ENV_STRUCTURE_CACHE_CAP = 1024
+
+    def env_structure_stats(self):
+        out = (C.c_int64 * len(self.ENV_STRUCTURE_STATS))()
+        self._check(self.lib.mpse_env_structure_stats(self.ctx, out, len(out)))
+        return dict(zip(self.ENV_STRUCTURE_STATS, [int(v) for v in out]))
+
+    def env_structure(self, qrow, qchan, qcol, sign_chan, qoff=None):
+        cache = self.__dict__.setdefault("_env_structs", {})
+        arrs = [np.ascontiguousarray(np.asarray(q, dtype=np.int64).reshape(len(q), -1)) for q in (qrow, qchan, qcol)]
+        nq = arrs[0].shape[1]
+        off = np.zeros(nq, dtype=np.int64) if qoff is None else np.ascontiguousarray(np.asarray(qoff, dtype=np.int64).reshape(-1))
+        if any(a.shape[1] != nq for a in arrs) or off.shape[0] != nq:
+            return 0
+        key = (int(sign_chan), off.tobytes()) + tuple((a.shape[0], a.tobytes()) for a in arrs)
+        hit = cache.get(key)
+        if hit is not None:
+            return hit
+        if len(cache) >= self.ENV_STRUCTURE_CACHE_CAP:
+            self.env_structure_trim()
+        h = C.c_uint64(0)
+        ptr = lambda a: a.ctypes.data_as(_i64p)
+        self._check(self.lib.mpse_env_structure_create(self.ctx, nq, arrs[0].shape[0], ptr(arrs[0]), arrs[1].shape[0],
+                                                       ptr(arrs[1]), arrs[2].shape[0], ptr(arrs[2]), int(sign_chan),
+                                                       ptr(off), C.byref(h)))
+        cache[key] = int(h.value)
+        return cache[key]
+
+    def env_structure_alive(self, handle):
+        return bool(handle) and handle in self.__dict__.get("_env_structs", {}).values()
+
+    def env_structure_trim(self):
+        cache = self.__dict__.setdefault("_env_structs", {})
+        for h in cache.values():
+            self._check(self.lib.mpse_env_structure_free(self.ctx, h))
+        cache.clear()
+
     def heff_fused_stats(self):
         a, b = C.c_int64(), C.c_int64()
         self._check(self.lib.mpse_heff_fused_stats(self.ctx, C.byref(a), C.byref(b)))
diff --git a/renormalizer_amd/lib/krylov.py b/renormalizer_amd/lib/krylov.py
--- a/renormalizer_amd/lib/krylov.py
+++ b/renormalizer_amd/lib/krylov.py
@@ -21,6 +21,9 @@
         nv = C.c_int()
         if Afunc.cmask is not None:
             eng._check(eng.lib.mpse_expm_centre_mask(eng.ctx, Afunc.cmask.ptr, Afunc.cmask.nbytes))
+        hl, hr = [h if eng.env_structure_alive(h) else 0 for h in Afunc.estruct]
+        if hl or hr:
+            eng._check(eng.lib.mpse_expm_env_structure(eng.ctx, hl, hr))
         eng._check(eng.lib.mpse_expm_lanczos(eng.ctx, v.code, C.byref(Afunc.heff), dt.real, dt.imag, v.ptr, out.ptr,
                                              rtol, atol, 0, C.byref(nv)))
         return out, nv.value
diff --git a/renormalizer_amd/mps/hop_expr.py b/renormalizer_amd/mps/hop_expr.py
--- a/renormalizer_amd/mps/hop_expr.py
+++ b/renormalizer_amd/mps/hop_expr.py
@@ -18,6 +18,7 @@
         self.nsite = nsite
         self.cshape = cshape
         self.cmask = None
+        self.estruct = (0, 0)
         self.l = eng.asdevice(ltensor)
         self.r = eng.asdevice(rtensor)
         if self.twolayer:
@@ -88,6 +89,14 @@
     return Hop(ltensor, rtensor, list(cmo), cshape, twolayer)
 
 
+def env_structure(eng, qbra, qmpo, qket, domain, mpo_qntot=None):
+    if qbra is None or qmpo is None or qket is None:
+        return 0
+    if domain == "L":
+        return eng.env_structure(qbra, qmpo, qket, +1)
+    return eng.env_structure(qbra, qmpo, qket, -1, mpo_qntot)
+
+
 _CMASK_CACHE = {}
 
 
diff --git a/renormalizer_amd/mps/mps.py b/renormalizer_amd/mps/mps.py
--- a/renormalizer_amd/mps/mps.py
+++ b/renormalizer_amd/mps/mps.py
@@ -11,7 +11,7 @@
 from ..model import Model, Op, OpSum
 from ..utils import CompressConfig, CompressCriteria, EvolveConfig, EvolveMethod, OptimizeConfig
 from . import svd_qn
-from .hop_expr import centre_tile_mask, hop_expr
+from .hop_expr import centre_tile_mask, env_structure, hop_expr
 from . import lib as _lib
 from .lib import Environ, contract_one_site
 from .mpo import Mpo
@@ -1271,6 +1271,15 @@
         self.hh_sites.tick()
         self.qr_redone = eng.block_qr_stats()[2]
         self.use_cmask = os.environ.get("MPSE_CENTRE_MASK", "1") != "0"
+        self.use_estruct = (os.environ.get("MPSE_ENV_STRUCTURE", "1") != "0" and getattr(mpo, "qn", None) is not None
+                            and len(mpo.qn) == self.n + 1)
+
+    ESTRUCT_MIN_BOND = 32
+
+    def env_struct(self, domain, bond, qn):
+        if not self.use_estruct or len(qn) < self.ESTRUCT_MIN_BOND:
+            return 0
+        return env_structure(self.eng, qn, self.mpo.qn[bond], qn, domain, self.mpo.qntot)
 
     def note_qr(self, imps):
         if self.learn_qr:
@@ -1284,6 +1293,8 @@
         hop = hop_expr(self.environ.read("L", imps - 1), self.environ.read("R", imps + 1), [self.mpo.device(imps, eng)],
                        shape)
         split = (not mps.to_right and imps != 0) or (mps.to_right and imps != n - 1)
+        if len(shape) == 3 and mps.qnidx == imps:
+            hop.estruct = (self.env_struct("L", imps, mps.qn[imps]), self.env_struct("R", imps + 1, mps.qn[imps + 1]))
         qnbigl = qnbigr = plan = None
         if split:
             qnbigl, qnbigr, _ = mps._get_big_qn([imps], need_mat=False)
@@ -1311,6 +1322,7 @@
             mps.qnidx = imps - 1
             r_array = environ.GetLR("R", imps, mps, mpo, itensor=r_array, method="System", canonical=True)
             hop_b = hop_expr(l_array, r_array, [], u.shape)
+            hop_b.estruct = (hop.estruct[0], self.env_struct("R", imps, mps.qn[imps]))
             if self.use_cmask and u.shape[0] * u.shape[1] >= (1 << 14):
                 hop_b.cmask = centre_tile_mask(eng, qnbigl, np.array(qnrset, dtype=int).reshape(-1, q), mps.qntot,
                                                u.shape)
@@ -1320,6 +1332,7 @@
         mps.qnidx = imps + 1
         l_array = environ.GetLR("L", imps, mps, mpo, itensor=l_array, method="System", canonical=True)
         hop_b = hop_expr(l_array, r_array, [], vt.shape)
+        hop_b.estruct = (self.env_struct("L", imps + 1, mps.qn[imps + 1]), hop.estruct[1])
         if self.use_cmask and vt.shape[0] * vt.shape[1] >= (1 << 14):
             hop_b.cmask = centre_tile_mask(eng, np.array(qnlset, dtype=int).reshape(-1, q), qnbigr, mps.qntot,
                                            vt.shape)
```
